# cuulee/reporter

Hardware: AMD Instinct MI355X
Metric: GPS probes matched/sec (whole node) (higher is better)
Workload: dtype f64; 1 GPU; c2; graph=metro, nodes=1048576, directed_edges=3527937, osmlr_segments=1361487, traces_per_gpu=10000, streams=1, device_batches=1, output_segments=1688548

## Files before the change

### reporter_amd/csrc/otr_devscan.h

```cpp
#pragma once
#include <hipcub/hipcub.hpp>

#include "otr_hostdev.h"

namespace otr {

struct Workspace {
  void* p = nullptr;
  size_t bytes = 0;
};


template <class In, class Out>
int scan_bytes(In in, Out out, int n, size_t* bytes, hipStream_t stream, std::string* err) {
  HIPCHK(hipcub::DeviceScan::InclusiveSum(nullptr, *bytes, in, out, n, stream));
  return OTR_OK;
}

template <class K, class V>
int sort_bytes(const K* k_in, K* k_out, const V* v_in, V* v_out, int n, int begin_bit, int end_bit, size_t* bytes,
               hipStream_t stream, std::string* err) {
  HIPCHK(hipcub::DeviceRadixSort::SortPairs(nullptr, *bytes, k_in, k_out, v_in, v_out, n, begin_bit, end_bit, stream));
  return OTR_OK;
}

template <class In, class Out, class K, class V>
int scan_sort_bytes(In in, Out out, const K* k_in, K* k_out, const V* v_in, V* v_out, int n, size_t* bytes,
                    hipStream_t stream, std::string* err) {
  size_t scan = 0, sort = 0;
  if (int rc = scan_bytes(in, out, n, &scan, stream, err)) return rc;
  if (int rc = sort_bytes(k_in, k_out, v_in, v_out, n, 0, 8 * (int)sizeof(K), &sort, stream, err)) return rc;
  *bytes = std::max(scan, sort);
  return OTR_OK;
}

template <class In, class Out>
int inclusive_sum(Workspace ws, In in, Out out, int n, hipStream_t stream, std::string* err) {
  HIPCHK(hipcub::DeviceScan::InclusiveSum(ws.p, ws.bytes, in, out, n, stream));
  return OTR_OK;
}

template <class K, class V>
int sort_pairs(Workspace ws, const K* k_in, K* k_out, const V* v_in, V* v_out, int n, int begin_bit, int end_bit,
               hipStream_t stream, std::string* err) {
  HIPCHK(hipcub::DeviceRadixSort::SortPairs(ws.p, ws.bytes, k_in, k_out, v_in, v_out, n, begin_bit, end_bit, stream));
  return OTR_OK;
}

template <class In, class Out>
int pool_scan(DevPool& pool, int slot, In in, Out out, int64_t n, hipStream_t stream, std::string* err) {
  Workspace ws;
  if (int rc = scan_bytes(in, out, (int)n, &ws.bytes, stream, err)) return rc;
  ws.p = pool.get<char>(slot, ws.bytes);
  return inclusive_sum(ws, in, out, (int)n, stream, err);
}

template <class K, class V>
int pool_sort(DevPool& pool, int slot, const K* k_in, K* k_out, const V* v_in, V* v_out, int64_t n, int begin_bit,
              int end_bit, hipStream_t stream, std::string* err) {
  Workspace ws;
  if (int rc = sort_bytes(k_in, k_out, v_in, v_out, (int)n, begin_bit, end_bit, &ws.bytes, stream, err)) return rc;
  ws.p = pool.get<char>(slot, ws.bytes);
  return sort_pairs(ws, k_in, k_out, v_in, v_out, (int)n, begin_bit, end_bit, stream, err);
}

template <class T>
struct Fetch {
  T* host;
  const T* dev;
};
template <class T>
Fetch<T> fetch(T* host, const T* dev) {
  return Fetch<T>{host, dev};
}
template <class... T>
int read_back(hipStream_t stream, std::string* err, Fetch<T>... f) {
  hipError_t e = hipSuccess;
  ((e = e != hipSuccess ? e : hipMemcpyAsync(f.host, f.dev, sizeof(T), hipMemcpyDeviceToHost, stream)), ...);
  HIPCHK(e);
  HIPCHK(hipStreamSynchronize(stream));
  return OTR_OK;
}

}
```

### reporter_amd/csrc/otr_engine.h

```cpp
#pragma once
#include <hip/hip_runtime.h>

#include <shared_mutex>
#include <string>
#include <vector>

#include "../../include/otr.h"
#include "otr_device.h"
#include "otr_hostdev.h"
#include "otr_tiers.h"

namespace otr {

struct Config {
  ModeParams mp;
  std::string graph_path;
  int device = 0;
};

ModeParams default_mode_params();
void finalize_params(MatchParams* p);
const char* check_params(const MatchParams& p);

struct GraphState {
  bool ready = false;
  int device = 0;
  DevGraph dg{};
  ModeParams defaults{};
  std::vector<void*> allocs;
  uint64_t n_nodes = 0, n_edges = 0, n_segments = 0;
  std::vector<unsigned long long> seg_id;
  std::shared_mutex mu;
};

GraphState& graph_state();
int engine_configure(const Config& cfg, std::string* err);

struct ReportLists {
  int32_t n;
  const int64_t* seg_off;
  const unsigned long long* seg_id;
  const double *start, *end;
  const uint8_t* internal;
  const int32_t* queue;
  const uint8_t* has_length;
  const int32_t *length, *begin_shape;
  const int64_t* end_time;
  const double* threshold;
  const uint32_t *rl, *tl;
  unsigned long long *rep_id, *rep_next;
  double *rep_t0, *rep_t1;
  int32_t *rep_length, *rep_queue, *n_rep, *shape_used, *counts;
  double* lengths;
  int32_t* length_set;
};

int report_lists_device(const ReportLists& h, std::string* err);

struct GSlab {
  uint32_t* key = nullptr;
  unsigned long long* lab = nullptr;
  uint32_t* qmark = nullptr;
  uint32_t* fr = nullptr;
  uint32_t* touched = nullptr;
};

void turn_table(double factor, int32_t* tab181);

uint64_t uuid_key_host(const char* uuid, int64_t len);

struct SessionStore;
void sessions_destroy(SessionStore* s);

struct SessionReports {
  int64_t n_windows, n_reports;
  const int64_t *trigger, *rep_off;
  const unsigned long long *id, *next_id;
  const double *t0, *t1;
  const int32_t *length, *queue_length;
  bool* added;
};
bool sessions_last_reports(SessionStore* s, SessionReports* out);

struct TileStore;
void tile_store_destroy(TileStore* s);

struct TileText;
void tile_text_destroy(TileText* t);

struct CulledRows {
  const otr_tile_row* sorted;
  const otr_tile_row* kept;
  const int64_t* kept_incl;
  int64_t n_kept;
};

struct Matcher {
  hipStream_t stream = nullptr;
  SessionStore* ses = nullptr;
  TileStore* tst = nullptr;
  TileText* ttx = nullptr;
  DevPool pool{PoolOwner::matcher, nullptr, 0};
  GSlab gslab[2];
  std::vector<int32_t> h_turn;
  std::vector<int64_t> h_trace_state_off, h_state_probe, h_trace_route_off, h_trace_seg_off, h_seg_way_off,
      h_trace_rep_off;
  std::vector<int32_t> h_cand_count, h_winner, h_subpath, h_seg_length, h_seg_queue, h_seg_bshape, h_seg_eshape,
      h_rep_length, h_rep_queue, h_shape_used, h_stats, h_trace_status;
  std::vector<uint32_t> h_cand_edge, h_route_edge, h_seg_way;
  std::vector<double> h_cand_p, h_cand_sqd, h_seg_start, h_seg_end, h_rep_t0, h_rep_t1, h_stats_len;
  std::vector<unsigned long long> h_seg_id, h_rep_id, h_rep_next;
  std::vector<uint8_t> h_seg_internal;
  std::vector<otr_tile_row> h_tile_rows;
  bool pts_have = false;
  otr_point_result pts{};
  std::vector<uint8_t> h_pt_kind;
  std::vector<uint32_t> h_pt_edge;
  std::vector<double> h_pt_frac, h_pt_lat, h_pt_lon, h_pt_dist;
  std::vector<int64_t> h_pt_state, h_pt_pos;
  bool trv_have = false;
  otr_traversal_result trv{};
  std::vector<int64_t> h_tr_off, h_tr_first, h_tr_s0, h_tr_s1;
  std::vector<uint32_t> h_tr_edge, h_tr_way;
  std::vector<uint64_t> h_tr_seg;
  std::vector<double> h_tr_f0, h_tr_f1, h_tr_t0, h_tr_t1;
  hipEvent_t ev[kEvents];
  bool ev_init = false;

  template <class T>
  T* need(int slot, size_t n);
  template <class T>
  T* want(int slot, size_t n);
  bool release_optional();
  bool opt_busy = false;
  int run(const otr_trace_batch* in, const ModeParams& mp, otr_batch_result* out, std::string* err);
  int matched_points(otr_point_result* out, std::string* err) const;
  int edge_traversals(otr_traversal_result* out, std::string* err) const;
  int edge_observations(int quantisation, otr_hist_entry** d_entries, int64_t* n, std::string* err);
  int tiles_cull(const otr_tile_row* rows, int64_t n, int memory, int privacy, int rules, const otr_tile_row** out,
                 int64_t* n_out, std::string* err);
  int hist_reduce(const void* in, int64_t n, int memory, int rows_in, int privacy, const otr_hist_entry** out,
                  int64_t* n_out, std::string* err);
  int cull_device(const otr_tile_row* d_in, int64_t n, int privacy, int rules, CulledRows* out, std::string* err);
  int copy_out(void* dst, const void* src, size_t bytes, int dst_memory, std::string* err);
  int ingest(const char* text, int64_t len, int memory, const otr_ingest_format* fmt, otr_ingest_result* out,
             std::string* err);
  int format_messages(const otr_message_format* fmt, const otr_messages* msgs, otr_format_result* out,
                      std::string* err);
  int sessions_open(const otr_session_config* cfg, int32_t uuid_bytes, std::string* err);
  int sessions_close(std::string* err);
  int sessions_push(const otr_session_points* pts, const otr_session_names* names, otr_session_result* out,
                    std::string* err);
  int sessions_punctuate(int64_t ts, otr_session_result* out, std::string* err);
  int sessions_advance(const otr_session_points* pts, const otr_session_names* names, otr_trace_batch* out,
                       std::string* err);
  int sessions_commit(const int32_t* shape_used, const int32_t* status, int memory, std::string* err);
  int sessions_windows(otr_session_result* out, std::string* err);
  int sessions_snapshot(otr_session_snapshot* out, std::string* err);
  int sessions_restore(const otr_session_snapshot* snap, const otr_session_names* names, int memory,
                       otr_session_restore_result* out, std::string* err);
  int sessions_restore_records(const otr_session_records* recs, const otr_session_names* names,
                               otr_session_restore_result* out, std::string* err);
  int sessions_export_records(otr_session_records* out, std::string* err);
  int sessions_take(int n_parts, int part, int remove, otr_session_snapshot* out, std::string* err);
  bool sessions_named() const;
  int sessions_names(otr_session_name_list* out, std::string* err);
  int sessions_last_refusal(otr_session_name_refusal* out, std::string* err);
  void sessions_refusal_message(const int64_t* d_message);
  void sessions_refusal_clear();
  const uint8_t* fmt_text = nullptr;
  int64_t fmt_text_len = 0;
  int tile_store_open(const otr_tile_store_config* cfg, int flags, std::string* err);
  int tile_store_snapshot(int flags, otr_tile_snapshot* out, std::string* err);
  int tile_store_restore(const otr_tile_snapshot* snap, int memory, otr_tile_restore_result* out, std::string* err);
  int tile_store_export_records(int32_t slice_size, otr_tile_records* out, std::string* err);
  int tile_store_restore_records(const otr_tile_records* in, otr_tile_restore_result* out, std::string* err);
  int tile_store_close(std::string* err);
  int tile_store_add_session(otr_tile_add_result* out, std::string* err);
  int tile_store_add_reports(int64_t n_windows, const int64_t* rep_off, const uint64_t* id, const uint64_t* next_id,
                             const double* t0, const double* t1, const int32_t* length, const int32_t* queue_length,
                             int memory, otr_tile_add_result* out, std::string* err);
  int tile_store_add_rows(const otr_tile_row* rows, int64_t n, int memory, otr_tile_add_result* out, std::string* err);
  int tile_store_flush(otr_tile_flush_result* out, std::string* err);
  int tiles_text(const otr_tile_row* rows, int64_t n, int memory, int quantisation, int rules, const char* source,
                 const char* mode, int flags, otr_tile_text_result* out, std::string* err);
  int tile_store_flush_text(const char* source, const char* mode, int flags, otr_tile_flush_result* flush,
                            otr_tile_text_result* out, std::string* err);
  ~Matcher();
};

}
```

### reporter_amd/csrc/otr_engine.hip

```cpp
#include <cerrno>
#include <cstdio>
#include <cstring>
#include <fcntl.h>
#include <sys/mman.h>
#include <sys/stat.h>
#include <unistd.h>

#include "otr_devscan.h"
#include "otr_engine.h"
#include "otr_kernels.h"
#include "otr_edge.h"
#include "otr_edge1.h"
#include "otr_launch.h"
#include "otr_points.h"
#include "otr_slots.h"
#include "otr_traversals.h"

namespace otr {
static_assert(kTraceWaves == 4, "grid_trace_rows (otr_launch.h) assumes 4 traces per block");

void finalize_params(MatchParams* p) {
  p->inv2s2 = 1.0 / (p->sigma_z * p->sigma_z * 2.0);
  p->inv_beta = 1.0 / p->beta;
  if (p->kmax > OTR_KMAX) p->kmax = OTR_KMAX;
  if (p->kmax < 1) p->kmax = 1;
}

const char* check_params(const MatchParams& p) {
  if (!(p.breakage_distance >= 0.0 && p.breakage_distance <= kMaxBreakage))
    return "breakage_distance must be within [0, 30000] m";
  if (!(p.max_route_distance_factor >= 0.0) || !(p.max_route_distance_factor < 1e6))
    return "max_route_distance_factor must be >= 0";
  if (!(p.max_route_time_factor >= 0.0) || !(p.max_route_time_factor < 1e6)) return "max_route_time_factor must be >= 0";
  if (!(p.turn_penalty_factor >= 0.0) || !(p.turn_penalty_factor <= 1e6)) return "turn_penalty_factor must be within [0, 1e6]";
  if (!(p.sigma_z > 0.0)) return "sigma_z must be > 0";
  if (!(p.beta > 0.0)) return "beta must be > 0";
  if (!(p.search_radius >= 0.0) || !(p.max_search_radius >= 0.0)) return "search_radius must be >= 0";
  if (!(p.interpolation_distance >= 0.0)) return "interpolation_distance must be >= 0";
  if (!(p.speed_kph >= 0.0) || !(p.queue_kph >= 0.0)) return "speed_kph and queue_kph must be >= 0";
  return nullptr;
}

ModeParams default_mode_params() {
  ModeParams mp{};
  for (int m = 0; m < OTR_MODES; ++m) {
    MatchParams& p = mp.m[m];
    p.sigma_z = 4.07;
    p.beta = 3.0;
    p.max_route_distance_factor = 5.0;
    p.max_route_time_factor = 2.0;
    p.breakage_distance = 2000.0;
    p.interpolation_distance = 10.0;
    p.search_radius = 50.0;
    p.max_search_radius = 100.0;
    p.gps_accuracy = 5.0;
    p.kmax = 32;
    p.queue_kph = 10.0;
  }
  mp.m[0].turn_penalty_factor = 200.0;
  mp.m[1].turn_penalty_factor = 140.0;
  mp.m[1].speed_kph = 18.0;
  mp.m[1].queue_kph = 5.0;
  mp.m[2].turn_penalty_factor = 100.0;
  mp.m[2].speed_kph = 5.1;
  mp.m[2].queue_kph = 2.0;
  for (int m = 0; m < OTR_MODES; ++m) finalize_params(&mp.m[m]);
  mp.delta = 60.0;
  return mp;
}

static uint32_t edge_time_ds(uint32_t attr, uint32_t len_mm, double speed_cap) {
  double kph = (double)OTR_ATTR_SPEED(attr);
  if (!(kph > 0.0)) kph = 30.0;
  if (speed_cap > 0.0 && speed_cap < kph) kph = speed_cap;
  const double v = (double)len_mm * 0.036 / kph;
  return v < 2.0e9 ? (uint32_t)llround(v) : 2000000000u;
}

static int seg_heading(const int32_t* a, const int32_t* b) {
  const double la1 = (double)a[0] * 1e-6, lo1 = (double)a[1] * 1e-6;
  const double la2 = (double)b[0] * 1e-6, lo2 = (double)b[1] * 1e-6;
  const double m = 20037581.187 / 180.0;
  const double x = (lo2 - lo1) * m * cos_deg(0.5 * (la1 + la2));
  const double y = (la2 - la1) * m;
  if (x == 0.0 && y == 0.0) return -1;
  double deg = atan2(x, y) * (180.0 / 3.14159265358979323846);
  if (deg < 0.0) deg = deg + 360.0;
  return (int)(llround(deg) % 360);
}

void turn_table(double factor, int32_t* tab) {
  const double x = -1.0 / 45.0;
  double r = 1.0, term = 1.0;
  for (int k = 1; k <= 20; ++k) {
    term = term * x / (double)k;
    r = r + term;
  }
  double f = 1.0;
  for (int i = 0; i <= 180; ++i) {
    const double v = 1000.0 * factor * f;
    tab[i] = factor > 0.0 ? (int32_t)llround(v) : 0;
    f = f * r;
  }
}

GraphState& graph_state() {
  static GraphState gs;
  return gs;
}

namespace {
struct Mapped {
  void* p = MAP_FAILED;
  size_t n = 0;
  ~Mapped() {
    if (p != MAP_FAILED) munmap(p, n);
  }
};
struct Staged {
  std::vector<void*> allocs;
  bool adopted = false;
  ~Staged() {
    if (!adopted)
      for (void* q : allocs) (void)hipFree(q);
  }
};
}

int engine_configure(const Config& cfg, std::string* err) {
  for (int m = 0; m < OTR_MODES; ++m)
    if (const char* bad = check_params(cfg.mp.m[m])) {
      if (err) *err = std::string("config: ") + bad;
      return OTR_BAD_REQUEST;
    }
  int fd = open(cfg.graph_path.c_str(), O_RDONLY);
  if (fd < 0) {
    if (err) *err = "cannot open graph file " + cfg.graph_path + ": " + strerror(errno);
    return OTR_BAD_REQUEST;
  }
  struct stat st;
  fstat(fd, &st);
  Mapped mf;
  mf.n = (size_t)st.st_size;
  mf.p = mf.n >= sizeof(otr_graph_header) ? mmap(nullptr, mf.n, PROT_READ, MAP_PRIVATE, fd, 0) : MAP_FAILED;
  close(fd);
  if (mf.p == MAP_FAILED) {
    if (err) *err = "cannot map graph file " + cfg.graph_path;
    return OTR_BAD_REQUEST;
  }
  const char* base = (const char*)mf.p;
  otr_graph_header h;
  memcpy(&h, base, sizeof(h));
  if (memcmp(h.magic, OTR_GRAPH_MAGIC, 8) != 0 || h.version != OTR_GRAPH_VERSION ||
      h.array_offset[OTR_A_END] > (uint64_t)st.st_size) {
    if (err) *err = "not an OTR graph file: " + cfg.graph_path;
    return OTR_BAD_REQUEST;
  }
  if (h.n_nodes >= (1u << 28)) {
    if (err) *err = "graph has more than 2^28 nodes";
    return OTR_BAD_REQUEST;
  }
  if (h.n_edges >= (1u << 28)) {
    if (err) *err = "graph has more than 2^28 directed edges";
    return OTR_BAD_REQUEST;
  }
  const uint32_t* dst = (const uint32_t*)(base + h.array_offset[OTR_A_EDGE_DST]);
  const float* lenf = (const float*)(base + h.array_offset[OTR_A_EDGE_LEN]);
  const uint32_t* attr = (const uint32_t*)(base + h.array_offset[OTR_A_EDGE_ATTR]);
  const uint32_t* row = (const uint32_t*)(base + h.array_offset[OTR_A_NODE_ROW]);
// ... 51 lines not shown
    int hb = -1, he = -1;
    for (uint32_t k = k0; k + 1 < k1 && hb < 0; ++k) hb = seg_heading(sll + 2ull * k, sll + 2ull * k + 2);
    for (uint32_t k = k1 - 1; k > k0 && he < 0; --k) he = seg_heading(sll + 2ull * k - 2, sll + 2ull * k);
    head[e] = make_short2((short)(hb < 0 ? 0 : hb), (short)(he < 0 ? 0 : he));
  }
  std::vector<uint2> adje(4ull * h.n_nodes + 4, make_uint2(0u, 0u));
  for (uint32_t u = 0; u < h.n_nodes; ++u)
    for (uint32_t k = 0; k < 4 && row[u] + k < row[u + 1]; ++k) {
      const uint32_t e = row[u] + k;
      adje[4ull * u + k] = make_uint2(e, (uint32_t)(uint16_t)head[e].x | ((uint32_t)(uint16_t)head[e].y << 16));
    }
  const size_t es = 4ull * h.n_edges + 4;
  std::vector<uint4> erec(es, make_uint4(kAdjDstMask, 0u, 0u, 0u));
  std::vector<uint32_t> erec_t(es * OTR_MODES, 0u);
  for (uint32_t b = 0; b < h.n_edges; ++b) {
    const uint32_t v = dst[b], deg = row[v + 1] - row[v];
    for (uint32_t k = 0; k < 4; ++k) {
      const uint32_t hend = (uint32_t)(uint16_t)head[b].y << 8;
      if (k >= deg) {
        erec[4ull * b + k] = make_uint4(kAdjDstMask, 0u, hend, v);
        continue;
      }
      const uint32_t e = row[v] + k;
      const uint32_t x = e | ((attr[e] & OTR_ATTR_ACCESS_MASK) << 28) | ((k == 3 && deg > 4) ? kAdjMore : 0u);
      erec[4ull * b + k] =
          make_uint4(x, len[e], (uint32_t)turn_degree((int)head[b].y, (int)head[e].x) | hend, v);
      for (int m = 0; m < OTR_MODES; ++m) erec_t[es * m + 4ull * b + k] = std::min(et[m][e], 0x1FFFFu);
    }
  }
  const uint32_t* cedge = (const uint32_t*)(base + h.array_offset[OTR_A_CELL_EDGE]);
  std::vector<uint4> crec(3 * ((size_t)h.n_cell_entries + 1), make_uint4(0u, 0u, 0u, 0u));
  for (uint64_t q = 0; q < h.n_cell_entries; ++q) {
    const uint32_t e = cedge[q];
    if (e >= h.n_edges) {
      if (err) *err = "graph cell index names a missing edge";
      return OTR_BAD_REQUEST;
    }
    const uint32_t k0 = eshape[e], k1 = eshape[e + 1];
    crec[3 * q] = make_uint4(e, k0, k1, attr[e]);
    uint32_t pt[8] = {0u, 0u, 0u, 0u, 0u, 0u, 0u, 0u};
    for (uint32_t i = 0; i < 4 && k0 + i < k1; ++i) {
      pt[2 * i] = (uint32_t)sll[2ull * (k0 + i)];
      pt[2 * i + 1] = (uint32_t)sll[2ull * (k0 + i) + 1];
    }
    crec[3 * q + 1] = make_uint4(pt[0], pt[1], pt[2], pt[3]);
    crec[3 * q + 2] = make_uint4(pt[4], pt[5], pt[6], pt[7]);
  }
  HIPCHK(hipSetDevice(cfg.device));
  Staged sg;
  bool alloc_ok = true;
  auto upv = [&](const void* src, size_t bytes) -> void* {
    void* d = nullptr;
    if (hipMalloc(&d, bytes ? bytes : 16) != hipSuccess) {
      alloc_ok = false;
      return nullptr;
    }
    sg.allocs.push_back(d);
    if (bytes && hipMemcpy(d, src, bytes, hipMemcpyHostToDevice) != hipSuccess) alloc_ok = false;
    return d;
  };
  auto up = [&](int a, size_t bytes) -> void* { return upv(base + h.array_offset[a], bytes); };
  DevGraph g{};
  g.node_row = (const uint32_t*)up(OTR_A_NODE_ROW, 4ull * (h.n_nodes + 1));
  g.rev_row = (const uint32_t*)up(OTR_A_REV_ROW, 4ull * (h.n_nodes + 1));
  g.node_ll = (const int2*)up(OTR_A_NODE_LL, 8ull * h.n_nodes);
  g.rev_edge = (const uint32_t*)up(OTR_A_REV_EDGE, 4ull * h.n_edges);
  g.edge_src = (const uint32_t*)up(OTR_A_EDGE_SRC, 4ull * h.n_edges);
  g.edge_dst = (const uint32_t*)up(OTR_A_EDGE_DST, 4ull * h.n_edges);
  g.edge_len = (const float*)up(OTR_A_EDGE_LEN, 4ull * h.n_edges);
  g.edge_attr = (const uint32_t*)up(OTR_A_EDGE_ATTR, 4ull * h.n_edges);
  g.edge_shape = (const uint32_t*)up(OTR_A_EDGE_SHAPE, 4ull * (h.n_edges + 1));
  g.edge_seg = (const uint32_t*)up(OTR_A_EDGE_SEG, 4ull * h.n_edges);
  g.edge_way = (const uint32_t*)up(OTR_A_EDGE_WAY, 4ull * h.n_edges);
  g.shape_ll = (const int2*)up(OTR_A_SHAPE_LL, 8ull * h.n_shape);
  g.seg_id = (const unsigned long long*)up(OTR_A_SEG_ID, 8ull * h.n_segments);
  g.seg_len = (const uint32_t*)up(OTR_A_SEG_LEN, 4ull * h.n_segments);
  g.cell_row = (const uint32_t*)up(OTR_A_CELL_ROW, 4ull * (h.n_cells + 1));
  g.cell_edge = (const uint32_t*)up(OTR_A_CELL_EDGE, 4ull * h.n_cell_entries);
  g.len_mm = (const uint32_t*)upv(len.data(), 4ull * len.size());
  g.edge_pack = (const uint4*)upv(pack.data(), sizeof(uint4) * pack.size());
  g.eprep = (const uint4*)upv(eprep.data(), sizeof(uint4) * eprep.size());
  g.adj = (const uint4*)upv(adj.data(), sizeof(uint4) * adj.size());
  g.node_minin = (const uint32_t*)upv(minin.data(), 4ull * minin.size());
  {
    std::vector<uint32_t> all_et, all_at;
    for (int m = 0; m < OTR_MODES; ++m) {
      all_et.insert(all_et.end(), et[m].begin(), et[m].end());
      all_at.insert(all_at.end(), at[m].begin(), at[m].end());
    }
    g.edge_t = (const uint32_t*)upv(all_et.data(), 4ull * all_et.size());
    g.adj_t = (const uint32_t*)upv(all_at.data(), 4ull * all_at.size());
    g.edge_t_stride = (uint32_t)et[0].size();
    g.adj_t_stride = (uint32_t)at[0].size();
  }
  g.edge_head = (const short2*)upv(head.data(), sizeof(short2) * head.size());
  g.adj_e = (const uint2*)upv(adje.data(), sizeof(uint2) * adje.size());
  g.erec = (const uint4*)upv(erec.data(), sizeof(uint4) * erec.size());
  g.erec_t = (const uint32_t*)upv(erec_t.data(), 4ull * erec_t.size());
  g.erec_stride = es;
  g.cell_rec = (const uint4*)upv(crec.data(), sizeof(uint4) * crec.size());
  if (!alloc_ok) {
    if (err) *err = "device allocation for the graph failed";
    return OTR_DEVICE_ERROR;
  }
  g.n_nodes = h.n_nodes;
  g.n_edges = h.n_edges;
  g.n_segments = h.n_segments;
  g.grid_rows = h.grid_rows;
  g.grid_cols = h.grid_cols;
  g.grid_min_lat = h.grid_min_lat;
  g.grid_min_lon = h.grid_min_lon;
  g.grid_cell_deg = h.grid_cell_deg;
  std::vector<unsigned long long> sid((const unsigned long long*)(base + h.array_offset[OTR_A_SEG_ID]),
                                      (const unsigned long long*)(base + h.array_offset[OTR_A_SEG_ID]) + h.n_segments);
  GraphState& gs = graph_state();
  std::vector<void*> old;
  {
    std::unique_lock<std::shared_mutex> lk(gs.mu);
    old.swap(gs.allocs);
    gs.allocs = sg.allocs;
    sg.adopted = true;
    gs.dg = g;
    gs.n_nodes = h.n_nodes;
    gs.n_edges = h.n_edges;
    gs.n_segments = h.n_segments;
    gs.seg_id.swap(sid);
    gs.defaults = cfg.mp;
    gs.device = cfg.device;
    gs.ready = true;
  }
  for (void* q : old) (void)hipFree(q);
  return OTR_OK;
}



bool Matcher::release_optional() {
  if (opt_busy) return false;
  bool any = false;
  for (int s = 0; s < (int)pool.b.size(); ++s)
    if (optional_slot(s) && pool.held(s, 0)) {
      if (!any && stream) (void)hipStreamSynchronize(stream);
      any = true;
      pool.drop(s);
    }
  return any;
}

Matcher::~Matcher() {
  if (ses) sessions_destroy(ses);
  if (tst) tile_store_destroy(tst);
  if (ttx) tile_text_destroy(ttx);
  pool.release();
  for (auto& sl : gslab)
    for (void* q : {(void*)sl.key, (void*)sl.lab, (void*)sl.qmark, (void*)sl.fr, (void*)sl.touched})
      if (q) (void)hipFree(q);
  if (ev_init)
    for (auto& e : ev) (void)hipEventDestroy(e);
  if (stream) (void)hipStreamDestroy(stream);
}

__global__ void k_capacity(int32_t n_traces, const int64_t* trace_state_off, const int32_t* cand_count,
                           const int32_t* path_len, int64_t* cap) {
  int t = blockIdx.x * blockDim.x + threadIdx.x;
  if (t >= n_traces) return;
  int64_t c = 2;
  for (int64_t s = trace_state_off[t]; s < trace_state_off[t + 1]; ++s) {
    if (cand_count[s] <= 0) continue;
    c += 3;
    if (path_len[s] > 0) c += path_len[s];
  }
  cap[t] = c;
}

__global__ void k_fill_i32(int32_t* p, int64_t n, int32_t v) {
  int64_t i = (int64_t)blockIdx.x * blockDim.x + threadIdx.x;
  if (i < n) p[i] = v;
}

__device__ inline void block_append(bool hit, int64_t value, int64_t* list, unsigned long long* count) {
  __shared__ unsigned int s_n;
  __shared__ unsigned long long s_base;
  if (threadIdx.x == 0) s_n = 0;
  __syncthreads();
  unsigned int my = 0;
  if (hit) my = atomicAdd(&s_n, 1u);
  __syncthreads();
  if (threadIdx.x == 0) s_base = s_n ? atomicAdd(count, (unsigned long long)s_n) : 0ull;
  __syncthreads();
  if (hit) list[s_base + my] = value;
}

__global__ void k_collect(int64_t n, const int32_t* flag, int64_t* list, unsigned long long* count) {
  const int64_t i = (int64_t)blockIdx.x * blockDim.x + threadIdx.x;
  block_append(i < n && flag[i], i, list, count);
}

__global__ void k_collect_tier(int64_t n, int32_t* flag, uint32_t want, int64_t* list, unsigned long long* count) {
  const int64_t i = (int64_t)blockIdx.x * blockDim.x + threadIdx.x;
  const int f = i < n ? flag[i] : 0;
  const bool sel = f != 0 && ((want >> f) & 1u);
  if (sel) flag[i] = 0;
  block_append(sel, i, list, count);
}

__global__ void k_collect_flagged(int64_t n, const int32_t* flag, int64_t* list, unsigned long long* count) {
  const int64_t i = (int64_t)blockIdx.x * blockDim.x + threadIdx.x;
  block_append(i < n && flag[i] != 0, i, list, count);
}

__global__ void k_collect_tier_from(const int64_t* cand, const unsigned long long* n_cand, int32_t* flag,
                                    uint32_t want, int64_t* list, unsigned long long* count) {
  const int64_t n = (int64_t)*n_cand;
  for (int64_t base = (int64_t)blockIdx.x * blockDim.x; base < n; base += (int64_t)gridDim.x * blockDim.x) {
    const int64_t i = base + threadIdx.x;
    const int64_t task = i < n ? cand[i] : 0;
    const int f = i < n ? flag[task] : 0;
    const bool sel = f != 0 && ((want >> f) & 1u);
    if (sel) flag[task] = 0;
    block_append(sel, task, list, count);
  }
}

constexpr int kSortBuckets = 4096;
__global__ __launch_bounds__(1024) void k_sort_hist(const int64_t* list, const unsigned long long* n_in,
                                                    const uint4* rec, int shift, uint32_t* hist) {
  __shared__ uint32_t h[kSortBuckets];
  const int64_t n = (int64_t)*n_in, i = (int64_t)blockIdx.x * blockDim.x + threadIdx.x;
  if ((int64_t)blockIdx.x * blockDim.x >= n) return;
  for (int b = threadIdx.x; b < kSortBuckets; b += blockDim.x) h[b] = 0;
  __syncthreads();
  if (i < n) atomicAdd(&h[min(rec[3 * list[i]].z >> shift, (uint32_t)kSortBuckets - 1u)], 1u);
  __syncthreads();
  for (int b = threadIdx.x; b < kSortBuckets; b += blockDim.x)
    if (h[b]) atomicAdd(&hist[b], h[b]);
}
__global__ __launch_bounds__(1024) void k_sort_scan(uint32_t* hist) {
  __shared__ uint32_t part[1024];
  constexpr int per = kSortBuckets / 1024;
  uint32_t v[per], t = 0;
  for (int q = 0; q < per; ++q) t += (v[q] = hist[threadIdx.x * per + q]);
  part[threadIdx.x] = t;
  __syncthreads();
  for (int off = 1; off < 1024; off <<= 1) {
    const uint32_t x = threadIdx.x >= (unsigned)off ? part[threadIdx.x - off] : 0u;
    __syncthreads();
    part[threadIdx.x] += x;
    __syncthreads();
  }
  uint32_t base = part[threadIdx.x] - t;
  for (int q = 0; q < per; ++q) {
    hist[threadIdx.x * per + q] = base;
    base += v[q];
  }
}
__global__ __launch_bounds__(1024) void k_sort_place(const int64_t* list, const unsigned long long* n_in,
                                                     const uint4* rec, int shift, uint32_t* cursor, int64_t* out) {
  __shared__ uint32_t h[kSortBuckets];
  const int64_t n = (int64_t)*n_in, i = (int64_t)blockIdx.x * blockDim.x + threadIdx.x;
  if ((int64_t)blockIdx.x * blockDim.x >= n) return;
  for (int b = threadIdx.x; b < kSortBuckets; b += blockDim.x) h[b] = 0;
  __syncthreads();
  int64_t task = 0;
  uint32_t key = 0, r = 0;
  if (i < n) {
    task = list[i];
    key = min(rec[3 * task].z >> shift, (uint32_t)kSortBuckets - 1u);
    r = atomicAdd(&h[key], 1u);
  }
  __syncthreads();
  for (int b = threadIdx.x; b < kSortBuckets; b += blockDim.x)
    if (h[b]) h[b] = atomicAdd(&cursor[b], h[b]);
  __syncthreads();
  if (i < n) out[h[key] + r] = task;
}

__global__ void k_collect_tier_list(const unsigned long long* n_in, int32_t* flag, uint32_t want, int64_t* list,
                                    unsigned long long* count) {
  const int64_t i = (int64_t)blockIdx.x * blockDim.x + threadIdx.x;
  const int f = i < (int64_t)*n_in ? flag[i] : 0;
  const bool sel = f != 0 && ((want >> f) & 1u);
  if (sel) flag[i] = 0;
  block_append(sel, i, list, count);
}

__global__ void k_step_list(int64_t n_states, const int64_t* prev, const uint8_t* brk, const int32_t* cand_count,
                            int64_t* list, unsigned long long* count) {
  const int64_t s = (int64_t)blockIdx.x * blockDim.x + threadIdx.x;
  block_append(s < n_states && cand_count[s] > 0 && prev[s] >= 0 && !brk[s], s, list, count);
}

__global__ void k_step_lists(int64_t n_states, const int64_t* prev, const uint8_t* brk, const int32_t* cand_count,
                             PathClass pc, int64_t* list, unsigned long long* count_front,
                             unsigned long long* count_back, unsigned long long* n_all) {
  const int64_t s = (int64_t)blockIdx.x * blockDim.x + threadIdx.x;
  if (s == 0) *n_all = (unsigned long long)n_states;
  const bool hit = s < n_states && cand_count[s] > 0 && prev[s] >= 0 && !brk[s];
  bool small = false;
  if (hit) {
    const int64_t sp = prev[s];
    const int md = pc.mode[pc.state_trace[s]] < OTR_MODES ? pc.mode[pc.state_trace[s]] : 0;
    const uint32_t r = pc.trans[pc.trans_off[s] + (int64_t)pc.winner[sp] * cand_count[s] + pc.winner[s]];
    const double b = fmin(floor(pc.bound[s] * 1000.0), (double)r) * 1e-3;
    small = !((pc.turn_modes >> md) & 1u) && pc.est4 * (float)(b * b) <= pc.small_keys;
  }
  const unsigned long long mf = __ballot(hit && small), mb = __ballot(hit && !small);
  const int lane = (int)(threadIdx.x % OTR_WAVE);
  unsigned long long bf = 0, bb = 0;
  if (lane == 0) {
    if (mf) bf = atomicAdd(count_front, (unsigned long long)__popcll(mf));
    if (mb) bb = atomicAdd(count_back, (unsigned long long)__popcll(mb));
  }
  bf = __shfl(bf, 0);
  bb = __shfl(bb, 0);
  const unsigned long long below = (1ull << lane) - 1ull;
  if (hit && small) list[bf + __popcll(mf & below)] = s;
  if (hit && !small) list[n_states - 1 - (int64_t)(bb + __popcll(mb & below))] = s;
}

__global__ __launch_bounds__(kCShards) void k_ctr_fold(const unsigned long long* in, unsigned long long* out) {
  __shared__ unsigned long long part[kCShards / OTR_WAVE];
  unsigned long long v = in[(size_t)blockIdx.x * kCShards + threadIdx.x];
  for (int o = OTR_WAVE / 2; o > 0; o >>= 1) v += __shfl_xor(v, o);
  if (lane_id() == 0) part[threadIdx.x / OTR_WAVE] = v;
  __syncthreads();
  if (threadIdx.x == 0) {
    unsigned long long t = 0;
    for (int w = 0; w < kCShards / OTR_WAVE; ++w) t += part[w];
    out[blockIdx.x] = t;
  }
}

constexpr double kSmallKeys = 24.0;
constexpr double kTinyKeys = 12.0;
constexpr double kSmallPathKeys = 16.0;

static const std::vector<int>& route_tiers() {
  static const std::vector<int> t = parse_route_tiers(getenv("OTR_TIERS"));
  return t;
}

static unsigned pgrid(unsigned full, int64_t units) {
  const int64_t u = std::max<int64_t>(8, (units + 7) / 8 * 8);
  return (unsigned)std::min<int64_t>((int64_t)full, u);
}

constexpr unsigned kCollectGrid = 512;

struct Batch {
  Matcher& mat;
  const otr_trace_batch* in;
  const ModeParams& mp;
  otr_batch_result* out;
  std::string* err;
  const DevGraph& g;
  hipStream_t stream;
  bool timing;
  bool used[10] = {false};
  int32_t T = 0;
  int64_t N = 0, S = 0, NT = 0, NT4 = 0, NT8 = 0, NTR = 0, C = 0;
  BatchDev b{};
  CandBuf cb{};
  StepBuf sb{};
  PrepArgs pr{};
  RouteArgs ra{};
  GenArgs ga{};
  ViterbiArgs va{};
  SegArgs sa{};
  HistArgs ha{};
  PointArgs pta{};
  bool want_points = false;
  TravArgs tva{};
  bool want_traversals = false;
  int64_t n_trav = 0;
  size_t hist_len = 0, scan_bytes = 0;
  int64_t *trace_state_off = nullptr, *state_probe = nullptr, *trans_off = nullptr, *path_off = nullptr,
          *cap_off = nullptr;
  int32_t *state_trace = nullptr, *path_len = nullptr;
  uint32_t turn_modes = 0;
  bool k32 = true;
  int vit_variant = 0;
  int route_g = 2, n_est_tiers = 0;
  float est_k = 0.f, est_v[OTR_MODES] = {};
  uint32_t est_tier_keys[8] = {0u, 0u, 0u, 0u, 0u, 0u, 0u, 0u};
  double tiny_keys = 0.0;
  static constexpr size_t bank = (size_t)OTR_COUNTERS * kCShards;
  static constexpr size_t n_ctr = kBanks * (size_t)OTR_COUNTERS;
  unsigned long long *d_counters = nullptr, *cnt = nullptr;
  int64_t *list = nullptr, *fail_tasks = nullptr, *flagged = nullptr;
  int32_t *task_ovf = nullptr, *d_turn = nullptr;
  uint32_t *trans = nullptr, *trans_tc = nullptr;
  uint4* task_rec = nullptr;
  unsigned long long *rwork = nullptr, *queues = nullptr;
  int32_t* task_dump = nullptr;
  bool node_tasks = true, turns = false, nresume = true, eresume = true;
  int64_t* steps = nullptr;
  unsigned long long *nsteps_d = nullptr, *nsteps4_d = nullptr, h_nsteps[2] = {0ull, 0ull};
  const unsigned long long* nscan_d = nullptr;
  int32_t* step_ovf = nullptr;
  bool small_paths = false;
  std::vector<unsigned long long> hc;
  unsigned long long h_fail[2] = {0ull, 0ull};
  std::vector<int64_t> route_n, seg_n, way_n, rep_n;

  int upload(), states(), candidates(), link(), route_first(), route_retry(), route_edge(), route_global(), viterbi();
  int paths(), paths_attempt(int64_t capacity), segments(), points(), traversals(), drain(), debug_fail(),
      name_failed();
  void fold_counters();
  int copy_out(), points_out(), traversals_out();

  template <class X> X* need(int slot, size_t n) { return mat.need<X>(slot, n); }
  template <class X> X* want(int slot, size_t n) { return mat.want<X>(slot, n); }
  void tb(int k) {
    if (timing) (void)hipEventRecord(mat.ev[2 * k], stream);
  }
  void te(int k) {
    if (timing) (void)hipEventRecord(mat.ev[2 * k + 1], stream), used[k] = true;
  }
  void tier_begin(int slot) {
    if (timing) (void)hipEventRecord(mat.ev[route_event(slot)], stream);
  }
  void tier_end(int slot) {
    if (timing) (void)hipEventRecord(mat.ev[route_event(slot) + 1], stream);
  }
  unsigned long long* tier_bank(int slot) const { return d_counters + kRouteTiers[slot].bank * bank; }
  unsigned long long* tier_work(int slot) const { return rwork ? tier_bank(slot) : nullptr; }
  unsigned long long* tier_list(int slot) const { return cnt + kRouteTiers[slot].list; }
  unsigned long long* tier_queue(int slot) const { return queues + kRouteTiers[slot].queue * kQueueWords; }
  unsigned long long ctr(int bank_, int k) const { return hc[(size_t)bank_ * OTR_COUNTERS + (size_t)k]; }

  int scan(const int64_t* src, int64_t* dst_np1, int64_t n);
  int read_i64(const int64_t* p, int64_t* v);
  int slabs(int tier, GSlabs* out);
  template <class V>
  int dl(V& vec, const void* src, size_t n) {
    vec.resize(n ? n : 1);
    if (n) HIPCHK(hipMemcpyAsync(vec.data(), src, n * sizeof(vec[0]), hipMemcpyDeviceToHost, stream));
    return OTR_OK;
  }
  template <int CAP, int G, bool LIST>
  void launch_route(unsigned grid, const RouteArgs& args, unsigned long long* ctr_bank);
  void first_tier(int slot, int cap, int g_, int64_t n_tasks, int64_t task_base, int64_t units);
  int retry_tier(int code, const RouteArgs& rb, unsigned long long* ctr_bank);
};

int Matcher::run(const otr_trace_batch* in, const ModeParams& mp, otr_batch_result* out, std::string* err) {
  pts_have = false;
  pts = otr_point_result{};
  trv_have = false;
  trv = otr_traversal_result{};
  const int rc = guarded(stream, err, [&]() -> int {
    GraphState& gs = graph_state();
    std::shared_lock<std::shared_mutex> graph_lock(gs.mu);
    if (!gs.ready) {
      if (err) *err = "otr_configure has not been called";
      return OTR_NOT_CONFIGURED;
    }
    HIPCHK(hipSetDevice(gs.device));
    if (!stream) HIPCHK(hipStreamCreateWithFlags(&stream, hipStreamNonBlocking));
    if (!ev_init) {
      for (auto& e : ev) HIPCHK(hipEventCreate(&e));
      ev_init = true;
    }
    memset(out, 0, sizeof(*out));
    out->n_traces = in->n_traces;
    if (in->n_traces <= 0) {
      pts_have = (in->flags & OTR_BATCH_MATCHED_POINTS) != 0;
      if (in->flags & OTR_BATCH_EDGE_TRAVERSALS) {
        trv.d_trace_off = need<int64_t>(S_TR_OFF, 1);
        HIPCHK(hipMemsetAsync(trv.d_trace_off, 0, 8, stream));
        HIPCHK(hipStreamSynchronize(stream));
        if (in->flags & OTR_BATCH_COPY_OUT) {
          h_tr_off.assign(1, 0);
          trv.trace_off = h_tr_off.data();
        }
        trv_have = true;
      }
      return OTR_OK;
    }
    Batch c{*this, in, mp, out, err, gs.dg, stream, (in->flags & OTR_BATCH_TIMING) != 0};
    c.T = in->n_traces;
    c.want_points = (in->flags & OTR_BATCH_MATCHED_POINTS) != 0;
    c.want_traversals = (in->flags & OTR_BATCH_EDGE_TRAVERSALS) != 0;
    int rc;
    if ((rc = c.upload()) || (rc = c.states()) || (rc = c.candidates()) || (rc = c.link()) || (rc = c.route_first()) ||
        (rc = c.route_retry()) || (rc = c.route_edge()) || (rc = c.route_global()) || (rc = c.viterbi()) ||
        (rc = c.paths()) || (rc = c.segments()) || (rc = c.points()) || (rc = c.traversals()) || (rc = c.drain()) ||
        (rc = c.debug_fail()) || (rc = c.name_failed()))
      return rc;
    c.fold_counters();
    if ((rc = c.copy_out()) || (rc = c.points_out())) return rc;
    return c.traversals_out();
  });
  opt_busy = false;
  return rc;
}

int Batch::upload() {
  b.n_traces = T;
  if (in->memory == OTR_MEM_HOST) {
    N = in->trace_offsets[T];
    int64_t* d_off = need<int64_t>(S_TRACE_OFF, T + 1);
    double* d_lat = need<double>(S_LAT, N);
    double* d_lon = need<double>(S_LON, N);
    int64_t* d_time = need<int64_t>(S_TIME, N);
    uint8_t* d_mode = need<uint8_t>(S_MODE, T);
    float* d_acc = in->accuracy ? need<float>(S_ACC, N) : nullptr;
    HIPCHK(hipMemcpyAsync(d_off, in->trace_offsets, 8 * (T + 1), hipMemcpyHostToDevice, stream));
    HIPCHK(hipMemcpyAsync(d_lat, in->lat, 8 * N, hipMemcpyHostToDevice, stream));
    HIPCHK(hipMemcpyAsync(d_lon, in->lon, 8 * N, hipMemcpyHostToDevice, stream));
    HIPCHK(hipMemcpyAsync(d_time, in->time, 8 * N, hipMemcpyHostToDevice, stream));
    HIPCHK(hipMemcpyAsync(d_mode, in->mode, T, hipMemcpyHostToDevice, stream));
    if (d_acc) HIPCHK(hipMemcpyAsync(d_acc, in->accuracy, 4 * N, hipMemcpyHostToDevice, stream));
    b.trace_off = d_off;
    b.lat = d_lat;
    b.lon = d_lon;
    b.time = d_time;
    b.mode = d_mode;
    b.acc = d_acc;
  } else {
    if (int rc = read_back(stream, err, fetch(&N, in->trace_offsets + T))) return rc;
    b.trace_off = in->trace_offsets;
    b.lat = in->lat;
    b.lon = in->lon;
    b.time = in->time;
    b.mode = in->mode;
    b.acc = in->accuracy;
  }
  out->n_probes = N;
  if (N > kMaxBatchProbes || max_launch_items(N, N, 1) > kMaxDispatchItems) {
    if (err)
      *err = "batch of " + std::to_string(N) + " probes: at most " + std::to_string(kMaxBatchProbes) +
             " per otr_match_batch call";
    return OTR_BAD_REQUEST;
  }
  mat.h_trace_status.assign(T, OTR_OK);
  d_counters = need<unsigned long long>(S_COUNTERS, kBanks * bank + n_ctr);
  HIPCHK(hipMemsetAsync(d_counters, 0, kBanks * bank * 8, stream));
  return OTR_OK;
}

int Batch::scan(const int64_t* src, int64_t* dst_np1, int64_t n) {
  HIPCHK(hipMemsetAsync(dst_np1, 0, 8, stream));
  if (n == 0) return OTR_OK;
  Workspace tmp;
  if (int rc = otr::scan_bytes(src, dst_np1 + 1, (int)n, &tmp.bytes, stream, err)) return rc;
  scan_bytes = std::max(scan_bytes, tmp.bytes);
  tmp.p = need<char>(S_SCAN_TMP, scan_bytes);
  return inclusive_sum(tmp, src, dst_np1 + 1, (int)n, stream, err);
}

int Batch::read_i64(const int64_t* p, int64_t* v) { return read_back(stream, err, fetch(v, p)); }

int Batch::states() {
  int rc;
  int64_t* state_cnt = need<int64_t>(S_STATE_CNT, T);
  trace_state_off = need<int64_t>(S_TRACE_STATE_OFF, T + 1);
  tb(OTR_STAGE_STATES);
  k_select_states<<<grid_ceil(T, 256), 256, 0, stream>>>(b, mp, state_cnt, nullptr, nullptr, nullptr);
  te(OTR_STAGE_STATES);
  if ((rc = scan(state_cnt, trace_state_off, T))) return rc;
  if ((rc = read_i64(trace_state_off + T, &S))) return rc;
  out->n_states = S;
  state_probe = need<int64_t>(S_STATE_PROBE, S);
  state_trace = need<int32_t>(S_STATE_TRACE, S);
  k_select_states<<<grid_ceil(T, 256), 256, 0, stream>>>(b, mp, state_cnt, trace_state_off, state_probe,
                                                         state_trace);
  return OTR_OK;
}

int Batch::candidates() {
  cb.edge = need<uint32_t>(S_CAND_EDGE, (size_t)S * OTR_KMAX);
  cb.p = need<double>(S_CAND_P, (size_t)S * OTR_KMAX);
  cb.sqd = need<double>(S_CAND_SQD, (size_t)S * OTR_KMAX);
  cb.count = need<int32_t>(S_CAND_COUNT, S);
  cb.radius = need<double>(S_CAND_RADIUS, S);
  if (S > 0) {
    tb(OTR_STAGE_CANDIDATES);
    bool kc32 = true;
    for (int m = 0; m < OTR_MODES; ++m) {
      const MatchParams& q = mp.m[m];
      const double rmax = b.acc ? q.max_search_radius
                                : std::min(q.max_search_radius, std::max(q.search_radius, q.gps_accuracy));
      kc32 = kc32 && q.kmax <= 32 && rmax <= 100.0;
    }
    static const int cand_g = getenv("OTR_CAND_G") ? atoi(getenv("OTR_CAND_G")) : 2;
    if (kc32 && cand_g == 2)
      k_candidates<2><<<(unsigned)grid_candidates((S + 1) / 2).blocks, 64, 0, stream>>>(g, b, mp, S, state_probe,
                                                                                       state_trace, cb, d_counters);
    else
      k_candidates<1><<<(unsigned)grid_candidates(S).blocks, 64, 0, stream>>>(g, b, mp, S, state_probe, state_trace, cb,
                                                                        d_counters);
    te(OTR_STAGE_CANDIDATES);
  }
  return OTR_OK;
}

int Batch::link() {
  int rc;
  for (int m = 0; m < OTR_MODES; ++m)
    if (mp.m[m].turn_penalty_factor > 0.0) turn_modes |= 1u << m;
  sb.prev = need<int64_t>(S_PREV, S);
  sb.g = need<double>(S_G, S);
  sb.bound = need<double>(S_BOUND, S);
  sb.forced = need<uint8_t>(S_FORCED, S);
  sb.bt = need<int32_t>(S_BT, S);
  sb.ntask = need<int64_t>(S_NTASK, S);
  sb.ntrans = need<int64_t>(S_NTRANS, S);
  int64_t* task_off = need<int64_t>(S_TASK_OFF, S + 1);
  trans_off = need<int64_t>(S_TRANS_OFF, S + 1);
  tb(OTR_STAGE_LINK);
  k_link<<<(unsigned)grid_link(T).blocks, 256, 0, stream>>>(b, mp, trace_state_off, state_probe, cb.count, sb);
  pr.n_states = S;
  pr.prev = sb.prev;
  pr.bound = sb.bound;
  pr.cand_count = cb.count;
  pr.cand_edge = cb.edge;
  pr.cand_p = cb.p;
  pr.state_trace = state_trace;
  pr.mode = b.mode;
  pr.cprep = need<uint4>(S_CPREP, (size_t)S * OTR_KMAX);
  pr.cprep_t = need<uint2>(S_CPREP_T, (size_t)S * OTR_KMAX);
  pr.clen = need<uint2>(S_CLEN, (size_t)S * OTR_KMAX);
  pr.nroot = need<int32_t>(S_CAND_NROOT, S);
  pr.turn_modes = turn_modes;
  for (int m = 0; m < OTR_MODES; ++m) k32 = k32 && mp.m[m].kmax <= 32;
  if (S > 0) {
    if (k32) k_prep<2><<<(unsigned)grid_per_state_waves(S, 2).blocks, 256, 0, stream>>>(g, pr);
    else k_prep<1><<<(unsigned)grid_per_state_waves(S, 1).blocks, 256, 0, stream>>>(g, pr);
  }
  static const int route_g_env = getenv("OTR_ROUTE_G") ? atoi(getenv("OTR_ROUTE_G")) : 2;
  route_g = route_g_env;
  {
    static const double est_scale = getenv("OTR_EST_K") ? atof(getenv("OTR_EST_K")) : 1.0;
    const double mlat = g.grid_min_lat + 0.5 * g.grid_rows * g.grid_cell_deg;
    const double area = (g.grid_rows * g.grid_cell_deg * kMetersPerDeg) *
                        (g.grid_cols * g.grid_cell_deg * kMetersPerDeg * cos_deg(fmin(fabs(mlat), 89.0)));
    est_k = (float)(est_scale * 0.5 * (area > 0.0 ? (double)g.n_nodes / area : 0.0));
    for (int m = 0; m < OTR_MODES; ++m) {
      const double kph = mp.m[m].speed_kph > 0.0 && mp.m[m].speed_kph < 50.0 ? mp.m[m].speed_kph : 50.0;
      est_v[m] = (float)(kph / 3.6);
    }
    const std::vector<int>& tl = route_tiers();
    n_est_tiers = (int)std::min<size_t>(tl.size(), 8);
    for (int t = 0; t < n_est_tiers; ++t) est_tier_keys[t] = (uint32_t)((tl[t] / 10) * 7 / 8);
  }
  static const double small_keys = getenv("OTR_SMALL_KEYS") ? atof(getenv("OTR_SMALL_KEYS")) : kSmallKeys;
  static const double tiny_keys_env = getenv("OTR_TINY_KEYS") ? atof(getenv("OTR_TINY_KEYS")) : kTinyKeys;
  tiny_keys = tiny_keys_env;
  const bool small_tier = route_g == 2 && k32 && small_keys > 0.0 && est_k > 0.f;
  const bool tiny_tier = small_tier && tiny_keys > 0.0;
  int64_t* ntask4 = small_tier ? need<int64_t>(S_NTASK4, S) : nullptr;
  int64_t* task4_off = small_tier ? need<int64_t>(S_TASK4_OFF, S + 1) : nullptr;
  int64_t* ntask8 = tiny_tier ? need<int64_t>(S_NTASK8, S) : nullptr;
  int64_t* task8_off = tiny_tier ? need<int64_t>(S_TASK8_OFF, S + 1) : nullptr;
  if (S > 0) {
    SmallArgs sm{};
    sm.ntask4 = ntask4;
    sm.ntask8 = ntask8;
    sm.tiny_keys = (float)tiny_keys;
    sm.bound = sb.bound;
    sm.bt = sb.bt;
    sm.forced = sb.forced;
    sm.cand_count = cb.count;
    sm.state_trace = state_trace;
    sm.mode = b.mode;
    sm.turn_modes = turn_modes;
    sm.est_k = est_k;
    for (int m = 0; m < OTR_MODES; ++m) sm.est_v[m] = est_v[m];
    sm.small_keys = (float)small_keys;
    k_ntask<<<grid_ceil(S, 256), 256, 0, stream>>>(S, sb.prev, pr.nroot, sb.ntask, sm);
  }
  if ((rc = scan(sb.ntask, task_off, S))) return rc;
  if (small_tier && (rc = scan(ntask4, task4_off, S))) return rc;
  if (tiny_tier && (rc = scan(ntask8, task8_off, S))) return rc;
  if ((rc = scan(sb.ntrans, trans_off, S))) return rc;
  HIPCHK(hipMemcpyAsync(&NT, task_off + S, 8, hipMemcpyDeviceToHost, stream));
  if (small_tier) HIPCHK(hipMemcpyAsync(&NT4, task4_off + S, 8, hipMemcpyDeviceToHost, stream));
  if (tiny_tier) HIPCHK(hipMemcpyAsync(&NT8, task8_off + S, 8, hipMemcpyDeviceToHost, stream));
  if ((rc = read_back(stream, err, fetch(&NTR, trans_off + S)))) return rc;
  NT += NT4 + NT8;
  task_ovf = need<int32_t>(S_TASK_OVF, NT);
  trans = need<uint32_t>(S_TRANS, NTR);
  trans_tc = need<uint32_t>(S_TRANS_TC, turn_modes ? NTR : 1);
  task_rec = need<uint4>(S_TASK_REC, 3 * (size_t)std::max<int64_t>(NT, 1));
  if (S > 0) {
    TaskArgs ta{};
    ta.n_states = S;
    ta.prev = sb.prev;
    ta.cand_count = cb.count;
    ta.cand_edge = cb.edge;
    ta.edge_dst = g.edge_dst;
    ta.task_off = task_off;
    ta.bound = sb.bound;
    ta.forced = sb.forced;
    ta.bt = sb.bt;
    ta.state_trace = state_trace;
    ta.mode = b.mode;
    ta.cprep = pr.cprep;
    ta.cprep_t = pr.cprep_t;
    ta.trans_off = trans_off;
    ta.turn_modes = turn_modes;
    ta.rec = task_rec;
    ta.ntask4 = ntask4;
    ta.task4_off = task4_off;
    ta.nt4 = NT4;
    ta.ntask8 = ntask8;
    ta.task8_off = task8_off;
    ta.nt8 = NT8;
    ta.flag_turn = task_ovf;
    ta.est_first_keys = route_g == 2 ? (OTR_CAP1 * OTR_LOAD1) / 8 : 0;
    ta.est_k = est_k;
    for (int m = 0; m < OTR_MODES; ++m) ta.est_v[m] = est_v[m];
    ta.n_tiers = n_est_tiers;
    for (int t = 0; t < n_est_tiers; ++t) ta.tier_keys[t] = est_tier_keys[t];
    if (NT > 0) HIPCHK(hipMemsetAsync(task_ovf, 0, 4 * NT, stream));
    if (k32) k_tasks<2><<<(unsigned)grid_per_state_waves(S, 2).blocks, 256, 0, stream>>>(ta);
    else k_tasks<1><<<(unsigned)grid_per_state_waves(S, 1).blocks, 256, 0, stream>>>(ta);
  }
  te(OTR_STAGE_LINK);
  return OTR_OK;
}

int Batch::slabs(int tier, GSlabs* out) {
  GSlab& sl = mat.gslab[tier];
  const uint32_t cap = (uint32_t)kRouteTiers[SLOT_GLOBAL + tier].cap;
  const uint32_t n = tier == 0 ? 1024u : 8u;
  if (!sl.key) {
    const size_t c = (size_t)cap * n;
    void* p[5] = {nullptr, nullptr, nullptr, nullptr, nullptr};
    const size_t bytes[5] = {4 * c, 8 * c, 4 * c, 8 * c, 4 * c};
    bool good = true;
    for (int attempt = 0; attempt < 2; ++attempt) {
      good = true;
      for (int q = 0; q < 5 && good; ++q) good = hipMalloc(&p[q], bytes[q]) == hipSuccess;
      if (good) break;
      (void)hipGetLastError();
      for (void*& q : p)
        if (q) (void)hipFree(q), q = nullptr;
      if (attempt > 0 || !mat.release_optional()) break;
    }
    if (good)
      good = hipMemsetAsync(p[0], 0xFF, 4 * c, stream) == hipSuccess &&
             hipMemsetAsync(p[1], 0xFF, 8 * c, stream) == hipSuccess &&
             hipMemsetAsync(p[2], 0, 4 * c, stream) == hipSuccess;
    if (!good) {
      (void)hipGetLastError();
      for (void* q : p)
        if (q) (void)hipFree(q);
      throw DeviceOom{PoolOwner::matcher, nullptr, S_NUM + tier, 28 * c};
    }
    sl.key = (uint32_t*)p[0];
    sl.lab = (unsigned long long*)p[1];
    sl.qmark = (uint32_t*)p[2];
    sl.fr = (uint32_t*)p[3];
    sl.touched = (uint32_t*)p[4];
  }
  out->key = sl.key;
  out->lab = sl.lab;
  out->qmark = sl.qmark;
  out->fr = sl.fr;
  out->touched = sl.touched;
  out->cap = cap;
  out->n = n;
  return OTR_OK;
}

template <int CAP, int G, bool LIST>
void Batch::launch_route(unsigned grid, const RouteArgs& args, unsigned long long* ctr_bank) {
  if (ctr_bank) k_route<CAP, G, LIST, false, true><<<grid, 64, 0, stream>>>(g, args, ctr_bank);
  else k_route<CAP, G, LIST, false, false><<<grid, 64, 0, stream>>>(g, args, nullptr);
}

void Batch::first_tier(int slot, int cap, int g_, int64_t n_tasks, int64_t task_base, int64_t units) {
  constexpr int64_t kMaxUnits = 1ll << 25;
  unsigned long long* ctr_bank = tier_work(slot);
  if (slot != SLOT_FIRST) tier_begin(slot);
  for (int64_t base = 0; base < units; base += kMaxUnits) {
    RouteArgs rf = ra;
    rf.n_tasks = n_tasks;
    rf.task_base = task_base;
    rf.unit_base = base;
    const int64_t u = std::min<int64_t>(kMaxUnits, units - base);
    const unsigned grid = (unsigned)(8 * ((u + 7) / 8));
    if (slot == SLOT_TINY) launch_route<OTR_CAP8, 8, false>(grid, rf, ctr_bank);
    else if (slot == SLOT_SMALL) launch_route<OTR_CAP4, 4, false>(grid, rf, ctr_bank);
    else if (g_ == 2) launch_route<OTR_CAP1, 2, false>(grid, rf, ctr_bank);
    else launch_route<256, 1, false>(grid, rf, ctr_bank);
  }
  if (slot != SLOT_FIRST) tier_end(slot);
  out->route_tier_code[slot] = route_tier_code(slot, cap, g_);
}

template <int I = 0, class F>
static bool with_retry_shape(int code, F&& f) {
  if constexpr (I < kRetryShapeN) {
    if (code == kRetryShapes[I].code()) {
      f(std::integral_constant<int, I>{});
      return true;
    }
    return with_retry_shape<I + 1>(code, f);
  } else {
    return false;
  }
}

int Batch::retry_tier(int code, const RouteArgs& rb, unsigned long long* ctr_bank) {
  const bool known = with_retry_shape(code, [&](auto i) {
    constexpr int cap = kRetryShapes[decltype(i)::value].cap, gw = kRetryShapes[decltype(i)::value].g;
    launch_route<cap, gw, true>(pgrid(cap <= 512 ? 16384u : 16384u * 512u / cap, (NT + gw - 1) / gw), rb, ctr_bank);
  });
  if (!known) {
    if (err) *err = "no route kernel for retry tier " + std::to_string(code);
    return OTR_DEVICE_ERROR;
  }
  return OTR_OK;
}

int Batch::route_first() {
  d_turn = need<int32_t>(S_TURN, 181 * OTR_MODES);
  mat.h_turn.resize(181 * OTR_MODES);
  for (int m = 0; m < OTR_MODES; ++m) turn_table(mp.m[m].turn_penalty_factor, mat.h_turn.data() + 181 * m);
  HIPCHK(hipMemcpyAsync(d_turn, mat.h_turn.data(), 4 * 181 * OTR_MODES, hipMemcpyHostToDevice, stream));
  ra.task_list = nullptr;
  ra.n_tasks = NT;
  ra.prev = sb.prev;
  ra.g = sb.g;
  ra.bound = sb.bound;
  ra.forced = sb.forced;
  ra.trans_off = trans_off;
  ra.trans = trans;
  ra.cand_count = cb.count;
  ra.cand_edge = cb.edge;
  ra.cand_p = cb.p;
  ra.state_trace = state_trace;
  ra.mode = b.mode;
  ra.bt = sb.bt;
  ra.turn = d_turn;
  ra.trans_tc = trans_tc;
  ra.cprep = pr.cprep;
  ra.cprep_t = pr.cprep_t;
  ra.clen = pr.clen;
  ra.rec = task_rec;
  for (int m = 0; m < OTR_MODES; ++m) ra.inv_beta[m] = mp.m[m].inv_beta;
  ra.overflow_flag = task_ovf;
  ra.stamps = d_counters;
  ra.est_k = est_k;
  for (int m = 0; m < OTR_MODES; ++m) ra.est_v[m] = est_v[m];
  ra.n_tiers = n_est_tiers;
  for (int t = 0; t < n_est_tiers; ++t) ra.tier_keys[t] = est_tier_keys[t];
  cnt = need<unsigned long long>(S_MISC, C_CURSORS + kShards);
  HIPCHK(hipMemsetAsync(cnt, 0, 8 * (C_CURSORS + kShards), stream));
  list = need<int64_t>(S_LIST, std::max<int64_t>(NT, S));
  fail_tasks = need<int64_t>(S_GFLAG, std::max<int64_t>(NT, 1));
  flagged = need<int64_t>(S_FLAGGED, std::max<int64_t>(NT, 1));
  ga.prev = sb.prev;
  ga.g = sb.g;
  ga.bt = sb.bt;
  ga.bound = sb.bound;
  ga.cand_count = cb.count;
  ga.cand_edge = cb.edge;
  ga.cand_p = cb.p;
  ga.cprep = pr.cprep;
  ga.cprep_t = pr.cprep_t;
  ga.state_trace = state_trace;
  ga.mode_of_trace = b.mode;
  ga.turn_modes = turn_modes;
  ga.turn = d_turn;
  ga.rec = task_rec;
  ga.trans_off = trans_off;
  ga.trans = trans;
  ga.trans_tc = trans_tc;
  ga.counters = d_counters;
  ga.n_overflow = cnt + C_GEN_OVERFLOW;
  if (NT == 0) return OTR_OK;
  rwork = (in->flags & OTR_BATCH_ROUTE_WORK) ? d_counters : nullptr;
  turns = turn_modes != 0u;
#ifdef OTR_FORCE_GENERAL
  node_tasks = true;
#else
  node_tasks = turn_modes != (1u << OTR_MODES) - 1u;
#endif
#ifdef OTR_FORCE_RETRY
  {
    const char* fe = getenv("OTR_FORCE_EDGE");
    ra.force_edge = fe ? atoi(fe) : 0;
  }
#endif
  queues = need<unsigned long long>(S_QUEUE, kQueues * kQueueWords);
  HIPCHK(hipMemsetAsync(queues, 0, 8 * kQueues * kQueueWords, stream));
  static const bool nresume_env = !getenv("OTR_NRESUME") || atoi(getenv("OTR_NRESUME")) != 0;
  static const bool eresume_env = !getenv("OTR_E1RESUME") || atoi(getenv("OTR_E1RESUME")) != 0;
  nresume = nresume_env;
  eresume = eresume_env;
  if ((nresume && node_tasks) || (eresume && turns)) task_dump = want<int32_t>(S_TASK_DUMP, NT);
  mat.opt_busy = true;
  ra.task_dump = task_dump;
  tb(OTR_STAGE_ROUTE);
  if (node_tasks) {
    const bool tiny_run = NT8 > 0 && (2 * NT8 >= NT || tiny_keys >= 1e8);
    const int64_t small_lo = tiny_run ? NT8 : 0;
    if (tiny_run) first_tier(SLOT_TINY, OTR_CAP8, 8, NT8, 0, (NT8 + 7) / 8);
    if (NT8 + NT4 - small_lo > 0)
      first_tier(SLOT_SMALL, OTR_CAP4, 4, NT8 + NT4, small_lo, (NT8 + NT4 - small_lo + 3) / 4);
    if (route_g == 2) first_tier(SLOT_FIRST, OTR_CAP1, 2, NT, NT8 + NT4, (NT - NT8 - NT4 + 1) / 2);
    else first_tier(SLOT_FIRST, 256, 1, NT, NT8 + NT4, NT);
  }
  te(OTR_STAGE_ROUTE);
  return OTR_OK;
}

int Batch::route_retry() {
  if (NT == 0) return OTR_OK;
  int rc;
  tb(OTR_STAGE_ROUTE_BIG);
  const std::vector<int>& tiers = route_tiers();
  const int ntier = (int)tiers.size();
  k_collect_flagged<<<grid_ceil(NT, 1024), 1024, 0, stream>>>(NT, task_ovf, flagged, cnt + C_FLAGGED);
  unsigned long long* ndump[2] = {nullptr, nullptr};
  uint32_t nslots[8] = {0u, 0u, 0u, 0u, 0u, 0u, 0u, 0u};
  auto nd_in = [&](int t) { return t > 0 && t < ntier && tiers[t] / 10 >= OTR_ND_IN_MIN; };
  auto nd_out = [&](int t) { return t + 1 < ntier && tiers[t] / 10 >= OTR_ND_OUT_MIN && nd_in(t + 1); };
  if (nresume && node_tasks && task_dump && ntier > 1) {
    static const double gb = getenv("OTR_NDUMP_GB") ? atof(getenv("OTR_NDUMP_GB")) : 4.0;
    const int64_t cap_bytes = (int64_t)(gb * (double)(1ll << 30));
    size_t words[2] = {0, 0};
    for (int t = 0; t + 1 < ntier && t < 8; ++t) {
      if (!nd_out(t)) continue;
      const uint32_t w = nd_words(tiers[t] / 10);
      nslots[t] = (uint32_t)std::min<int64_t>(std::max<int64_t>(NT / 4, 1024), cap_bytes / (8 * (int64_t)w));
      words[t & 1] = std::max<size_t>(words[t & 1], (size_t)nslots[t] * w);
    }
    for (int q = 0; q < 2; ++q)
      if (words[q]) ndump[q] = want<unsigned long long>(q == 0 ? S_NDUMP0 : S_NDUMP1, words[q]);
    if ((words[0] && !ndump[0]) || (words[1] && !ndump[1])) ndump[0] = ndump[1] = nullptr;
  }
  for (int tier = 0; tier < (node_tasks ? ntier : 0); ++tier) {
    const int slot = SLOT_NODE + tier;
    unsigned long long* c = tier_list(slot);
    k_collect_tier_from<<<kCollectGrid, 1024, 0, stream>>>(flagged, cnt + C_FLAGGED, task_ovf,
                                                          0x2u | (((2u << tier) - 1u) << 16), list + 0, c);
    RouteArgs rb = ra;
    rb.task_list = list;
    rb.list_count = c;
    rb.queue = tier_queue(slot);
    const bool din = nd_in(tier) && nd_out(tier - 1) && ndump[(tier + 1) & 1] != nullptr;
    const bool dout = nd_out(tier) && ndump[tier & 1] != nullptr;
    rb.dump_in = din ? ndump[(tier + 1) & 1] : nullptr;
    rb.dump_in_words = din ? nd_words(tiers[tier - 1] / 10) : 0u;
    rb.dump_out = dout ? ndump[tier & 1] : nullptr;
    rb.dump_ctr = queues + dump_ctr_word(slot);
    rb.dump_out_words = dout ? nd_words(tiers[tier] / 10) : 0u;
    rb.dump_out_slots = dout ? nslots[tier] : 0u;
    out->route_tier_code[slot] = tiers[tier];
    tier_begin(slot);
    if ((rc = retry_tier(tiers[tier], rb, tier_work(slot)))) return rc;
    tier_end(slot);
  }
#ifndef OTR_FORCE_GENERAL
  {
    constexpr int cap = kRouteTiers[SLOT_WIDE64].cap;
    unsigned long long* c = tier_list(SLOT_WIDE64);
    k_collect_tier_from<<<kCollectGrid, 1024, 0, stream>>>(flagged, cnt + C_FLAGGED, task_ovf, 0x8u, list, c);
    RouteArgs rb = ra;
    rb.task_list = list;
    rb.list_count = c;
    rb.queue = tier_queue(SLOT_WIDE64);
    out->route_tier_code[SLOT_WIDE64] = route_tier_code(SLOT_WIDE64, cap, 1);
    tier_begin(SLOT_WIDE64);
    if (rwork) k_route<cap, 1, true, true, true><<<pgrid(4096, NT), 64, 0, stream>>>(g, rb, tier_bank(SLOT_WIDE64));
    else k_route<cap, 1, true, true, false><<<pgrid(4096, NT), 64, 0, stream>>>(g, rb, nullptr);
    tier_end(SLOT_WIDE64);
  }
#endif
  return OTR_OK;
}

int Batch::route_edge() {
  if (NT == 0) return OTR_OK;
  if (turns) {
    unsigned long long* dump[2] = {nullptr, nullptr};
    uint32_t dslots[2] = {0u, 0u};
    constexpr int cap512 = kRouteTiers[SLOT_EDGE_512].cap, cap1024 = kRouteTiers[SLOT_EDGE_1024].cap;
    const int caps[3] = {OTR_E1CAP, cap512, cap1024};
    const uint32_t dwords[2] = {e1_dump_words(OTR_E1CAP), e1_dump_words(cap512)};
    if (eresume && task_dump) {
      const int64_t cap_bytes[2] = {4ll << 30, 1ll << 30};
      const int64_t wanted[2] = {std::max<int64_t>(NT / 16, 4096), std::max<int64_t>(NT / 64, 1024)};
      for (int q = 0; q < 2; ++q) {
        const int64_t n = std::min<int64_t>(wanted[q], cap_bytes[q] / (8 * (int64_t)dwords[q]));
        dump[q] = want<unsigned long long>(q == 0 ? S_E1DUMP0 : S_E1DUMP1, (size_t)n * dwords[q]);
        dslots[q] = dump[q] ? (uint32_t)n : 0u;
      }
      if (!dump[0]) dump[1] = nullptr, dslots[1] = 0u;
    }
    for (int et = 0; et < 3; ++et) {
      const int slot = kEdgeSlots[et];
      out->route_tier_code[slot] = route_tier_code(slot, caps[et], 1);
      unsigned long long* c = tier_list(slot);
      k_collect_tier_from<<<kCollectGrid, 1024, 0, stream>>>(flagged, cnt + C_FLAGGED, task_ovf, 0x20u << et, list, c);
      RouteArgs rb = ra;
      rb.task_list = list;
      static const bool esort = !getenv("OTR_SORT") || atoi(getenv("OTR_SORT")) != 0;
      int64_t* list2 = nullptr;
      uint32_t* hist = nullptr;
      if (et == 0 && esort && NT >= 65536) {
        list2 = want<int64_t>(S_SORT_LIST, NT);
        hist = list2 ? want<uint32_t>(S_SORT_HIST, kSortBuckets) : nullptr;
      }
      if (list2 && hist) {
        int bits = 0;
        while (bits < 32 && (g.n_edges >> bits) > 0u) ++bits;
        const int shift = bits > 12 ? bits - 12 : 0;
        HIPCHK(hipMemsetAsync(hist, 0, 4 * kSortBuckets, stream));
        k_sort_hist<<<grid_ceil(NT, 1024), 1024, 0, stream>>>(list, c, task_rec, shift, hist);
        k_sort_scan<<<1, 1024, 0, stream>>>(hist);
        k_sort_place<<<grid_ceil(NT, 1024), 1024, 0, stream>>>(list, c, task_rec, shift, hist, list2);
        rb.task_list = list2;
      }
      rb.list_count = c;
      rb.queue = tier_queue(slot);
      rb.dump_in = et > 0 ? dump[et - 1] : nullptr;
      rb.dump_in_words = et > 0 ? dwords[et - 1] : 0u;
      rb.dump_in_cap = et == 1 ? OTR_E1CAP : cap512;
      rb.dump_out = et < 2 ? dump[et] : nullptr;
      rb.dump_ctr = queues + dump_ctr_word(slot);
      rb.dump_out_words = et < 2 ? dwords[et] : 0u;
      rb.dump_out_slots = et < 2 ? dslots[et] : 0u;
      rb.task_dump = task_dump;
      unsigned long long* rcn = tier_work(slot);
      tier_begin(slot);
      if (et == 0) k_route_e1<OTR_E1CAP><<<pgrid(8192, NT), 64, 0, stream>>>(g, rb, rcn);
      else if (et == 1) k_route_e1<cap512><<<pgrid(4096, NT), 64, 0, stream>>>(g, rb, rcn);
      else k_route_e1<cap1024><<<pgrid(2048, NT), 64, 0, stream>>>(g, rb, rcn);
      tier_end(slot);
    }
  }
  mat.opt_busy = false;
  return OTR_OK;
}

int Batch::route_global() {
  if (NT == 0) return OTR_OK;
  int rc;
  for (int gt = 0; gt < 2; ++gt) {
    const int slot = SLOT_GLOBAL + gt;
    unsigned long long* c = tier_list(slot);
    k_collect_tier_from<<<kCollectGrid, 1024, 0, stream>>>(flagged, cnt + C_FLAGGED, task_ovf,
                                                          gt == 0 ? 0x1Eu : 0x2u, list, c);
    GSlabs gs2;
    if ((rc = slabs(gt, &gs2))) return rc;
    ga.mode = 0;
    ga.list = list;
    ga.list_count = c;
    ga.flag = task_ovf;
    ga.counters = tier_bank(slot);
    out->route_tier_code[slot] = route_tier_code(slot, (int)gs2.cap, 0);
    tier_begin(slot);
    k_general<<<pgrid(gs2.n, NT), kGenThreads, 0, stream>>>(g, ga, gs2);
    tier_end(slot);
  }
  k_collect_tier_from<<<kCollectGrid, 1024, 0, stream>>>(flagged, cnt + C_FLAGGED, task_ovf, 0x1Eu, fail_tasks,
                                                        cnt + C_TASKS_LEFT);
  te(OTR_STAGE_ROUTE_BIG);
  return OTR_OK;
}

int Batch::viterbi() {
  va.n_traces = T;
  va.trace_state_off = trace_state_off;
  va.cand_count = cb.count;
  va.cand_sqd = cb.sqd;
  va.prev = sb.prev;
  va.trans_off = trans_off;
  va.trans = trans;
  va.trans_tc = trans_tc;
  va.turn_modes = turn_modes;
  va.g = sb.g;
  va.mode = b.mode;
  for (int m = 0; m < OTR_MODES; ++m) va.inv2s2[m] = mp.m[m].inv2s2;
  for (int m = 0; m < OTR_MODES; ++m) va.inv_beta[m] = mp.m[m].inv_beta;
  va.bp = need<int8_t>(S_BP, (size_t)S * OTR_KMAX);
  va.brk = need<uint8_t>(S_BRK, S);
  va.end_win = need<int32_t>(S_END_WIN, S);
  va.winner = need<int32_t>(S_WINNER, S);
  va.subpath = need<int32_t>(S_SUBPATH, S);
  tb(OTR_STAGE_VITERBI);
  {
    static const int64_t split_below = getenv("OTR_VIT_SPLIT") ? atoll(getenv("OTR_VIT_SPLIT")) : 8192;
    if (k32 && T < split_below) {
      vit_variant = 11;
      k_viterbi<1, true><<<(unsigned)(T < 1048576 ? T : 1048576), 64, 0, stream>>>(va, d_counters);
    } else if (k32) {
      vit_variant = 20;
      const int64_t w = (T + 1) / 2;
      k_viterbi<2><<<(unsigned)(w < 1048576 ? w : 1048576), 64, 0, stream>>>(va, d_counters);
    } else {
      vit_variant = 10;
      k_viterbi<1><<<(unsigned)(T < 1048576 ? T : 1048576), 64, 0, stream>>>(va, d_counters);
    }
  }
  te(OTR_STAGE_VITERBI);
  return OTR_OK;
}

int Batch::paths() {
  int rc;
  path_off = need<int64_t>(S_PATH_OFF, S);
  path_len = need<int32_t>(S_PATH_LEN, S);
  if (S > 0) k_fill_i32<<<grid_ceil(S, 256), 256, 0, stream>>>(path_len, S, 0);
  {
    steps = need<int64_t>(S_LIST2, std::max<int64_t>(S, 1));
    nsteps_d = cnt + C_STEPS;
    static const double small_path_keys =
        getenv("OTR_SMALL_PATH_KEYS") ? atof(getenv("OTR_SMALL_PATH_KEYS")) : kSmallPathKeys;
    small_paths = small_path_keys > 0.0 && est_k > 0.f && (small_path_keys >= 1e8 || 2 * (NT4 + NT8) >= NT);
    nsteps4_d = cnt + C_STEPS_FRONT;
    unsigned long long* nall_d = cnt + C_STEPS_ALL;
    static_assert(C_STEPS_ALL == C_STEPS_FRONT + 1, "cleared together below");
    if (S > 0 && small_paths) {
      PathClass pc{};
      pc.winner = va.winner;
      pc.trans_off = trans_off;
      pc.trans = trans;
      pc.bound = sb.bound;
      pc.state_trace = state_trace;
      pc.mode = b.mode;
      pc.turn_modes = turn_modes;
      pc.est4 = 8.f * est_k;
      pc.small_keys = (float)small_path_keys;
      HIPCHK(hipMemsetAsync(nsteps4_d, 0, 16, stream));
      k_step_lists<<<grid_ceil(S, 256), 256, 0, stream>>>(S, sb.prev, va.brk, cb.count, pc, steps, nsteps4_d, nsteps_d,
                                                          nall_d);
      if ((rc = read_back(stream, err, fetch(&h_nsteps[0], nsteps4_d), fetch(&h_nsteps[1], nsteps_d)))) return rc;
    } else if (S > 0) {
      k_step_list<<<grid_ceil(S, 1024), 1024, 0, stream>>>(S, sb.prev, va.brk, cb.count, steps, nsteps_d);
    }
    nscan_d = small_paths ? nall_d : nsteps_d;
    step_ovf = need<int32_t>(S_STEP_OVF, S + 1);
    int64_t capacity = kShards * ((int64_t)S * 24 / kShards + 1024);
    bool paths_fit = S == 0;
    for (int attempt = 0; attempt < 8 && S > 0; ++attempt) {
      if ((rc = paths_attempt(capacity))) return rc;
      unsigned long long capflag = 0;
      std::vector<unsigned long long> cur(kShards);
      HIPCHK(hipMemcpyAsync(&capflag, cnt + C_CAP_FLAG, 8, hipMemcpyDeviceToHost, stream));
      HIPCHK(hipMemcpyAsync(cur.data(), cnt + C_CURSORS, 8 * kShards, hipMemcpyDeviceToHost, stream));
      HIPCHK(hipStreamSynchronize(stream));
      if ((capflag & 0xFFFFFFFFu) == 0) {
        paths_fit = true;
        break;
      }
      unsigned long long mx = 0;
      for (auto c : cur) mx = c > mx ? c : mx;
      capacity = kShards * ((int64_t)mx + (int64_t)mx / 2 + 1024);
    }
    if (!paths_fit) {
      if (err) *err = "winner paths did not fit the path buffer after 8 attempts";
      return OTR_DEVICE_ERROR;
    }
  }
  return OTR_OK;
}

int Batch::paths_attempt(int64_t capacity) {
  int rc;
  uint32_t* path = need<uint32_t>(S_PATH, capacity);
  HIPCHK(hipMemsetAsync(step_ovf, 0, 4 * (S + 1), stream));
  HIPCHK(hipMemsetAsync(cnt + C_PATH_TIER, 0, 8 * (C_CAP_FLAG + 1 - C_PATH_TIER), stream));
  HIPCHK(hipMemsetAsync(cnt + C_EDGE_PATH, 0, 8 * 2, stream));
  HIPCHK(hipMemsetAsync(cnt + C_CURSORS, 0, 8 * kShards, stream));
  PathArgs pa{};
  pa.steps = steps;
  pa.n_steps = S;
  pa.n_steps_dev = nsteps_d;
  pa.prev = sb.prev;
  pa.bound = sb.bound;
  pa.brk = va.brk;
  pa.winner = va.winner;
  pa.cand_edge = cb.edge;
  pa.cand_p = cb.p;
  pa.state_trace = state_trace;
  pa.mode = b.mode;
  pa.cprep = ra.cprep;
  pa.cprep_t = ra.cprep_t;
  pa.bt = sb.bt;
  pa.turn_modes = turn_modes;
  pa.path_off = path_off;
  pa.path_len = path_len;
  pa.path = path;
  pa.cursor = cnt + C_CURSORS;
  pa.capacity = capacity;
  pa.overflow_flag = step_ovf;
  pa.cap_flag = (int32_t*)(cnt + C_CAP_FLAG);
  pa.cand_count = cb.count;
  pa.trans_off = trans_off;
  pa.trans = trans;
  pa.force_edge = ra.force_edge;
  constexpr int kPQWords = 16 * 8;
  unsigned long long* pq = need<unsigned long long>(S_PQUEUE, 8 * kPQWords);
  HIPCHK(hipMemsetAsync(pq, 0, 8 * 8 * kPQWords, stream));
  tb(OTR_STAGE_PATHS);
  if (small_paths) {
    if (h_nsteps[0] > 0) {
      PathArgs p4 = pa;
      p4.n_steps_dev = nsteps4_d;
      k_paths<OTR_CAP4, 4><<<(unsigned)grid_paths((int64_t)(h_nsteps[0] + 1) / 2).blocks, 64, 0, stream>>>(
          g, p4, nullptr, nullptr);
    }
    if (h_nsteps[1] > 0) {
      PathArgs p2 = pa;
      p2.from_back = true;
      k_paths<OTR_CAP1, 2><<<(unsigned)grid_paths((int64_t)h_nsteps[1]).blocks, 64, 0, stream>>>(g, p2, nullptr,
                                                                                                 nullptr);
    }
  } else {
    k_paths<OTR_CAP1, 2><<<(unsigned)grid_paths(S).blocks, 64, 0, stream>>>(g, pa, nullptr, nullptr);
  }
  te(OTR_STAGE_PATHS);
  tb(OTR_STAGE_PATHS_BIG);
  for (int tier = 0; tier < 3; ++tier) {
    unsigned long long* c = cnt + C_PATH_TIER + tier;
    k_collect_tier_list<<<grid_ceil(S, 1024), 1024, 0, stream>>>(nscan_d, step_ovf, 0x2u, list, c);
    PathArgs pb = pa;
    pb.queue = pq + tier * kPQWords;
    if (tier == 0) k_paths<512, 1><<<pgrid(16384, S), 64, 0, stream>>>(g, pb, list, c);
    else if (tier == 1) k_paths<1024, 1><<<pgrid(8192, S), 64, 0, stream>>>(g, pb, list, c);
    else k_paths<4096, 1><<<pgrid(4096, S), 64, 0, stream>>>(g, pb, list, c);
  }
  if (turn_modes != 0u) {
    for (int et = 0; et < 2; ++et) {
      unsigned long long* c = cnt + C_EDGE_PATH + et;
      k_collect_tier_list<<<grid_ceil(S, 1024), 1024, 0, stream>>>(nscan_d, step_ovf, et == 0 ? 0x20u : 0x40u,
                                                                   list, c);
      PathArgs pb = pa;
      pb.queue = pq + (3 + et) * kPQWords;
      if (et == 0) k_paths_edge<384><<<pgrid(4096, S), 64, 0, stream>>>(g, pb, d_turn, list, c, 6);
      else k_paths_edge<2048><<<pgrid(512, S), 64, 0, stream>>>(g, pb, d_turn, list, c, 3);
    }
  }
  ga.steps = steps;
  ga.winner = va.winner;
  ga.path_off = path_off;
  ga.path_len = path_len;
  ga.path = path;
  ga.cursor = cnt + C_CURSORS;
  ga.capacity = capacity;
  ga.cap_flag = (int32_t*)(cnt + C_CAP_FLAG);
  for (int gt = 0; gt < 2; ++gt) {
    unsigned long long* c = cnt + C_PATH_GLOBAL + gt;
    k_collect_tier_list<<<grid_ceil(S, 1024), 1024, 0, stream>>>(nscan_d, step_ovf, gt == 0 ? 0xAu : 0x2u, list,
                                                                 c);
    GSlabs gs2;
    if ((rc = slabs(gt, &gs2))) return rc;
    ga.mode = 1;
    ga.list = list;
    ga.list_count = c;
    ga.flag = step_ovf;
    ga.counters = nullptr;
    k_general<<<pgrid(gs2.n, S), kGenThreads, 0, stream>>>(g, ga, gs2);
  }
  k_collect_tier_list<<<grid_ceil(S, 1024), 1024, 0, stream>>>(nscan_d, step_ovf, 0xAu, list, cnt + C_PATHS_LEFT);
  te(OTR_STAGE_PATHS_BIG);
  return OTR_OK;
}

int Batch::segments() {
  int rc;
  int64_t* cap = need<int64_t>(S_CAP, T);
  cap_off = need<int64_t>(S_CAP_OFF, T + 1);
  k_capacity<<<grid_ceil(T, 256), 256, 0, stream>>>(T, trace_state_off, cb.count, path_len, cap);
  if ((rc = scan(cap, cap_off, T))) return rc;
  if ((rc = read_i64(cap_off + T, &C))) return rc;
  sa.b = b;
  sa.trace_state_off = trace_state_off;
  sa.state_probe = state_probe;
  sa.cand_count = cb.count;
  sa.cand_edge = cb.edge;
  sa.cand_p = cb.p;
  sa.prev = sb.prev;
  sa.brk = va.brk;
  sa.winner = va.winner;
  sa.path_off = path_off;
  sa.path_len = path_len;
  sa.path = (const uint32_t*)need<uint32_t>(S_PATH, 1);
  sa.pos = need<int64_t>(S_POS, S);
  sa.act = need<int64_t>(S_ACT, S);
  sa.ent = need<int64_t>(S_ENT, S);
  sa.suba = need<int32_t>(S_SUBA, S);
  sa.subb = need<int32_t>(S_SUBB, S);
  sa.por_e = need<uint32_t>(S_POR_E, C);
  sa.por_s0 = need<int64_t>(S_POR_S0, C);
  sa.por_s1 = need<int64_t>(S_POR_S1, C);
  sa.por_sa = need<int32_t>(S_POR_SA, C);
  sa.gstart = need<int32_t>(S_GSTART, C);
  sa.cap_off = cap_off;
  sa.route = need<uint32_t>(S_ROUTE, C);
  sa.route_n = need<int64_t>(S_ROUTE_N, T);
  sa.seg_id = need<unsigned long long>(S_SEG_ID, C);
  sa.seg_start = need<double>(S_SEG_START, C);
  sa.seg_end = need<double>(S_SEG_END, C);
  sa.seg_length = need<int32_t>(S_SEG_LEN, C);
  sa.seg_queue = need<int32_t>(S_SEG_QUEUE, C);
  sa.seg_internal = need<uint8_t>(S_SEG_INTERNAL, C);
  sa.seg_bshape = need<int32_t>(S_SEG_BSHAPE, C);
  sa.seg_eshape = need<int32_t>(S_SEG_ESHAPE, C);
  sa.seg_index = need<uint32_t>(S_SEG_INDEX, C);
  sa.seg_n = need<int64_t>(S_SEG_N, T);
  sa.seg_way_n = need<int64_t>(S_SEG_WAY_N, C);
  sa.seg_way = need<uint32_t>(S_SEG_WAY, C);
  sa.way_n = need<int64_t>(S_WAY_N, T);
  sa.rep_id = need<unsigned long long>(S_REP_ID, C);
  sa.rep_next = need<unsigned long long>(S_REP_NEXT, C);
  sa.rep_t0 = need<double>(S_REP_T0, C);
  sa.rep_t1 = need<double>(S_REP_T1, C);
  sa.rep_length = need<int32_t>(S_REP_LEN, C);
  sa.rep_queue = need<int32_t>(S_REP_QUEUE, C);
  sa.rep_seg = need<uint32_t>(S_REP_SEG, C);
  sa.rep_n = need<int64_t>(S_REP_N, T);
  sa.shape_used = need<int32_t>(S_SHAPE_USED, T);
  sa.stats = need<int32_t>(S_STATS, 7 * (size_t)T);
  sa.stats_len = need<double>(S_STATS_LEN, 2 * (size_t)T);
  sa.threshold = (double)(in->threshold_sec >= 0 ? in->threshold_sec : 15);
  sa.report_levels = in->report_levels;
  sa.transition_levels = in->transition_levels;
  for (int m = 0; m < OTR_MODES; ++m) sa.queue_kph[m] = mp.m[m].queue_kph;
  tb(OTR_STAGE_SEGMENTS);
  k_segments<<<(unsigned)grid_segments(T).blocks, 64, 0, stream>>>(g, sa, d_counters);
  te(OTR_STAGE_SEGMENTS);
  ha.b = b;
  ha.cap_off = cap_off;
  ha.rep_n = sa.rep_n;
  ha.rep_id = sa.rep_id;
  ha.rep_t0 = sa.rep_t0;
  ha.rep_t1 = sa.rep_t1;
  ha.rep_length = sa.rep_length;
  ha.rep_queue = sa.rep_queue;
  ha.rep_seg = sa.rep_seg;
  ha.quantisation = in->quantisation > 0 ? in->quantisation : 3600;
  ha.base_time = in->hist_base_time;
  ha.hours = in->hist_hours;
  ha.n_segments = g.n_segments;
  ha.n_rows = d_counters + 8 * kCShards;
  hist_len = (size_t)(in->hist_hours > 0 ? in->hist_hours : 0) * g.n_segments * OTR_HIST_BINS;
  ha.hist = hist_len ? (in->hist_device ? in->hist_device : need<uint32_t>(S_HIST, hist_len)) : nullptr;
  if (hist_len) HIPCHK(hipMemsetAsync(ha.hist, 0, hist_len * 4, stream));
  tb(OTR_STAGE_HISTOGRAM);
  if (hist_len || !(in->flags & OTR_BATCH_TILE_ROWS))
    k_histogram<<<(unsigned)grid_trace_rows(T).blocks, 256, 0, stream>>>(ha);
  te(OTR_STAGE_HISTOGRAM);
  if (in->flags & OTR_BATCH_TILE_ROWS) {
    TileArgs ta{};
    ta.b = b;
    ta.cap_off = cap_off;
    ta.rep_n = sa.rep_n;
    ta.rep_id = sa.rep_id;
    ta.rep_next = sa.rep_next;
    ta.rep_t0 = sa.rep_t0;
    ta.rep_t1 = sa.rep_t1;
    ta.rep_length = sa.rep_length;
    ta.rep_queue = sa.rep_queue;
    ta.quantisation = ha.quantisation;
    ta.rules = in->tile_rules;
    ta.row_cnt = need<int64_t>(S_ROW_CNT, T);
    k_tile_rows<<<(unsigned)grid_trace_rows(T).blocks, 256, 0, stream>>>(ta);
    int64_t* row_off = need<int64_t>(S_ROW_OFF, T + 1);
    if ((rc = scan(ta.row_cnt, row_off, T))) return rc;
    int64_t R = 0;
    if ((rc = read_i64(row_off + T, &R))) return rc;
    ta.row_off = row_off;
    ta.rows = need<otr_tile_row>(S_ROWS, R > 0 ? R : 1);
    if (R > 0) k_tile_rows<<<(unsigned)grid_trace_rows(T).blocks, 256, 0, stream>>>(ta);
    out->d_rows = ta.rows;
    out->n_rows = R;
  }
  HIPCHK(hipGetLastError());
  return OTR_OK;
}

int Batch::points() {
  if (!want_points) return OTR_OK;
  pta.b = b;
  pta.trace_state_off = trace_state_off;
  pta.state_probe = state_probe;
  pta.cand_count = cb.count;
  pta.cand_edge = cb.edge;
  pta.cand_p = cb.p;
  pta.winner = va.winner;
  pta.brk = va.brk;
  pta.path_off = path_off;
  pta.path_len = path_len;
  pta.path = sa.path;
  pta.act = sa.act;
  pta.pos = sa.pos;
  pta.kind = need<uint8_t>(S_PT_KIND, N);
  pta.edge = need<uint32_t>(S_PT_EDGE, N);
  pta.frac = need<double>(S_PT_FRAC, N);
  pta.lat = need<double>(S_PT_LAT, N);
  pta.lon = need<double>(S_PT_LON, N);
  pta.dist = need<double>(S_PT_DIST, N);
  pta.state = need<int64_t>(S_PT_STATE, N);
  pta.pos_mm = need<int64_t>(S_PT_POS, N);
  if (timing) (void)hipEventRecord(mat.ev[kPointsEvent], stream);
  k_matched_points<<<(unsigned)grid_segments(T).blocks, 64, 0, stream>>>(g, pta);
  if (timing) (void)hipEventRecord(mat.ev[kPointsEvent + 1], stream);
  HIPCHK(hipGetLastError());
  return OTR_OK;
}

int Batch::points_out() {
  int rc;
  if (!want_points) return OTR_OK;
  if (out->n_overflow_traces > 0) {
    int32_t* d_status = need<int32_t>(S_PT_STATUS, T);
    HIPCHK(hipMemcpyAsync(d_status, mat.h_trace_status.data(), 4 * (size_t)T, hipMemcpyHostToDevice, stream));
    k_points_failed<<<(unsigned)std::min<int64_t>(T, 1024), 64, 0, stream>>>(pta, d_status);
    HIPCHK(hipGetLastError());
  }
  otr_point_result& r = mat.pts;
  r.n_probes = N;
  if (timing) {
    (void)hipEventElapsedTime(&r.kernel_ms, mat.ev[kPointsEvent], mat.ev[kPointsEvent + 1]);
    (void)hipGetLastError();
  }
  r.d_kind = pta.kind;
  r.d_edge = pta.edge;
  r.d_frac = pta.frac;
  r.d_lat = pta.lat;
  r.d_lon = pta.lon;
  r.d_dist = pta.dist;
  r.d_state = pta.state;
  r.d_pos_mm = pta.pos_mm;
  if (in->flags & OTR_BATCH_COPY_OUT) {
    if ((rc = dl(mat.h_pt_kind, pta.kind, N)) || (rc = dl(mat.h_pt_edge, pta.edge, N)) ||
        (rc = dl(mat.h_pt_frac, pta.frac, N)) || (rc = dl(mat.h_pt_lat, pta.lat, N)) ||
        (rc = dl(mat.h_pt_lon, pta.lon, N)) || (rc = dl(mat.h_pt_dist, pta.dist, N)) ||
        (rc = dl(mat.h_pt_state, pta.state, N)) || (rc = dl(mat.h_pt_pos, pta.pos_mm, N)))
      return rc;
    r.kind = mat.h_pt_kind.data();
    r.edge = mat.h_pt_edge.data();
    r.frac = mat.h_pt_frac.data();
    r.lat = mat.h_pt_lat.data();
    r.lon = mat.h_pt_lon.data();
    r.dist = mat.h_pt_dist.data();
    r.state = mat.h_pt_state.data();
    r.pos_mm = mat.h_pt_pos.data();
  }
  HIPCHK(hipStreamSynchronize(stream));
  mat.pts_have = true;
  return OTR_OK;
}

int Matcher::matched_points(otr_point_result* out, std::string* err) const {
  if (!pts_have) {
    if (err)
      *err = "otr_matched_points: the matcher has run no batch, or its last otr_match_batch did not set "
             "OTR_BATCH_MATCHED_POINTS";
    return OTR_BAD_REQUEST;
  }
  *out = pts;
  return OTR_OK;
}

int Batch::traversals() {
  int rc;
  if (!want_traversals) return OTR_OK;
  tva.b = b;
  tva.trace_state_off = trace_state_off;
  tva.state_probe = state_probe;
  tva.cand_count = cb.count;
  tva.cand_edge = cb.edge;
  tva.cand_p = cb.p;
  tva.winner = va.winner;
  tva.act = sa.act;
  tva.pos = sa.pos;
  tva.subb = sa.subb;
  tva.por_e = sa.por_e;
  tva.por_s0 = sa.por_s0;
  tva.por_s1 = sa.por_s1;
  tva.por_sa = sa.por_sa;
  tva.cap_off = cap_off;
  tva.route = sa.route;
  tva.route_n = sa.route_n;
  tva.count = need<int64_t>(S_TR_CNT, T);
  int64_t* off = need<int64_t>(S_TR_OFF, T + 1);
  tva.trav_off = off;
  if (timing) (void)hipEventRecord(mat.ev[kTravEvent], stream);
  k_trav_count<<<(unsigned)grid_segments(T).blocks, 64, 0, stream>>>(tva);
  if ((rc = scan(tva.count, off, T))) return rc;
  if ((rc = read_i64(off + T, &n_trav))) return rc;
  const size_t n = (size_t)n_trav;
  tva.edge = need<uint32_t>(S_TR_EDGE, n);
  tva.way = need<uint32_t>(S_TR_WAY, n);
  tva.seg_id = need<unsigned long long>(S_TR_SEG, n);
  tva.first_state = need<int64_t>(S_TR_FIRST, n);
  tva.f0 = need<double>(S_TR_F0, n);
  tva.f1 = need<double>(S_TR_F1, n);
  tva.s0_mm = need<int64_t>(S_TR_S0, n);
  tva.s1_mm = need<int64_t>(S_TR_S1, n);
  tva.t_enter = need<double>(S_TR_T0, n);
  tva.t_exit = need<double>(S_TR_T1, n);
  if (n_trav > 0) k_edge_traversals<<<(unsigned)grid_segments(T).blocks, 64, 0, stream>>>(g, tva);
  if (timing) (void)hipEventRecord(mat.ev[kTravEvent + 1], stream);
  HIPCHK(hipGetLastError());
  return OTR_OK;
}

int Batch::traversals_out() {
  int rc;
  if (!want_traversals) return OTR_OK;
  otr_traversal_result& r = mat.trv;
  r.n_traversals = n_trav;
  r.n_traces = T;
  if (timing) {
    (void)hipEventElapsedTime(&r.kernel_ms, mat.ev[kTravEvent], mat.ev[kTravEvent + 1]);
    (void)hipGetLastError();
  }
  r.d_trace_off = const_cast<int64_t*>(tva.trav_off);
  r.d_edge = tva.edge;
  r.d_way = tva.way;
  r.d_seg_id = reinterpret_cast<uint64_t*>(tva.seg_id);
  r.d_first_state = tva.first_state;
  r.d_f0 = tva.f0;
  r.d_f1 = tva.f1;
  r.d_s0_mm = tva.s0_mm;
  r.d_s1_mm = tva.s1_mm;
  r.d_t_enter = tva.t_enter;
  r.d_t_exit = tva.t_exit;
  if (in->flags & OTR_BATCH_COPY_OUT) {
    const size_t n = (size_t)n_trav;
    if ((rc = dl(mat.h_tr_off, tva.trav_off, (size_t)T + 1)) || (rc = dl(mat.h_tr_edge, tva.edge, n)) ||
        (rc = dl(mat.h_tr_way, tva.way, n)) || (rc = dl(mat.h_tr_seg, tva.seg_id, n)) ||
        (rc = dl(mat.h_tr_first, tva.first_state, n)) || (rc = dl(mat.h_tr_f0, tva.f0, n)) ||
        (rc = dl(mat.h_tr_f1, tva.f1, n)) || (rc = dl(mat.h_tr_s0, tva.s0_mm, n)) ||
        (rc = dl(mat.h_tr_s1, tva.s1_mm, n)) || (rc = dl(mat.h_tr_t0, tva.t_enter, n)) ||
        (rc = dl(mat.h_tr_t1, tva.t_exit, n)))
      return rc;
    r.trace_off = mat.h_tr_off.data();
    r.edge = mat.h_tr_edge.data();
    r.way = mat.h_tr_way.data();
    r.seg_id = mat.h_tr_seg.data();
    r.first_state = mat.h_tr_first.data();
    r.f0 = mat.h_tr_f0.data();
    r.f1 = mat.h_tr_f1.data();
    r.s0_mm = mat.h_tr_s0.data();
    r.s1_mm = mat.h_tr_s1.data();
    r.t_enter = mat.h_tr_t0.data();
    r.t_exit = mat.h_tr_t1.data();
  }
  HIPCHK(hipStreamSynchronize(stream));
  mat.trv_have = true;
  return OTR_OK;
}

static const char kNoTraversals[] =
    ": the matcher has run no batch, or its last otr_match_batch did not set OTR_BATCH_EDGE_TRAVERSALS";

int Matcher::edge_traversals(otr_traversal_result* out, std::string* err) const {
  if (!trv_have) {
    if (err) *err = std::string("otr_edge_traversals") + kNoTraversals;
    return OTR_BAD_REQUEST;
  }
  *out = trv;
  return OTR_OK;
}

int Matcher::edge_observations(int quantisation, otr_hist_entry** d_entries, int64_t* n, std::string* err) {
  return guarded(stream, err, [&]() -> int {
    *d_entries = nullptr;
    *n = 0;
    if (!trv_have) {
      if (err) *err = std::string("otr_edge_observations") + kNoTraversals;
      return OTR_BAD_REQUEST;
    }
    const int64_t nt = trv.n_traversals;
    if (nt <= 0) return OTR_OK;
    if (nt >= (int64_t)INT32_MAX) {
      if (err) *err = "too many traversals for one call";
      return OTR_BAD_REQUEST;
    }
    GraphState& gs = graph_state();
    std::shared_lock<std::shared_mutex> graph_lock(gs.mu);
    HIPCHK(hipSetDevice(gs.device));
    TravObsArgs oa{};
    oa.n = nt;
    oa.edge = trv.d_edge;
    oa.first_state = trv.d_first_state;
    oa.f0 = trv.d_f0;
    oa.f1 = trv.d_f1;
    oa.s0_mm = trv.d_s0_mm;
    oa.s1_mm = trv.d_s1_mm;
    oa.t_enter = trv.d_t_enter;
    oa.t_exit = trv.d_t_exit;
    oa.quantisation = quantisation > 0 ? quantisation : 3600;
    oa.keep = need<int64_t>(S_TR_KEEP, (size_t)nt);
    int64_t* keep_off = need<int64_t>(S_TR_KEEP_OFF, (size_t)nt + 1);
    oa.keep_off = keep_off;
    int rc;
    Workspace tmp;
    if ((rc = scan_bytes(oa.keep, keep_off + 1, (int)nt, &tmp.bytes, stream, err))) return rc;
    tmp.p = need<char>(S_TR_TMP, tmp.bytes);
    const unsigned grid = (unsigned)std::min<int64_t>(kTravObsGrid, (nt + 255) / 256);
    k_trav_obs_keep<<<grid, 256, 0, stream>>>(oa);
    HIPCHK(hipMemsetAsync(keep_off, 0, 8, stream));
    if ((rc = inclusive_sum(tmp, oa.keep, keep_off + 1, (int)nt, stream, err))) return rc;
    int64_t ne = 0;
    if ((rc = read_back(stream, err, fetch(&ne, keep_off + nt)))) return rc;
    if (ne < 0 || ne > nt) {
      if (err) *err = "edge observations: the keep scan failed";
      return OTR_DEVICE_ERROR;
    }
    oa.entries = need<otr_hist_entry>(S_TR_ENTRIES, (size_t)ne);
    if (ne > 0) k_trav_obs_fill<<<grid, 256, 0, stream>>>(gs.dg, oa);
    HIPCHK(hipGetLastError());
    HIPCHK(hipStreamSynchronize(stream));
    *d_entries = oa.entries;
    *n = ne;
    return OTR_OK;
  });
}

int Batch::drain() {
  hc.resize(n_ctr);
  k_ctr_fold<<<(unsigned)n_ctr, kCShards, 0, stream>>>(d_counters, d_counters + kBanks * bank);
  HIPCHK(hipMemcpyAsync(hc.data(), d_counters + kBanks * bank, n_ctr * 8, hipMemcpyDeviceToHost, stream));
  HIPCHK(hipMemcpyAsync(&h_fail[0], cnt + C_TASKS_LEFT, 8, hipMemcpyDeviceToHost, stream));
  HIPCHK(hipMemcpyAsync(&h_fail[1], cnt + C_PATHS_LEFT, 8, hipMemcpyDeviceToHost, stream));
  route_n.resize(T), seg_n.resize(T), way_n.resize(T), rep_n.resize(T);
  HIPCHK(hipMemcpyAsync(route_n.data(), sa.route_n, 8 * T, hipMemcpyDeviceToHost, stream));
  HIPCHK(hipMemcpyAsync(seg_n.data(), sa.seg_n, 8 * T, hipMemcpyDeviceToHost, stream));
  HIPCHK(hipMemcpyAsync(rep_n.data(), sa.rep_n, 8 * T, hipMemcpyDeviceToHost, stream));
  HIPCHK(hipMemcpyAsync(way_n.data(), sa.way_n, 8 * T, hipMemcpyDeviceToHost, stream));
  HIPCHK(hipStreamSynchronize(stream));
  return OTR_OK;
}

int Batch::debug_fail() {
  if (h_fail[0] + h_fail[1] > 0 && getenv("OTR_DEBUG_FAIL")) {
    unsigned long long hc2[C_CURSORS];
    HIPCHK(hipMemcpy(hc2, cnt, 8 * C_CURSORS, hipMemcpyDeviceToHost));
    fprintf(stderr, "otr: %llu route tasks, %llu paths beyond every tier; tier lists:", h_fail[0], h_fail[1]);
    for (int k = 0; k < C_CURSORS; ++k) fprintf(stderr, " %llu", hc2[k]);
    fprintf(stderr, "\n");
    if (h_fail[1]) {
      const int64_t* steps_d = need<int64_t>(S_LIST2, 1);
      std::vector<int64_t> ks(std::min<unsigned long long>(h_fail[1], 6));
      HIPCHK(hipMemcpy(ks.data(), list, 8 * ks.size(), hipMemcpyDeviceToHost));
      for (int64_t k : ks) {
        int64_t s = 0, sp = 0, to = 0;
        int32_t wi = 0, wj = 0, K = 0;
        double bd = 0;
        HIPCHK(hipMemcpy(&s, steps_d + k, 8, hipMemcpyDeviceToHost));
        HIPCHK(hipMemcpy(&sp, sb.prev + s, 8, hipMemcpyDeviceToHost));
        HIPCHK(hipMemcpy(&wj, need<int32_t>(S_WINNER, 1) + s, 4, hipMemcpyDeviceToHost));
        HIPCHK(hipMemcpy(&wi, need<int32_t>(S_WINNER, 1) + sp, 4, hipMemcpyDeviceToHost));
        HIPCHK(hipMemcpy(&K, cb.count + s, 4, hipMemcpyDeviceToHost));
        HIPCHK(hipMemcpy(&to, trans_off + s, 8, hipMemcpyDeviceToHost));
        HIPCHK(hipMemcpy(&bd, sb.bound + s, 8, hipMemcpyDeviceToHost));
        uint32_t r = 0;
        HIPCHK(hipMemcpy(&r, trans + to + (int64_t)wi * K + wj, 4, hipMemcpyDeviceToHost));
        fprintf(stderr, "otr: step k %lld state %lld prev %lld winners %d/%d K %d trans_off %lld bound %.3f route %u\n",
                (long long)k, (long long)s, (long long)sp, wi, wj, K, (long long)to, bd, r);
      }
    }
  }
  return OTR_OK;
}

int Batch::name_failed() {
  if (h_fail[0] + h_fail[1] > 0) {
    for (int which = 0; which < 2; ++which) {
      const unsigned long long nf = h_fail[which];
      if (!nf) continue;
      std::vector<int64_t> idx(nf), st(nf);
      HIPCHK(hipMemcpy(idx.data(), which == 0 ? fail_tasks : list, 8 * nf, hipMemcpyDeviceToHost));
      const int64_t* src = need<int64_t>(S_LIST2, 1);
      for (unsigned long long k = 0; k < nf; ++k) {
        int64_t sidx = 0;
        int32_t t = 0;
        if (which == 0) {
          uint32_t s32 = 0;
          HIPCHK(hipMemcpy(&s32, task_rec + 3 * idx[k], 4, hipMemcpyDeviceToHost));
          sidx = s32;
        } else {
          HIPCHK(hipMemcpy(&sidx, src + idx[k], 8, hipMemcpyDeviceToHost));
        }
        HIPCHK(hipMemcpy(&t, state_trace + sidx, 4, hipMemcpyDeviceToHost));
        if (t >= 0 && t < T && mat.h_trace_status[t] == OTR_OK) {
          mat.h_trace_status[t] = OTR_MATCH_ERROR;
          ++out->n_overflow_traces;
        }
      }
    }
  }
  return OTR_OK;
}

void Batch::fold_counters() {
  const int bank_first = kRouteTiers[SLOT_FIRST].bank;
  for (int k = 0; k < OTR_COUNTERS; ++k) out->counters[k] = ctr(bank_first, k);
  for (int k : {3, 4, 13, 14})
    out->counters[k] += ctr(kRouteTiers[SLOT_SMALL].bank, k) + ctr(kRouteTiers[SLOT_TINY].bank, k);
  out->counters[11] = out->counters[12] = 0;
  for (int t = 0; t < kRouteSlots; ++t) {
    const int tb_ = kRouteTiers[t].bank;
    const TierKind kind = kRouteTiers[t].kind;
    out->route_tier_work[t][0] = ctr(tb_, 6);
    out->route_tier_work[t][1] = ctr(tb_, 3);
    out->route_tier_work[t][2] = ctr(tb_, 4);
    out->route_tier_work[t][3] = ctr(tb_, 5);
    if (kind == TierKind::NodeRetry || kind == TierKind::Wide64) {
      out->counters[9] += ctr(tb_, 3);
      out->counters[10] += ctr(tb_, 4);
    }
    if (kind == TierKind::NodeRetry) {
      out->counters[11] += ctr(tb_, 11);
      out->counters[12] += ctr(tb_, 12);
    }
  }
  out->counters[5] = (uint64_t)NT;
  out->counters[6] = (uint64_t)NTR;
  out->counters[22] = ctr(kRouteTiers[kEdgeSlots[1]].bank, 22) + ctr(kRouteTiers[kEdgeSlots[2]].bank, 22);
  out->counters[23] = ctr(kRouteTiers[kEdgeSlots[0]].bank, 23) + ctr(kRouteTiers[kEdgeSlots[1]].bank, 23);
  if (!(in->flags & OTR_BATCH_TILE_ROWS)) out->n_rows = (int64_t)out->counters[8];
  else out->counters[8] = (uint64_t)out->n_rows;
  out->d_hist = ha.hist;
  out->hist_len = (int64_t)hist_len;
  out->kernel_ms[OTR_VITERBI_VARIANT] = (float)vit_variant;
  if (timing) {
    for (int k = 0; k < 10; ++k)
      if (used[k]) (void)hipEventElapsedTime(&out->kernel_ms[k], mat.ev[2 * k], mat.ev[2 * k + 1]);
    for (int t = 0; t < kRouteSlots; ++t)
      if (t != SLOT_FIRST && out->route_tier_code[t] != 0)
        (void)hipEventElapsedTime(&out->route_tier_ms[t], mat.ev[route_event(t)], mat.ev[route_event(t) + 1]);
    out->route_tier_ms[SLOT_FIRST] =
        out->kernel_ms[OTR_STAGE_ROUTE] - out->route_tier_ms[SLOT_SMALL] - out->route_tier_ms[SLOT_TINY];
    (void)hipGetLastError();
  }
}

int Batch::copy_out() {
  int rc;
  int64_t nroute = 0, nseg = 0, nrep = 0;
  for (int t = 0; t < T; ++t) {
    nroute += route_n[t];
    nseg += seg_n[t];
    nrep += rep_n[t];
  }
  out->n_route = nroute;
  out->n_seg = nseg;
  out->n_rep = nrep;
  out->status = out->n_overflow_traces ? OTR_MATCH_ERROR : OTR_OK;
  const bool full = (in->flags & OTR_BATCH_COPY_OUT) != 0;
  if (!full && !(in->flags & OTR_BATCH_COPY_REPORTS)) return OTR_OK;
  out->trace_status = mat.h_trace_status.data();
  if (full) {
    if ((rc = dl(mat.h_trace_state_off, trace_state_off, T + 1))) return rc;
    if ((rc = dl(mat.h_state_probe, state_probe, S))) return rc;
    if ((rc = dl(mat.h_cand_count, cb.count, S))) return rc;
    if ((rc = dl(mat.h_cand_edge, cb.edge, (size_t)S * OTR_KMAX))) return rc;
    if ((rc = dl(mat.h_cand_p, cb.p, (size_t)S * OTR_KMAX))) return rc;
    if ((rc = dl(mat.h_cand_sqd, cb.sqd, (size_t)S * OTR_KMAX))) return rc;
    if ((rc = dl(mat.h_winner, va.winner, S))) return rc;
    if ((rc = dl(mat.h_subpath, va.subpath, S))) return rc;
  }
  if ((rc = dl(mat.h_shape_used, sa.shape_used, T))) return rc;
  if ((rc = dl(mat.h_stats, sa.stats, 7 * (size_t)T))) return rc;
  if ((rc = dl(mat.h_stats_len, sa.stats_len, 2 * (size_t)T))) return rc;
  int64_t nway = 0;
  for (int t = 0; t < T; ++t) nway += way_n[t];
  CompactArgs ca{};
  ca.n_traces = T;
  ca.cap_off = cap_off;
  int64_t* route_off = need<int64_t>(S_C_ROUTE_OFF, T + 1);
  int64_t* seg_off = need<int64_t>(S_C_SEG_OFF, T + 1);
  int64_t* way_off = need<int64_t>(S_C_WAY_OFF, T + 1);
  int64_t* rep_off = need<int64_t>(S_C_REP_OFF, T + 1);
  if ((rc = scan(sa.seg_n, seg_off, T)) || (rc = scan(sa.way_n, way_off, T)) || (rc = scan(sa.rep_n, rep_off, T)))
    return rc;
  if (full && (rc = scan(sa.route_n, route_off, T))) return rc;
  ca.route_off = full ? route_off : nullptr;
  ca.seg_off = seg_off;
  ca.way_off = way_off;
  ca.rep_off = rep_off;
  SegArgs* d_sa = need<SegArgs>(S_C_ARGS, 1);
  HIPCHK(hipMemcpyAsync(d_sa, &sa, sizeof(SegArgs), hipMemcpyHostToDevice, stream));
  ca.s = d_sa;
  auto n1 = [](int64_t n) { return (size_t)(n > 0 ? n : 1); };
  ca.route = need<uint32_t>(S_C_ROUTE, n1(nroute));
  ca.seg_id = need<unsigned long long>(S_C_SEG_ID, n1(nseg));
  ca.seg_start = need<double>(S_C_SEG_START, n1(nseg));
  ca.seg_end = need<double>(S_C_SEG_END, n1(nseg));
  ca.seg_length = need<int32_t>(S_C_SEG_LEN, n1(nseg));
  ca.seg_queue = need<int32_t>(S_C_SEG_QUEUE, n1(nseg));
  ca.seg_internal = need<uint8_t>(S_C_SEG_INTERNAL, n1(nseg));
  ca.seg_bshape = need<int32_t>(S_C_SEG_BSHAPE, n1(nseg));
  ca.seg_eshape = need<int32_t>(S_C_SEG_ESHAPE, n1(nseg));
  ca.seg_way_n = need<int64_t>(S_C_SEG_WAY_N, n1(nseg));
  ca.seg_way = need<uint32_t>(S_C_SEG_WAY, n1(nway));
  ca.rep_id = need<unsigned long long>(S_C_REP_ID, n1(nrep));
  ca.rep_next = need<unsigned long long>(S_C_REP_NEXT, n1(nrep));
  ca.rep_t0 = need<double>(S_C_REP_T0, n1(nrep));
  ca.rep_t1 = need<double>(S_C_REP_T1, n1(nrep));
  ca.rep_length = need<int32_t>(S_C_REP_LEN, n1(nrep));
  ca.rep_queue = need<int32_t>(S_C_REP_QUEUE, n1(nrep));
  k_compact<<<(unsigned)grid_compact(T).blocks, 64, 0, stream>>>(ca);
  int64_t* seg_way_off = need<int64_t>(S_C_SEG_WAY_OFF, (size_t)nseg + 1);
  if ((rc = scan(ca.seg_way_n, seg_way_off, nseg))) return rc;
  HIPCHK(hipGetLastError());
  if (full && (rc = dl(mat.h_route_edge, ca.route, nroute))) return rc;
  if (!full) mat.h_route_edge.clear();
  if ((rc = dl(mat.h_seg_id, ca.seg_id, nseg)) || (rc = dl(mat.h_seg_start, ca.seg_start, nseg)) ||
      (rc = dl(mat.h_seg_end, ca.seg_end, nseg)) || (rc = dl(mat.h_seg_length, ca.seg_length, nseg)) ||
      (rc = dl(mat.h_seg_queue, ca.seg_queue, nseg)) || (rc = dl(mat.h_seg_internal, ca.seg_internal, nseg)) ||
      (rc = dl(mat.h_seg_bshape, ca.seg_bshape, nseg)) || (rc = dl(mat.h_seg_eshape, ca.seg_eshape, nseg)) ||
      (rc = dl(mat.h_seg_way_off, seg_way_off, (size_t)nseg + 1)) || (rc = dl(mat.h_seg_way, ca.seg_way, nway)) ||
      (rc = dl(mat.h_rep_id, ca.rep_id, nrep)) || (rc = dl(mat.h_rep_next, ca.rep_next, nrep)) ||
      (rc = dl(mat.h_rep_t0, ca.rep_t0, nrep)) || (rc = dl(mat.h_rep_t1, ca.rep_t1, nrep)) ||
      (rc = dl(mat.h_rep_length, ca.rep_length, nrep)) || (rc = dl(mat.h_rep_queue, ca.rep_queue, nrep)))
    return rc;
  HIPCHK(hipStreamSynchronize(stream));
  mat.h_trace_route_off.assign(T + 1, 0);
  mat.h_trace_seg_off.assign(T + 1, 0);
  mat.h_trace_rep_off.assign(T + 1, 0);
  for (int t = 0; t < T; ++t) {
    mat.h_trace_route_off[t + 1] = mat.h_trace_route_off[t] + route_n[t];
    mat.h_trace_seg_off[t + 1] = mat.h_trace_seg_off[t] + seg_n[t];
    mat.h_trace_rep_off[t + 1] = mat.h_trace_rep_off[t] + rep_n[t];
  }
  auto P = [](auto& v) { return v.empty() ? nullptr : v.data(); };
  if (full) {
    out->trace_state_off = P(mat.h_trace_state_off);
    out->state_probe = P(mat.h_state_probe);
    out->cand_count = P(mat.h_cand_count);
    out->cand_edge = P(mat.h_cand_edge);
    out->cand_p = P(mat.h_cand_p);
    out->cand_sqd = P(mat.h_cand_sqd);
    out->winner = P(mat.h_winner);
    out->subpath = P(mat.h_subpath);
    out->trace_route_off = P(mat.h_trace_route_off);
    out->route_edge = P(mat.h_route_edge);
  }
  out->trace_seg_off = P(mat.h_trace_seg_off);
  out->seg_id = (uint64_t*)P(mat.h_seg_id);
  out->seg_start = P(mat.h_seg_start);
  out->seg_end = P(mat.h_seg_end);
  out->seg_length = P(mat.h_seg_length);
  out->seg_queue = P(mat.h_seg_queue);
  out->seg_internal = P(mat.h_seg_internal);
  out->seg_begin_shape = P(mat.h_seg_bshape);
  out->seg_end_shape = P(mat.h_seg_eshape);
  out->seg_way_off = P(mat.h_seg_way_off);
  out->seg_way = P(mat.h_seg_way);
  out->trace_rep_off = P(mat.h_trace_rep_off);
  out->rep_id = (uint64_t*)P(mat.h_rep_id);
  out->rep_next = (uint64_t*)P(mat.h_rep_next);
  out->rep_t0 = P(mat.h_rep_t0);
  out->rep_t1 = P(mat.h_rep_t1);
  out->rep_length = P(mat.h_rep_length);
  out->rep_queue = P(mat.h_rep_queue);
  out->shape_used = P(mat.h_shape_used);
  out->stats = P(mat.h_stats);
  out->stats_len = P(mat.h_stats_len);
  return OTR_OK;
}

__global__ void k_report_lists(ReportLists a) {
  const int c = blockIdx.x * blockDim.x + threadIdx.x;
  if (c >= a.n) return;
  const int64_t o = a.seg_off[c];
  ReportStats rs;
  report_segments((int32_t)(a.seg_off[c + 1] - o), a.seg_id + o, a.start + o, a.end + o, a.internal + o, a.queue + o,
                  a.has_length + o, a.length + o, a.begin_shape + o, nullptr, a.end_time[c], a.threshold[c], a.rl[c],
                  a.tl[c], a.rep_id + o, a.rep_next + o, a.rep_t0 + o, a.rep_t1 + o, a.rep_length + o, a.rep_queue + o,
                  nullptr, &rs);
  a.n_rep[c] = rs.n_rep;
  a.shape_used[c] = rs.shape_used;
  for (int k = 0; k < 6; ++k) a.counts[6 * c + k] = rs.counts[k];
  for (int k = 0; k < 2; ++k) {
    a.lengths[2 * c + k] = rs.lengths[k];
    a.length_set[2 * c + k] = rs.length_set[k];
  }
}

int report_lists_device(const ReportLists& h, std::string* err) {
  GraphState& gs = graph_state();
  HIPCHK(hipSetDevice(gs.device));
  const int32_t n = h.n;
  if (n <= 0) return OTR_OK;
  const int64_t S = h.seg_off[n];
  std::vector<void*> mem;
  bool ok = true;
  auto put = [&](const void* src, size_t bytes) -> void* {
    void* d = nullptr;
    if (hipMalloc(&d, bytes ? bytes : 16) != hipSuccess) ok = false;
    mem.push_back(d);
    if (ok && bytes && src && hipMemcpy(d, src, bytes, hipMemcpyHostToDevice) != hipSuccess) ok = false;
    return d;
  };
  ReportLists d = h;
  d.seg_off = (const int64_t*)put(h.seg_off, 8ull * (n + 1));
  d.seg_id = (const unsigned long long*)put(h.seg_id, 8ull * S);
  d.start = (const double*)put(h.start, 8ull * S);
  d.end = (const double*)put(h.end, 8ull * S);
  d.internal = (const uint8_t*)put(h.internal, (size_t)S);
  d.queue = (const int32_t*)put(h.queue, 4ull * S);
  d.has_length = (const uint8_t*)put(h.has_length, (size_t)S);
  d.length = (const int32_t*)put(h.length, 4ull * S);
  d.begin_shape = (const int32_t*)put(h.begin_shape, 4ull * S);
  d.end_time = (const int64_t*)put(h.end_time, 8ull * n);
  d.threshold = (const double*)put(h.threshold, 8ull * n);
  d.rl = (const uint32_t*)put(h.rl, 4ull * n);
  d.tl = (const uint32_t*)put(h.tl, 4ull * n);
  d.rep_id = (unsigned long long*)put(nullptr, 8ull * S);
  d.rep_next = (unsigned long long*)put(nullptr, 8ull * S);
  d.rep_t0 = (double*)put(nullptr, 8ull * S);
  d.rep_t1 = (double*)put(nullptr, 8ull * S);
  d.rep_length = (int32_t*)put(nullptr, 4ull * S);
  d.rep_queue = (int32_t*)put(nullptr, 4ull * S);
  d.n_rep = (int32_t*)put(nullptr, 4ull * n);
  d.shape_used = (int32_t*)put(nullptr, 4ull * n);
  d.counts = (int32_t*)put(nullptr, 24ull * n);
  d.lengths = (double*)put(nullptr, 16ull * n);
  d.length_set = (int32_t*)put(nullptr, 8ull * n);
  auto release = [&] {
    for (void* q : mem)
      if (q) (void)hipFree(q);
  };
  if (!ok) {
    release();
    if (err) *err = "device allocation failed (report lists)";
    return OTR_DEVICE_ERROR;
  }
  k_report_lists<<<grid_ceil(n, 128), 128>>>(d);
  hipError_t e = hipDeviceSynchronize();
  auto get = [&](void* dst, const void* src, size_t bytes) {
    if (e == hipSuccess && bytes) e = hipMemcpy(dst, src, bytes, hipMemcpyDeviceToHost);
  };
  get(h.rep_id, d.rep_id, 8ull * S);
// ... 20 lines not shown
```

### reporter_amd/csrc/otr_kernels.h

```cpp
#pragma once
#include <cstddef>
#include <type_traits>

#include "otr_device.h"
#include "otr_mincode.h"
#include "otr_pred.h"
#include "otr_report.h"
#include "otr_tilerow.h"

#ifndef OTR_CAP1
#define OTR_CAP1 160
#endif
#ifndef OTR_LOAD1
#define OTR_LOAD1 7
#endif
#ifndef OTR_E1CAP
#define OTR_E1CAP 360
#endif
#ifndef OTR_E1LOAD
#define OTR_E1LOAD 14
#endif

namespace otr {

// ... 1171 lines not shown
  const int64_t n = sp >= 0 ? nroot[sp] : 0;
  bool small = false, tiny = false;
  if (sa.ntask4 != nullptr && n > 0 && sa.cand_count[s] <= OTR_WAVE / 4 && !sa.forced[s]) {
    const int md = sa.mode[sa.state_trace[s]] < OTR_MODES ? sa.mode[sa.state_trace[s]] : 0;
    const uint32_t bmm = (uint32_t)bound_mm_of(sa.bound[s]);
    const int32_t bt = sa.bt[s];
#ifdef OTR_FORCE_GENERAL
    const bool general = true;
#else
    const bool general = !pack_fits(bmm, pack_shift(bt)) || ((sa.turn_modes >> md) & 1u);
#endif
    if (!general) {
      float reach = (float)bmm * 1e-3f;
      if (bt >= 0) reach = fminf(reach, (float)bt * 0.1f * sa.est_v[md]);
      const float est = sa.est_k * reach * reach;
      small = est <= sa.small_keys;
      tiny = sa.ntask8 != nullptr && sa.cand_count[s] <= OTR_WAVE / 8 && est <= sa.tiny_keys;
    }
  }
  if (sa.ntask8 != nullptr) sa.ntask8[s] = tiny ? n : 0;
  if (sa.ntask4 != nullptr) sa.ntask4[s] = small && !tiny ? n : 0;
  ntask[s] = small || tiny ? 0 : n;
}

struct RouteArgs {
  const int64_t* task_list;
  int64_t n_tasks;
  const int64_t* prev;
  const double* g;
  const double* bound;
  const uint8_t* forced;
  const int64_t* trans_off;
  uint32_t* trans;
  const int32_t* cand_count;
  const uint32_t* cand_edge;
  const double* cand_p;
  const int32_t* state_trace;
  const uint8_t* mode;
  const uint4* cprep;
  const uint2* cprep_t;
  const uint2* clen;
  const int32_t* bt;
  const uint4* rec;
  const unsigned long long* list_count;
  const int32_t* turn;
  uint32_t* trans_tc;
  double inv_beta[OTR_MODES];
  int32_t* overflow_flag;
  float est_k;
  float est_v[OTR_MODES];
  uint32_t tier_keys[8];
  int n_tiers;
  int64_t unit_base;
  int64_t task_base;
  unsigned long long* queue;
  unsigned long long* stamps;
  int force_edge;
  const unsigned long long* dump_in;
  uint32_t dump_in_words, dump_in_cap;
  unsigned long long* dump_out;
  unsigned long long* dump_ctr;
  uint32_t dump_out_words, dump_out_slots;
  int32_t* task_dump;
};

struct TaskArgs {
  int64_t n_states;
  const int64_t* prev;
  const int32_t* cand_count;
  const uint32_t* cand_edge;
  const uint32_t* edge_dst;
  const int64_t* task_off;
  const double* bound;
  const uint8_t* forced;
  const int32_t* bt;
  const int32_t* state_trace;
  const uint8_t* mode;
  const uint4* cprep;
  const uint2* cprep_t;
  const int64_t* trans_off;
  uint32_t turn_modes;
  uint4* rec;
  const int64_t* ntask4;
  const int64_t* task4_off;
  int64_t nt4;
  const int64_t* ntask8;
  const int64_t* task8_off;
  int64_t nt8;
  int32_t* flag_turn;
  int est_first_keys;
  float est_k;
  float est_v[OTR_MODES];
  uint32_t tier_keys[8];
  int n_tiers;
};

template <int G>
__global__ __launch_bounds__(256) void k_tasks(TaskArgs a) {
  constexpr int GL = OTR_WAVE / G;
  const int64_t s = ((int64_t)blockIdx.x * (blockDim.x / OTR_WAVE) + threadIdx.x / OTR_WAVE) * G +
                    (threadIdx.x % OTR_WAVE) / GL;
  const int lane = threadIdx.x % GL;
  if (s >= a.n_states) return;
  const int64_t sp = a.prev[s];
  if (sp < 0 || a.cand_count[s] <= 0) return;
  const int Ka = a.cand_count[sp];
  const int md = a.mode[a.state_trace[s]] < OTR_MODES ? a.mode[a.state_trace[s]] : 0;
  const uint32_t turn = (a.turn_modes >> md) & 1u;
  const uint32_t ce = lane < Ka ? a.cand_edge[sp * OTR_KMAX + lane] : 0xFFFFFFFFu;
  const uint32_t root = lane < Ka ? (turn ? ce : a.edge_dst[ce]) : 0xFFFFFFFFu;
  const uint32_t w = lane < Ka ? a.cprep[sp * OTR_KMAX + lane].w : 0xFFFFFFFFu;
  const uint32_t t0 = (lane < Ka && !turn) ? a.cprep_t[sp * OTR_KMAX + lane].y : 0u;
  unsigned long long same = 0;
  uint32_t d0min = 0xFFFFFFFFu;
  for (int k = 0; k < Ka; ++k) {
    const uint32_t rk = (uint32_t)__shfl((int)root, k, GL), wk = (uint32_t)__shfl((int)w, k, GL);
    const uint32_t tk = (uint32_t)__shfl((int)t0, k, GL);
    if (rk == root && tk == t0) {
      same |= 1ull << k;
      d0min = wk < d0min ? wk : d0min;
    }
  }
  const bool rep = lane < Ka && (__ffsll((long long)same) - 1) == lane;
  const unsigned long long reps = group_bits<G>(__ballot(rep));
  if (!rep) return;
  const int64_t n4 = a.ntask4 != nullptr ? a.ntask4[s] : 0;
  const int64_t n8 = a.ntask8 != nullptr ? a.ntask8[s] : 0;
  const int64_t tbase = n8 > 0 ? a.task8_off[s] : (n4 > 0 ? a.nt8 + a.task4_off[s] : a.nt8 + a.nt4 + a.task_off[s]);
  const int64_t tend = n8 > 0 ? tbase + n8 : (n4 > 0 ? tbase + n4 : a.nt8 + a.nt4 + a.task_off[s + 1]);
  const int64_t o = tbase + __popcll(reps & ((1ull << lane) - 1ull));
  if (o >= tend) return;
  const uint32_t bmm = (uint32_t)bound_mm_of(a.bound[s]);
  const int32_t bt = a.bt[s];
  const uint32_t sh = pack_shift(bt);
#ifdef OTR_FORCE_GENERAL
  const bool general = true;
#else
  const bool general = !pack_fits(bmm, sh) || turn;
#endif
  uint32_t pre = 0u;
  if (a.est_first_keys > 0 && !general && !turn && !a.forced[s]) {
    float reach = (float)bmm * 1e-3f;
    if (bt >= 0) reach = fminf(reach, (float)bt * 0.1f * a.est_v[md]);
    const float est = a.est_k * reach * reach;
    if (est > (float)a.est_first_keys) {
      uint32_t st = 0;
      while ((int)st + 1 < a.n_tiers && (float)a.tier_keys[st] < est) ++st;
      pre = 1u | (st << 1);
    }
  }
  const uint32_t meta = (uint32_t)a.cand_count[s] | ((uint32_t)md << 8) | ((a.forced[s] ? 1u : 0u) << 10) |
                        (sh << 11) | ((general ? 1u : 0u) << 16) | (turn << 17) | (pre << 18);
  const int64_t to = a.trans_off[s];
  if (turn && a.flag_turn) a.flag_turn[o] = 5;
  a.rec[3 * o] = make_uint4((uint32_t)s, (uint32_t)sp, root, bmm);
  a.rec[3 * o + 1] = make_uint4(d0min, meta, (uint32_t)same, (uint32_t)(same >> 32));
  a.rec[3 * o + 2] = make_uint4(0u, (uint32_t)bt, (uint32_t)to, (uint32_t)((uint64_t)to >> 32));
}

#ifndef OTR_ROUTE2_WAVES
#define OTR_ROUTE2_WAVES 8
#endif

__device__ inline int nth_set_bit(unsigned long long m, int q) {
  for (int j = 0; j < q; ++j) m &= m - 1;
  return __ffsll((long long)m) - 1;
}

template <int CAP, int G, bool LIST, bool WIDE = false, bool CNT = true>
__device__ __forceinline__ void route_unit(const DevGraph& gr, const RouteArgs& a, unsigned long long* counters,
                                           SearchLds<CAP, WIDE ? 2 : 0>* Ls, int64_t w, int64_t n_tasks,
                                           uint32_t* sink, uint4 (*trec)[3]) {
  constexpr int LM = WIDE ? 2 : 0;
  using Gr = Grp<G>;
  const int lane = Gr::gl();
  const int64_t tw = (LIST ? 0 : a.task_base) + w * G + Gr::g();
  const bool have = tw < n_tasks;
  const int64_t task = have ? (LIST ? a.task_list[tw] : tw) : 0;
  OTR_STAMP(ts_in);
  bool search, fits, forced;
  int start_tier = -1;
  uint32_t tnode = kEmpty, tpart = 0, gapT = 1, d0min = 0xFFFFFFFFu, root = 0, bmm = 0, mode_bit = 1;
  uint32_t pd = 0, pt = 0xFFFFFFFFu;
  int Kb;
  Pack K;
  uint32_t ej = 0, e_q = 0, t_q = 0;
  double pj = 0, p_q = 0;
  int iq = 0;
  constexpr bool kKeep = !LIST && !CNT && !old_rounds(G);
  {
    const uint4 r0 = have ? a.rec[3 * task] : make_uint4(0u, 0u, 0u, 0u);
    const uint4 r1 = have ? a.rec[3 * task + 1] : make_uint4(0xFFFFFFFFu, 0u, 0u, 0u);
    const uint4 r2 = have ? a.rec[3 * task + 2] : make_uint4(0u, 0u, 0u, 0u);
    if (lane == 0) {
      trec[Gr::g()][0] = r0;
      trec[Gr::g()][1] = r1;
      trec[Gr::g()][2] = r2;
    }
    const int64_t s = r0.x;
    const unsigned long long mask = ((unsigned long long)r1.w << 32) | r1.z;
    const int64_t sp = r0.y;
    Kb = (int)(r1.y & 0xFFu);
    K.sh = (r1.y >> 11) & 31u;
    const bool general = (r1.y >> 16) & 1u;
    fits = Kb <= Gr::GL && (WIDE || !general) && !((r1.y >> 17) & 1u);
    const bool pre = G >= 2 && !LIST && have && ((r1.y >> 18) & 1u);
    if (pre) {
      start_tier = (int)((r1.y >> 19) & 7u);
      fits = false;
    }
    mode_bit = 1u << ((r1.y >> 8) & 3u);
    bmm = r0.w;
    root = r0.z;
    d0min = r1.x;
    const int32_t bt = (int32_t)r2.y;
    bool needed = false;
    uint4 cq = make_uint4(0u, 0u, 0u, 0u);
    if (have && !pre && lane < Kb) {
      ej = a.cand_edge[s * OTR_KMAX + lane];
      pj = a.cand_p[s * OTR_KMAX + lane];
      cq = a.cprep[s * OTR_KMAX + lane];
      tpart = cq.x;
    }
    const int nsrc = have && !pre ? __popcll(mask) : 0;
    iq = lane < nsrc ? nth_set_bit(mask, lane) : 0;
    if (lane < nsrc) {
      e_q = a.cand_edge[sp * OTR_KMAX + iq];
      p_q = a.cand_p[sp * OTR_KMAX + iq];
      if (bt >= 0) t_q = a.cprep_t[sp * OTR_KMAX + iq].y;
    }
    for (int q = 0; q < nsrc; ++q) {
      uint32_t ei;
      double pi;
      if (q < Gr::GL) {
        ei = (uint32_t)__shfl((int)e_q, q, Gr::GL);
        pi = __shfl(p_q, q, Gr::GL);
      } else {
        const int i = nth_set_bit(mask, q);
        ei = a.cand_edge[sp * OTR_KMAX + i];
        pi = a.cand_p[sp * OTR_KMAX + i];
      }
      if (lane < Kb && !(ej == ei && pj >= pi)) needed = true;
    }
    const uint32_t t0 = (uint32_t)__shfl((int)t_q, 0, Gr::GL);
    bool feasible_root = d0min <= bmm;
    pd = feasible_root ? bmm - d0min : 0u;
    if (bt >= 0) {
      feasible_root = feasible_root && t0 <= (uint32_t)bt;
      pt = t0 <= (uint32_t)bt ? (uint32_t)bt - t0 : 0u;
    }
    forced = have && ((r1.y >> 10) & 1u);
    const unsigned long long need_mask = __ballot(needed);
    search = have && fits && !forced && feasible_root && Gr::mine(need_mask) != 0ull;
    if (needed) {
      tnode = cq.y;
      gapT = cq.z ? cq.z : 1u;
    }
  }
  unsigned long long settled = 0, relaxed = 0, rounds = 0;
  OTR_STAMP(ts_set);
  NDump nd{};
  int dslot = -1;
  constexpr bool kIn = LIST && !WIDE && CAP >= OTR_ND_IN_MIN, kOut = LIST && !WIDE && CAP >= OTR_ND_OUT_MIN;
  constexpr bool kDumps = kIn || kOut;
  if (kIn) {
    const int32_t rs = (a.dump_in != nullptr && search) ? a.task_dump[task] : -1;
    nd.in = rs >= 0 ? a.dump_in + (size_t)rs * a.dump_in_words : nullptr;
  }
  if (kOut) {
    nd.base = a.dump_out;
    nd.ctr = a.dump_ctr;
    nd.words = a.dump_out_words;
    nd.slots = a.dump_out_slots;
#ifdef OTR_FORCE_RETRY
    nd.stop_rounds = (a.force_edge >> 7) & 1 ? 2 + Gr::g() : 0;
#endif
  }
  search_init<CAP, LM, G>(Ls);
  bool ok = search_run<CAP, LM, G, kIn, kOut>(Ls, gr, K, mode_bit, search, root, pd, pt, tnode, tpart, gapT, Kb, &settled,
                                   &relaxed, &rounds, counters ? counters + 16 * kCShards : nullptr, sink,
                                   kDumps ? &nd : nullptr, kDumps ? &dslot : nullptr) &&
            fits;
#ifdef OTR_FORCE_RETRY
  if (G >= 2 && !LIST) ok = false;
#endif
  OTR_STAMP(ts_srch);
  SearchLds<CAP, LM>& L = Ls[Gr::g()];
  int64_t lab = -1;
  if (ok && search && tnode != kEmpty && !forced) {
    const int sl = lds_find(L, tnode);
    if (sl >= 0 && LabelT<LM>::label(L.lab[sl]) != LabelT<LM>::kNone) lab = (int64_t)LabelT<LM>::label(L.lab[sl]);
  }
  asm volatile("" ::: "memory");
  uint32_t ntr = 0;
  if (have && forced && Kb > Gr::GL) {
    const uint4 r1 = trec[Gr::g()][1], r2 = trec[Gr::g()][2];
    const unsigned long long mask = ((unsigned long long)r1.w << 32) | r1.z;
    uint32_t* trow = a.trans + (int64_t)(((uint64_t)r2.w << 32) | r2.z);
    for (int q = 0; q < __popcll(mask); ++q) {
      const int i = nth_set_bit(mask, q);
      for (int j = lane; j < Kb; j += Gr::GL) trow[(int64_t)i * Kb + j] = kNoRoute;
    }
  } else if (have && (ok || forced)) {
    const uint4 r0 = trec[Gr::g()][0], r1 = trec[Gr::g()][1], r2 = trec[Gr::g()][2];
    const int64_t s = r0.x;
    const unsigned long long mask = ((unsigned long long)r1.w << 32) | r1.z;
    if (search) ntr = (uint32_t)Kb * (uint32_t)__popcll(mask);
// ... 1111 lines not shown
```

### reporter_amd/csrc/otr_tiles.hip

```cpp
#include <cstring>
#include <utility>
#include <vector>

#include "otr_devscan.h"
#include "otr_engine.h"
#include "otr_slots.h"
#include "otr_tile_kernels.h"
#include "otr_util_kernels.h"

namespace otr {

int Matcher::tiles_cull(const otr_tile_row* rows, int64_t n, int memory, int privacy, int rules,
                        const otr_tile_row** out, int64_t* n_out, std::string* err) {
  return guarded(stream, err, [&]() -> int {
    GraphState& gs = graph_state();
    HIPCHK(hipSetDevice(gs.device));
    if (!stream) HIPCHK(hipStreamCreateWithFlags(&stream, hipStreamNonBlocking));
    *n_out = 0;
    *out = nullptr;
    h_tile_rows.clear();
    if (n <= 0) return OTR_OK;
    if (n >= (int64_t)INT32_MAX) {
      if (err) *err = "too many tile rows for one call";
      return OTR_BAD_REQUEST;
    }
    otr_tile_row* d_in = need<otr_tile_row>(S_ROWS_IN, n);
    HIPCHK(hipMemcpyAsync(d_in, rows, sizeof(otr_tile_row) * n,
                          memory == OTR_MEM_DEVICE ? hipMemcpyDeviceToDevice : hipMemcpyHostToDevice, stream));
    CulledRows c;
    const int rc = cull_device(d_in, n, privacy, rules, &c, err);
    if (rc != OTR_OK) return rc;
    const int64_t nk = c.n_kept;
    h_tile_rows.resize(nk > 0 ? nk : 1);
    if (nk > 0) HIPCHK(hipMemcpy(h_tile_rows.data(), c.kept, sizeof(otr_tile_row) * nk, hipMemcpyDeviceToHost));
    HIPCHK(hipGetLastError());
    *out = h_tile_rows.data();
    *n_out = nk;
    return OTR_OK;
  });
}

int Matcher::cull_device(const otr_tile_row* d_in, int64_t n, int privacy, int rules, CulledRows* out,
                         std::string* err) {
  return guarded(stream, err, [&]() -> int {
    otr_tile_row* d = need<otr_tile_row>(S_ROWS_OUT, n);
    otr_tile_row* d_kept = need<otr_tile_row>(S_ROWS_KEPT, n);
    int32_t* perm_a = need<int32_t>(S_IDX_A, n);
    int32_t* perm_b = need<int32_t>(S_IDX_B, n);
    unsigned long long* key_a = need<unsigned long long>(S_KEY_A, n);
    unsigned long long* key_b = need<unsigned long long>(S_KEY_B, n);
    int64_t* head = need<int64_t>(S_FILE_HEAD, n);
    int64_t* keep = need<int64_t>(S_KEEP, n);
    int64_t* pos = need<int64_t>(S_POS_SCAN, n);
    int64_t* fstart = need<int64_t>(S_FILE_START, n);
    const int ni = (int)n;
    int rc;
    Workspace tmp;
    if ((rc = scan_sort_bytes(head, pos, key_a, key_b, perm_a, perm_b, ni, &tmp.bytes, stream, err))) return rc;
    tmp.p = need<char>(S_SORT_TMP, tmp.bytes);
    k_iota<int32_t><<<grid_ceil(n, 256), 256, 0, stream>>>(perm_a, n);
    const bool pair_order = rules == OTR_TILE_RULES_STREAM;
    for (int f = pair_order ? TF_NEXT : TF_COUNT - 1; f >= 0; --f) {
      if (pair_order) k_pair_key<<<grid_ceil(n, 256), 256, 0, stream>>>(d_in, perm_a, n, f, key_a);
      else k_line_key<<<grid_ceil(n, 256), 256, 0, stream>>>(d_in, perm_a, n, f, key_a);
      const int end_bit = (f == TF_FILE || pair_order) ? 64 : 63;
      if ((rc = sort_pairs(tmp, key_a, key_b, perm_a, perm_b, ni, 0, end_bit, stream, err))) return rc;
      std::swap(perm_a, perm_b);
    }
    k_gather_rows<<<grid_ceil(n, 256), 256, 0, stream>>>(d_in, perm_a, n, d);
    k_run_heads<<<grid_ceil(n, 256), 256, 0, stream>>>(d, n, head);
    if ((rc = inclusive_sum(tmp, head, pos, ni, stream, err))) return rc;
    k_scatter_index<int64_t><<<grid_ceil(n, 256), 256, 0, stream>>>(head, pos, n, fstart);
    int64_t nr = 0;
    if ((rc = read_back(stream, err, fetch(&nr, pos + (n - 1))))) return rc;
    if (nr < 1 || nr > n) {
      if (err) *err = "tile run split failed";
      return OTR_DEVICE_ERROR;
    }
    uint8_t* run_keep = need<uint8_t>(S_RUN_KEEP, nr);
    k_cull_runs<<<grid_ceil(nr, 256), 256, 0, stream>>>(d, n, fstart, nr, privacy, run_keep);
    k_row_keep<<<grid_ceil(n, 256), 256, 0, stream>>>(pos, run_keep, n, keep);
    if ((rc = inclusive_sum(tmp, keep, head, ni, stream, err))) return rc;
    std::swap(pos, head);
    k_scatter_flagged<otr_tile_row><<<grid_ceil(n, 256), 256, 0, stream>>>(d, keep, pos, n, d_kept);
    int64_t nk = 0;
    if ((rc = read_back(stream, err, fetch(&nk, pos + (n - 1))))) return rc;
    if (nk < 0 || nk > n) {
      if (err) *err = "tile cull compaction failed";
      return OTR_DEVICE_ERROR;
    }
    out->sorted = d;
    out->kept = d_kept;
    out->kept_incl = pos;
    out->n_kept = nk;
    return OTR_OK;
  });
}

__global__ void k_rows_to_entries(const otr_tile_row* r, int64_t n, otr_hist_entry* e) {
  const int64_t i = (int64_t)blockIdx.x * blockDim.x + threadIdx.x;
  if (i >= n) return;
  otr_hist_entry x;
  x.file = r[i].file;
  x.id = r[i].id;
  x.next_id = r[i].next_id;
  x.speed_bin = (uint32_t)r[i].speed_bin;
  x.count = 1u;
  e[i] = x;
}
struct EntryRange {
  unsigned long long id_or, next_or, file_or, bmin, bmax, foreign;
};
constexpr int kRangeBlocks = 128;
__global__ __launch_bounds__(1024) void k_entry_range(const otr_hist_entry* e, int64_t n, EntryRange* r) {
  unsigned long long v[6] = {0ull, 0ull, 0ull, ~0ull, 0ull, 0ull};
  for (int64_t i = (int64_t)blockIdx.x * blockDim.x + threadIdx.x; i < n; i += (int64_t)gridDim.x * blockDim.x) {
    const otr_hist_entry x = e[i];
    v[0] |= x.id;
    v[1] |= x.next_id;
    v[2] |= x.file;
    const unsigned long long b = x.file >> 25;
    v[3] = b < v[3] ? b : v[3];
    v[4] = b > v[4] ? b : v[4];
    v[5] |= (x.file & 0x1FFFFFFull) != (((x.id & 7ull) << 22) | ((x.id >> 3) & 0x3FFFFFull)) ? 1ull : 0ull;
  }
  for (int o = OTR_WAVE / 2; o > 0; o >>= 1) {
    for (int q : {0, 1, 2, 5}) v[q] |= __shfl_xor(v[q], o);
    const unsigned long long a = __shfl_xor(v[3], o), b = __shfl_xor(v[4], o);
    v[3] = a < v[3] ? a : v[3];
    v[4] = b > v[4] ? b : v[4];
  }
  __shared__ unsigned long long part[1024 / OTR_WAVE][6];
  if (lane_id() == 0)
    for (int q = 0; q < 6; ++q) part[threadIdx.x / OTR_WAVE][q] = v[q];
  __syncthreads();
  if (threadIdx.x == 0) {
    for (int w = 1; w < (int)(blockDim.x / OTR_WAVE); ++w) {
      for (int q : {0, 1, 2, 5}) v[q] |= part[w][q];
      v[3] = part[w][3] < v[3] ? part[w][3] : v[3];
      v[4] = part[w][4] > v[4] ? part[w][4] : v[4];
    }
    atomicOr(&r->id_or, v[0]);
    atomicOr(&r->next_or, v[1]);
    atomicOr(&r->file_or, v[2]);
    atomicMin(&r->bmin, v[3]);
    atomicMax(&r->bmax, v[4]);
    atomicOr(&r->foreign, v[5]);
  }
}
static int bit_width(unsigned long long v) { return v ? 64 - __builtin_clzll(v) : 0; }
__global__ void k_entry_key(const otr_hist_entry* e, const int32_t* perm, int64_t n, int field,
                            unsigned long long bmin, unsigned long long* key) {
  const int64_t i = (int64_t)blockIdx.x * blockDim.x + threadIdx.x;
  if (i >= n) return;
  const otr_hist_entry& x = e[perm[i]];
  unsigned long long k;
  switch (field) {
    case 0: k = x.file; break;
    case 1: k = x.id; break;
    case 2: k = x.next_id; break;
    case 3: k = x.speed_bin; break;
    case 4: k = (x.next_id << 3) | (x.speed_bin & 7u); break;
    default:
      k = (((x.file >> 25) - bmin) << 46) | ((x.id & 7ull) << 43) | (((x.id >> 3) & 0x3FFFFFull) << 21) |
          ((x.id >> 25) & 0x1FFFFFull);
  }
  key[i] = k;
}
__global__ void k_gather_entries(const otr_hist_entry* in, const int32_t* idx, int64_t n, otr_hist_entry* out) {
  const int64_t i = (int64_t)blockIdx.x * blockDim.x + threadIdx.x;
  if (i < n) out[i] = in[idx[i]];
}
__global__ void k_entry_heads(const otr_hist_entry* e, int64_t n, int pair, int64_t* head) {
  const int64_t i = (int64_t)blockIdx.x * blockDim.x + threadIdx.x;
  if (i >= n) return;
  bool h = i == 0;
  if (!h) {
    const otr_hist_entry &a = e[i - 1], &b = e[i];
    h = a.file != b.file || a.id != b.id || a.next_id != b.next_id || (!pair && a.speed_bin != b.speed_bin);
  }
  head[i] = h ? 1 : 0;
}
__global__ void k_entry_counts(const otr_hist_entry* e, int64_t n, int64_t* c) {
  const int64_t i = (int64_t)blockIdx.x * blockDim.x + threadIdx.x;
  if (i < n) c[i] = e[i].count;
}
__global__ void k_entry_reduce(const otr_hist_entry* e, int64_t n, const int64_t* run_start, int64_t n_runs,
                               const int64_t* csum, otr_hist_entry* out) {
  const int64_t r = (int64_t)blockIdx.x * blockDim.x + threadIdx.x;
  if (r >= n_runs) return;
  const int64_t s = run_start[r], t = r + 1 < n_runs ? run_start[r + 1] : n;
  otr_hist_entry x = e[s];
  const int64_t tot = csum[t - 1] - (s > 0 ? csum[s - 1] : 0);
  x.count = (uint32_t)(tot < 0xFFFFFFFFll ? tot : 0xFFFFFFFFll);
  out[r] = x;
}
struct PairFile {
  unsigned long long s1, n1, s2, n2;
  int64_t t1, t2;
};
__device__ inline bool pf_after(unsigned long long as, unsigned long long an, unsigned long long bs,
                                unsigned long long bn) {
  return as > bs || (as == bs && an > bn);
}
__device__ inline void pf_add(PairFile& T, unsigned long long s, unsigned long long n, int64_t t) {
  if (pf_after(s, n, T.s1, T.n1)) {
    T.s2 = T.s1;
    T.n2 = T.n1;
    T.t2 = T.t1;
    T.s1 = s;
    T.n1 = n;
    T.t1 = t;
  } else if (pf_after(s, n, T.s2, T.n2)) {
    T.s2 = s;
    T.n2 = n;
    T.t2 = t;
  }
}
__global__ void k_pair_file_heads(const otr_hist_entry* e, const int64_t* pair_start, int64_t n_pairs, int64_t* head) {
  const int64_t p = (int64_t)blockIdx.x * blockDim.x + threadIdx.x;
  if (p < n_pairs) head[p] = p == 0 || e[pair_start[p]].file != e[pair_start[p - 1]].file ? 1 : 0;
}
struct PairKey {
  unsigned long long s, n;
  int64_t t;
};
__global__ void k_pair_keys(const otr_hist_entry* e, const int64_t* pair_start, int64_t n_pairs, int64_t n,
                            const int64_t* csum, PairKey* K) {
  const int64_t p = (int64_t)blockIdx.x * blockDim.x + threadIdx.x;
  if (p >= n_pairs) return;
  const int64_t s = pair_start[p], t = p + 1 < n_pairs ? pair_start[p + 1] : n;
  const otr_hist_entry& x = e[s];
  K[p] = PairKey{dec_key(x.id), dec_key(x.next_id), csum[t - 1] - (s > 0 ? csum[s - 1] : 0)};
}
__global__ __launch_bounds__(1024) void k_pair_file_top2(const PairKey* K, int64_t n_pairs, const int64_t* ffirst,
                                                        int64_t nf, PairFile* F) {
  const int64_t f = blockIdx.x;
  const int64_t p0 = ffirst[f], p1 = f + 1 < nf ? ffirst[f + 1] : n_pairs;
  PairFile T{0ull, 0ull, 0ull, 0ull, 0, 0};
  for (int64_t p = p0 + threadIdx.x; p < p1; p += blockDim.x) {
    const PairKey k = K[p];
    pf_add(T, k.s, k.n, k.t);
  }
  __shared__ PairFile sh[1024];
  sh[threadIdx.x] = T;
  __syncthreads();
  for (int w = 512; w > 0; w >>= 1) {
    if ((int)threadIdx.x < w) {
      const PairFile U = sh[threadIdx.x + w];
      if (U.s1) pf_add(T, U.s1, U.n1, U.t1);
      if (U.s2) pf_add(T, U.s2, U.n2, U.t2);
      sh[threadIdx.x] = T;
    }
    __syncthreads();
  }
  if (threadIdx.x == 0) F[f] = T;
}
__global__ void k_entry_keep(const int64_t* pair_pos, int64_t n, const PairKey* K, const int64_t* fidx,
                             const PairFile* F, int32_t privacy, int64_t* keep) {
  const int64_t i = (int64_t)blockIdx.x * blockDim.x + threadIdx.x;
  if (i >= n) return;
  const int64_t p = pair_pos[i] - 1;
  const PairKey pk = K[p];
  bool k = pk.t >= (int64_t)privacy;
  const PairFile& f = F[fidx[p] - 1];
  if (f.s2 != 0ull && f.t1 == 1) {
    if ((pk.s == f.s1 && pk.n == f.n1) || (pk.s == f.s2 && pk.n == f.n2)) k = f.t2 + 1 >= (int64_t)privacy;
  }
  keep[i] = k ? 1 : 0;
}

int Matcher::copy_out(void* dst, const void* src, size_t bytes, int dst_memory, std::string* err) {
  HIPCHK(hipMemcpyAsync(dst, src, bytes, dst_memory == OTR_MEM_DEVICE ? hipMemcpyDeviceToDevice : hipMemcpyDeviceToHost,
                        stream));
  HIPCHK(hipStreamSynchronize(stream));
  return OTR_OK;
}

int Matcher::hist_reduce(const void* in, int64_t n, int memory, int rows_in, int privacy, const otr_hist_entry** out,
                         int64_t* n_out, std::string* err) {
  return guarded(stream, err, [&]() -> int {
    GraphState& gs = graph_state();
    HIPCHK(hipSetDevice(gs.device));
    if (!stream) HIPCHK(hipStreamCreateWithFlags(&stream, hipStreamNonBlocking));
    *out = nullptr;
    *n_out = 0;
    if (n <= 0) return OTR_OK;
    if (n >= (int64_t)INT32_MAX) {
      if (err) *err = "too many histogram entries for one call";
      return OTR_BAD_REQUEST;
    }
    otr_hist_entry* e_in = need<otr_hist_entry>(S_HE_IN, n);
    otr_hist_entry* e_sorted = need<otr_hist_entry>(S_HE_SORTED, n);
    otr_hist_entry* e_red = need<otr_hist_entry>(S_HE_RED, n);
    otr_hist_entry* e_out = need<otr_hist_entry>(S_HE_OUT, n);
    int32_t* perm_a = need<int32_t>(S_IDX_A, n);
    int32_t* perm_b = need<int32_t>(S_IDX_B, n);
    unsigned long long* key_a = need<unsigned long long>(S_KEY_A, n);
    unsigned long long* key_b = need<unsigned long long>(S_KEY_B, n);
    int64_t* head = need<int64_t>(S_FILE_HEAD, n);
    int64_t* pos = need<int64_t>(S_POS_SCAN, n);
    int64_t* rstart = need<int64_t>(S_FILE_START, n);
    int64_t* csum = need<int64_t>(S_KEEP, n);
    EntryRange* rng = need<EntryRange>(S_HE_RANGE, 1);
    const int ni = (int)n;
    int rc;
    Workspace tmp;
    if ((rc = scan_sort_bytes(head, pos, key_a, key_b, perm_a, perm_b, ni, &tmp.bytes, stream, err))) return rc;
    tmp.p = need<char>(S_SORT_TMP, tmp.bytes);
    const hipMemcpyKind kind = memory == OTR_MEM_DEVICE ? hipMemcpyDeviceToDevice : hipMemcpyHostToDevice;
    if (rows_in) {
      otr_tile_row* rows = need<otr_tile_row>(S_ROWS_IN, n);
      HIPCHK(hipMemcpyAsync(rows, in, sizeof(otr_tile_row) * n, kind, stream));
      k_rows_to_entries<<<grid_ceil(n, 256), 256, 0, stream>>>(rows, n, e_in);
    } else {
      HIPCHK(hipMemcpyAsync(e_in, in, sizeof(otr_hist_entry) * n, kind, stream));
    }
    EntryRange hr{0ull, 0ull, 0ull, ~0ull, 0ull, 0ull};
    HIPCHK(hipMemcpyAsync(rng, &hr, sizeof(hr), hipMemcpyHostToDevice, stream));
    k_entry_range<<<(unsigned)std::min<int64_t>(kRangeBlocks, (n + 1023) / 1024), 1024, 0, stream>>>(e_in, n, rng);
    if ((rc = read_back(stream, err, fetch(&hr, rng)))) return rc;
    std::vector<std::pair<int, int>> passes;
    const int wn = bit_width(hr.next_or), wi = bit_width(hr.id_or), ws = bit_width(hr.bmax - hr.bmin);
    if (wn + 3 <= 64) passes.push_back({4, wn + 3});
    else passes.insert(passes.end(), {{3, 3}, {2, wn}});
    if (!hr.foreign && wi <= 46 && ws + 46 <= 64) passes.push_back({5, std::max(46 + ws, 1)});
    else passes.insert(passes.end(), {{1, std::max(wi, 1)}, {0, std::max(bit_width(hr.file_or), 1)}});
    k_iota<int32_t><<<grid_ceil(n, 256), 256, 0, stream>>>(perm_a, n);
    for (const auto& ps : passes) {
      k_entry_key<<<grid_ceil(n, 256), 256, 0, stream>>>(e_in, perm_a, n, ps.first, hr.bmin, key_a);
      if ((rc = sort_pairs(tmp, key_a, key_b, perm_a, perm_b, ni, 0, ps.second, stream, err))) return rc;
      std::swap(perm_a, perm_b);
    }
    k_gather_entries<<<grid_ceil(n, 256), 256, 0, stream>>>(e_in, perm_a, n, e_sorted);
    k_entry_heads<<<grid_ceil(n, 256), 256, 0, stream>>>(e_sorted, n, 0, head);
    if ((rc = inclusive_sum(tmp, head, pos, ni, stream, err))) return rc;
    k_scatter_index<int64_t><<<grid_ceil(n, 256), 256, 0, stream>>>(head, pos, n, rstart);
    k_entry_counts<<<grid_ceil(n, 256), 256, 0, stream>>>(e_sorted, n, head);
    if ((rc = inclusive_sum(tmp, head, csum, ni, stream, err))) return rc;
    int64_t nr = 0;
    if ((rc = read_back(stream, err, fetch(&nr, pos + (n - 1))))) return rc;
    if (nr < 1 || nr > n) {
      if (err) *err = "histogram run split failed";
      return OTR_DEVICE_ERROR;
    }
    k_entry_reduce<<<grid_ceil(nr, 256), 256, 0, stream>>>(e_sorted, n, rstart, nr, csum, e_red);
    otr_hist_entry* result = e_red;
    int64_t nres = nr;
    if (privacy > 1) {
      const int nri = (int)nr;
      k_entry_heads<<<grid_ceil(nr, 256), 256, 0, stream>>>(e_red, nr, 1, head);
      if ((rc = inclusive_sum(tmp, head, pos, nri, stream, err))) return rc;
      k_scatter_index<int64_t><<<grid_ceil(nr, 256), 256, 0, stream>>>(head, pos, nr, rstart);
      int64_t np = 0;
      HIPCHK(hipMemcpyAsync(&np, pos + (nr - 1), 8, hipMemcpyDeviceToHost, stream));
      k_entry_counts<<<grid_ceil(nr, 256), 256, 0, stream>>>(e_red, nr, head);
      if ((rc = inclusive_sum(tmp, head, csum, nri, stream, err))) return rc;
      HIPCHK(hipStreamSynchronize(stream));
      int64_t* fidx = need<int64_t>(S_HE_FIDX, std::max<int64_t>(np, 1));
      int64_t* fhead = need<int64_t>(S_HE_FHEAD, std::max<int64_t>(np, 1));
      k_pair_file_heads<<<grid_ceil(np, 256), 256, 0, stream>>>(e_red, rstart, np, fhead);
      if ((rc = inclusive_sum(tmp, fhead, fidx, (int)np, stream, err))) return rc;
      int64_t nf = 0;
      if ((rc = read_back(stream, err, fetch(&nf, fidx + (np - 1))))) return rc;
      PairFile* pf = need<PairFile>(S_HE_PFILE, std::max<int64_t>(nf, 1));
      int64_t* ffirst = need<int64_t>(S_HE_FFIRST, std::max<int64_t>(nf, 1));
      PairKey* pkey = need<PairKey>(S_HE_PKEY, std::max<int64_t>(np, 1));
      k_scatter_index<int64_t><<<grid_ceil(np, 256), 256, 0, stream>>>(fhead, fidx, np, ffirst);
      k_pair_keys<<<grid_ceil(np, 256), 256, 0, stream>>>(e_red, rstart, np, nr, csum, pkey);
      k_pair_file_top2<<<(unsigned)nf, 1024, 0, stream>>>(pkey, np, ffirst, nf, pf);
      int64_t* keep = head;
      k_entry_keep<<<grid_ceil(nr, 256), 256, 0, stream>>>(pos, nr, pkey, fidx, pf, privacy, keep);
      int64_t* kpos = rstart;
      if ((rc = inclusive_sum(tmp, keep, kpos, nri, stream, err))) return rc;
      k_scatter_flagged<otr_hist_entry><<<grid_ceil(nr, 256), 256, 0, stream>>>(e_red, keep, kpos, nr, e_out);
      if ((rc = read_back(stream, err, fetch(&nres, kpos + (nr - 1))))) return rc;
      result = e_out;
    }
    HIPCHK(hipGetLastError());
    HIPCHK(hipStreamSynchronize(stream));
    *out = result;
    *n_out = nres;
    return OTR_OK;
  });
}

}
```

### reporter_amd/csrc/otr_util_kernels.h

```cpp
#pragma once
#include <hip/hip_runtime.h>

#include <cstdint>

namespace otr {

template <class T>
__global__ void k_iota(T* v, int64_t n) {
  const int64_t i = (int64_t)blockIdx.x * blockDim.x + threadIdx.x;
  if (i < n) v[i] = (T)i;
}

template <class T>
__global__ void k_gather_by(const T* src, const int32_t* idx, int64_t n, T* dst) {
  const int64_t i = (int64_t)blockIdx.x * blockDim.x + threadIdx.x;
  if (i < n) dst[i] = src[idx[i]];
}

template <class T>
__global__ void k_scatter_flagged(const T* in, const int64_t* flag, const int64_t* pos, int64_t n, T* out) {
  const int64_t i = (int64_t)blockIdx.x * blockDim.x + threadIdx.x;
  if (i < n && flag[i]) out[pos[i] - 1] = in[i];
}

template <class Out>
__global__ void k_scatter_index(const int64_t* flag, const int64_t* pos, int64_t n, Out* out) {
  const int64_t i = (int64_t)blockIdx.x * blockDim.x + threadIdx.x;
  if (i < n && flag[i]) out[pos[i] - 1] = (Out)i;
}

}
```

Baseline: 36.96 million probes/s.

## Batch device readbacks through pinned mailbox and fuse multi-column scans

Result: faster. 37.70 million probes/s, median of 6 (+2.0%).

```diff
diff --git a/reporter_amd/csrc/otr_devscan.h b/reporter_amd/csrc/otr_devscan.h
--- a/reporter_amd/csrc/otr_devscan.h
+++ b/reporter_amd/csrc/otr_devscan.h
@@ -34,6 +34,28 @@
   return OTR_OK;
 }
 
+template <int K, bool SHIFT>
+struct ArrayColumns {
+  const int64_t* p[K];
+  __host__ __device__ int64_t operator()(int q, int64_t i) const {
+    if (!p[q]) return 0;
+    if (SHIFT) return i > 0 ? p[q][i - 1] : 0;
+    return p[q][i];
+  }
+};
+
+template <class T>
+struct ShiftedLoad {
+  const T* src;
+  __host__ __device__ T operator()(int64_t i) const { return i > 0 ? src[i - 1] : T(0); }
+};
+template <class T>
+using ShiftedInput = hipcub::TransformInputIterator<T, ShiftedLoad<T>, hipcub::CountingInputIterator<int64_t>>;
+template <class T>
+ShiftedInput<T> shifted_input(const T* src) {
+  return ShiftedInput<T>(hipcub::CountingInputIterator<int64_t>(0), ShiftedLoad<T>{src});
+}
+
 template <class In, class Out>
 int inclusive_sum(Workspace ws, In in, Out out, int n, hipStream_t stream, std::string* err) {
   HIPCHK(hipcub::DeviceScan::InclusiveSum(ws.p, ws.bytes, in, out, n, stream));
@@ -44,6 +66,75 @@
 int sort_pairs(Workspace ws, const K* k_in, K* k_out, const V* v_in, V* v_out, int n, int begin_bit, int end_bit,
                hipStream_t stream, std::string* err) {
   HIPCHK(hipcub::DeviceRadixSort::SortPairs(ws.p, ws.bytes, k_in, k_out, v_in, v_out, n, begin_bit, end_bit, stream));
+  return OTR_OK;
+}
+
+template <int K>
+struct TupleK {
+  int64_t v[K];
+};
+template <int K>
+struct TupleAdd {
+  __host__ __device__ TupleK<K> operator()(const TupleK<K>& a, const TupleK<K>& b) const {
+    TupleK<K> r;
+    for (int q = 0; q < K; ++q) r.v[q] = a.v[q] + b.v[q];
+    return r;
+  }
+};
+template <int K, class Load>
+struct TupleLoad {
+  Load load;
+  __host__ __device__ TupleK<K> operator()(int64_t i) const {
+    TupleK<K> r;
+    for (int q = 0; q < K; ++q) r.v[q] = load(q, i);
+    return r;
+  }
+};
+template <int K>
+struct TupleOut {
+  int64_t* out[K];
+  int64_t at;
+  struct Ref {
+    int64_t* out[K];
+    int64_t i;
+    __host__ __device__ const Ref& operator=(const TupleK<K>& x) const {
+      for (int q = 0; q < K; ++q)
+        if (out[q]) out[q][i] = x.v[q];
+      return *this;
+    }
+  };
+  using iterator_category = std::random_access_iterator_tag;
+  using value_type = TupleK<K>;
+  using difference_type = int64_t;
+  using pointer = void;
+  using reference = Ref;
+  __host__ __device__ Ref operator[](int64_t n) const {
+    Ref r;
+    for (int q = 0; q < K; ++q) r.out[q] = out[q];
+    r.i = at + n;
+    return r;
+  }
+  __host__ __device__ Ref operator*() const { return (*this)[0]; }
+  __host__ __device__ TupleOut operator+(int64_t n) const {
+    TupleOut r = *this;
+    r.at += n;
+    return r;
+  }
+  __host__ __device__ TupleOut& operator+=(int64_t n) {
+    at += n;
+    return *this;
+  }
+};
+template <int K, class Load>
+using TupleInput = hipcub::TransformInputIterator<TupleK<K>, TupleLoad<K, Load>, hipcub::CountingInputIterator<int64_t>>;
+
+template <int K, class Load>
+int tuple_sums(Workspace* ws, Load load, int64_t* const (&out)[K], int n, hipStream_t stream, std::string* err) {
+  TupleInput<K, Load> in(hipcub::CountingInputIterator<int64_t>(0), TupleLoad<K, Load>{load});
+  TupleOut<K> o{};
+  for (int q = 0; q < K; ++q) o.out[q] = out[q];
+  o.at = 0;
+  HIPCHK(hipcub::DeviceScan::InclusiveScan(ws->p, ws->bytes, in, o, TupleAdd<K>(), n, stream));
   return OTR_OK;
 }
 
diff --git a/reporter_amd/csrc/otr_engine.h b/reporter_amd/csrc/otr_engine.h
--- a/reporter_amd/csrc/otr_engine.h
+++ b/reporter_amd/csrc/otr_engine.h
@@ -1,6 +1,7 @@
 #pragma once
 #include <hip/hip_runtime.h>
 
+#include <initializer_list>
 #include <shared_mutex>
 #include <string>
 #include <vector>
@@ -103,6 +104,19 @@
   DevPool pool{PoolOwner::matcher, nullptr, 0};
   GSlab gslab[2];
   std::vector<int32_t> h_turn;
+  const int32_t* turn_dev = nullptr;
+  std::vector<char> seg_args;
+  const void* seg_args_dev = nullptr;
+  static constexpr int kMailWords = 512;
+  unsigned long long* mail = nullptr;
+  struct MailRun {
+    const void* src;
+    int words;
+  };
+  int post(std::initializer_list<MailRun> runs, unsigned long long* dst, std::string* err);
+  int post_wait(std::initializer_list<MailRun> runs, std::string* err);
+  unsigned long long* h_drain = nullptr;
+  size_t h_drain_words = 0;
   std::vector<int64_t> h_trace_state_off, h_state_probe, h_trace_route_off, h_trace_seg_off, h_seg_way_off,
       h_trace_rep_off;
   std::vector<int32_t> h_cand_count, h_winner, h_subpath, h_seg_length, h_seg_queue, h_seg_bshape, h_seg_eshape,
diff --git a/reporter_amd/csrc/otr_engine.hip b/reporter_amd/csrc/otr_engine.hip
--- a/reporter_amd/csrc/otr_engine.hip
+++ b/reporter_amd/csrc/otr_engine.hip
@@ -15,6 +15,7 @@
 #include "otr_points.h"
 #include "otr_slots.h"
 #include "otr_traversals.h"
+#include "otr_util_kernels.h"
 
 namespace otr {
 static_assert(kTraceWaves == 4, "grid_trace_rows (otr_launch.h) assumes 4 traces per block");
@@ -372,12 +373,40 @@
   if (tst) tile_store_destroy(tst);
   if (ttx) tile_text_destroy(ttx);
   pool.release();
+  if (mail) (void)hipHostFree(mail);
+  if (h_drain) (void)hipHostFree(h_drain);
   for (auto& sl : gslab)
     for (void* q : {(void*)sl.key, (void*)sl.lab, (void*)sl.qmark, (void*)sl.fr, (void*)sl.touched})
       if (q) (void)hipFree(q);
   if (ev_init)
     for (auto& e : ev) (void)hipEventDestroy(e);
   if (stream) (void)hipStreamDestroy(stream);
+}
+
+int Matcher::post(std::initializer_list<MailRun> runs, unsigned long long* dst, std::string* err) {
+  if (!mail) HIPCHK(hipHostMalloc((void**)&mail, 8 * kMailWords, hipHostMallocMapped | hipHostMallocCoherent));
+  PostArgs a{};
+  int q = 0, words = 0;
+  for (const MailRun& r : runs) {
+    if (q >= kPostRuns || r.words < 0 || (!dst && words + r.words > kMailWords)) {
+      if (err) *err = "mailbox record too large";
+      return OTR_DEVICE_ERROR;
+    }
+    a.src[q] = (const unsigned long long*)r.src;
+    a.n[q] = r.words;
+    words += r.words;
+    ++q;
+  }
+  a.dst = dst;
+  if (!dst) HIPCHK(hipHostGetDevicePointer((void**)&a.dst, mail, 0));
+  k_post<<<1, 64, 0, stream>>>(a);
+  return OTR_OK;
+}
+
+int Matcher::post_wait(std::initializer_list<MailRun> runs, std::string* err) {
+  if (int rc = post(runs, nullptr, err)) return rc;
+  HIPCHK(hipStreamSynchronize(stream));
+  return OTR_OK;
 }
 
 __global__ void k_capacity(int32_t n_traces, const int64_t* trace_state_off, const int32_t* cand_count,
@@ -424,9 +453,45 @@
   block_append(sel, i, list, count);
 }
 
-__global__ void k_collect_flagged(int64_t n, const int32_t* flag, int64_t* list, unsigned long long* count) {
-  const int64_t i = (int64_t)blockIdx.x * blockDim.x + threadIdx.x;
-  block_append(i < n && flag[i] != 0, i, list, count);
+constexpr int kFlagsPerThread = 4, kFlaggedBlock = 1024;
+__global__ __launch_bounds__(kFlaggedBlock) void k_collect_flagged(int64_t n, const int32_t* flag, int64_t* list,
+                                                                  unsigned long long* count) {
+  __shared__ unsigned int s_wave[kFlaggedBlock / OTR_WAVE];
+  __shared__ unsigned long long s_base;
+  const int64_t i0 = ((int64_t)blockIdx.x * kFlaggedBlock + threadIdx.x) * kFlagsPerThread;
+  int4 f = make_int4(0, 0, 0, 0);
+  if (i0 + 3 < n) {
+    f = *reinterpret_cast<const int4*>(flag + i0);
+  } else if (i0 < n) {
+    f.x = flag[i0];
+    if (i0 + 1 < n) f.y = flag[i0 + 1];
+    if (i0 + 2 < n) f.z = flag[i0 + 2];
+  }
+  const unsigned int c = (f.x != 0) + (f.y != 0) + (f.z != 0) + (f.w != 0);
+  const int lane = (int)(threadIdx.x % OTR_WAVE), w = (int)(threadIdx.x / OTR_WAVE);
+  unsigned int incl = c;
+  for (int o = 1; o < OTR_WAVE; o <<= 1) {
+    const unsigned int v = (unsigned int)__shfl_up((int)incl, o);
+    if (lane >= o) incl += v;
+  }
+  if (lane == OTR_WAVE - 1) s_wave[w] = incl;
+  __syncthreads();
+  if (threadIdx.x == 0) {
+    unsigned int t = 0;
+    for (int k = 0; k < kFlaggedBlock / OTR_WAVE; ++k) {
+      const unsigned int x = s_wave[k];
+      s_wave[k] = t;
+      t += x;
+    }
+    s_base = t ? atomicAdd(count, (unsigned long long)t) : 0ull;
+  }
+  __syncthreads();
+  if (c == 0) return;
+  int64_t o = (int64_t)s_base + s_wave[w] + (incl - c);
+  if (f.x != 0) list[o++] = i0;
+  if (f.y != 0) list[o++] = i0 + 1;
+  if (f.z != 0) list[o++] = i0 + 2;
+  if (f.w != 0) list[o++] = i0 + 3;
 }
 
 __global__ void k_collect_tier_from(const int64_t* cand, const unsigned long long* n_cand, int32_t* flag,
@@ -505,16 +570,20 @@
 }
 
 __global__ void k_step_list(int64_t n_states, const int64_t* prev, const uint8_t* brk, const int32_t* cand_count,
-                            int64_t* list, unsigned long long* count) {
+                            int64_t* list, unsigned long long* count, int32_t* ovf) {
   const int64_t s = (int64_t)blockIdx.x * blockDim.x + threadIdx.x;
+  if (s < n_states) ovf[s] = 0;
+  if (s == 0) ovf[n_states] = 0;
   block_append(s < n_states && cand_count[s] > 0 && prev[s] >= 0 && !brk[s], s, list, count);
 }
 
 __global__ void k_step_lists(int64_t n_states, const int64_t* prev, const uint8_t* brk, const int32_t* cand_count,
                              PathClass pc, int64_t* list, unsigned long long* count_front,
-                             unsigned long long* count_back, unsigned long long* n_all) {
+                             unsigned long long* count_back, unsigned long long* n_all, int32_t* ovf) {
   const int64_t s = (int64_t)blockIdx.x * blockDim.x + threadIdx.x;
   if (s == 0) *n_all = (unsigned long long)n_states;
+  if (s < n_states) ovf[s] = 0;
+  if (s == 0) ovf[n_states] = 0;
   const bool hit = s < n_states && cand_count[s] > 0 && prev[s] >= 0 && !brk[s];
   bool small = false;
   if (hit) {
@@ -566,6 +635,8 @@
 }
 
 constexpr unsigned kCollectGrid = 512;
+
+static constexpr size_t line(size_t words) { return (words + 31) / 32 * 32; }
 
 struct Batch {
   Matcher& mat;
@@ -606,7 +677,12 @@
   double tiny_keys = 0.0;
   static constexpr size_t bank = (size_t)OTR_COUNTERS * kCShards;
   static constexpr size_t n_ctr = kBanks * (size_t)OTR_COUNTERS;
-  unsigned long long *d_counters = nullptr, *cnt = nullptr;
+  static constexpr int kPQWords = 16 * 8;
+  static constexpr size_t kCntAt = line(kBanks * bank + n_ctr);
+  static constexpr size_t kQueuesAt = kCntAt + line(C_CURSORS + kShards);
+  static constexpr size_t kPQAt = kQueuesAt + line((size_t)kQueues * kQueueWords);
+  static constexpr size_t kControlWords = kPQAt + line(8 * kPQWords);
+  unsigned long long *d_counters = nullptr, *cnt = nullptr, *pq = nullptr;
   int64_t *list = nullptr, *fail_tasks = nullptr, *flagged = nullptr;
   int32_t *task_ovf = nullptr, *d_turn = nullptr;
   uint32_t *trans = nullptr, *trans_tc = nullptr;
@@ -619,12 +695,14 @@
   const unsigned long long* nscan_d = nullptr;
   int32_t* step_ovf = nullptr;
   bool small_paths = false;
-  std::vector<unsigned long long> hc;
+  int64_t* cap = nullptr;
+  int path_attempts = 0;
+  const unsigned long long* hc = nullptr;
   unsigned long long h_fail[2] = {0ull, 0ull};
-  std::vector<int64_t> route_n, seg_n, way_n, rep_n;
-
-  int upload(), states(), candidates(), link(), route_first(), route_retry(), route_edge(), route_global(), viterbi();
-  int paths(), paths_attempt(int64_t capacity), segments(), points(), traversals(), drain(), debug_fail(),
+  const int64_t *route_n = nullptr, *seg_n = nullptr, *way_n = nullptr, *rep_n = nullptr;
+
+  int upload(), check_probes(), states(), candidates(), link(), route_first(), route_retry(), route_edge(), route_global(), viterbi();
+  int paths(), paths_attempt(int64_t capacity, bool again), segments(), points(), traversals(), drain(), debug_fail(),
       name_failed();
   void fold_counters();
   int copy_out(), points_out(), traversals_out();
@@ -651,6 +729,10 @@
 
   int scan(const int64_t* src, int64_t* dst_np1, int64_t n);
   int read_i64(const int64_t* p, int64_t* v);
+  template <class... R>
+  int post_wait(R... runs) {
+    return mat.post_wait({runs...}, err);
+  }
   int slabs(int tier, GSlabs* out);
   template <class V>
   int dl(V& vec, const void* src, size_t n) {
@@ -739,7 +821,6 @@
     b.mode = d_mode;
     b.acc = d_acc;
   } else {
-    if (int rc = read_back(stream, err, fetch(&N, in->trace_offsets + T))) return rc;
     b.trace_off = in->trace_offsets;
     b.lat = in->lat;
     b.lon = in->lon;
@@ -747,6 +828,16 @@
     b.mode = in->mode;
     b.acc = in->accuracy;
   }
+  mat.h_trace_status.assign(T, OTR_OK);
+  d_counters = need<unsigned long long>(S_COUNTERS, kControlWords);
+  cnt = d_counters + kCntAt;
+  queues = d_counters + kQueuesAt;
+  pq = d_counters + kPQAt;
+  HIPCHK(hipMemsetAsync(d_counters, 0, kControlWords * 8, stream));
+  return in->memory == OTR_MEM_HOST ? check_probes() : OTR_OK;
+}
+
+int Batch::check_probes() {
   out->n_probes = N;
   if (N > kMaxBatchProbes || max_launch_items(N, N, 1) > kMaxDispatchItems) {
     if (err)
@@ -754,23 +845,23 @@
              " per otr_match_batch call";
     return OTR_BAD_REQUEST;
   }
-  mat.h_trace_status.assign(T, OTR_OK);
-  d_counters = need<unsigned long long>(S_COUNTERS, kBanks * bank + n_ctr);
-  HIPCHK(hipMemsetAsync(d_counters, 0, kBanks * bank * 8, stream));
   return OTR_OK;
 }
 
 int Batch::scan(const int64_t* src, int64_t* dst_np1, int64_t n) {
-  HIPCHK(hipMemsetAsync(dst_np1, 0, 8, stream));
-  if (n == 0) return OTR_OK;
+  const auto in0 = shifted_input(src);
   Workspace tmp;
-  if (int rc = otr::scan_bytes(src, dst_np1 + 1, (int)n, &tmp.bytes, stream, err)) return rc;
+  if (int rc = otr::scan_bytes(in0, dst_np1, (int)n + 1, &tmp.bytes, stream, err)) return rc;
   scan_bytes = std::max(scan_bytes, tmp.bytes);
   tmp.p = need<char>(S_SCAN_TMP, scan_bytes);
-  return inclusive_sum(tmp, src, dst_np1 + 1, (int)n, stream, err);
-}
-
-int Batch::read_i64(const int64_t* p, int64_t* v) { return read_back(stream, err, fetch(v, p)); }
+  return inclusive_sum(tmp, in0, dst_np1, (int)n + 1, stream, err);
+}
+
+int Batch::read_i64(const int64_t* p, int64_t* v) {
+  if (int rc = post_wait(Matcher::MailRun{p, 1})) return rc;
+  *v = (int64_t)mat.mail[0];
+  return OTR_OK;
+}
 
 int Batch::states() {
   int rc;
@@ -780,7 +871,14 @@
   k_select_states<<<grid_ceil(T, 256), 256, 0, stream>>>(b, mp, state_cnt, nullptr, nullptr, nullptr);
   te(OTR_STAGE_STATES);
   if ((rc = scan(state_cnt, trace_state_off, T))) return rc;
-  if ((rc = read_i64(trace_state_off + T, &S))) return rc;
+  if (in->memory == OTR_MEM_HOST) {
+    if ((rc = read_i64(trace_state_off + T, &S))) return rc;
+  } else {
+    if ((rc = post_wait(Matcher::MailRun{trace_state_off + T, 1}, Matcher::MailRun{in->trace_offsets + T, 1}))) return rc;
+    S = (int64_t)mat.mail[0];
+    N = (int64_t)mat.mail[1];
+    if ((rc = check_probes())) return rc;
+  }
   out->n_states = S;
   state_probe = need<int64_t>(S_STATE_PROBE, S);
   state_trace = need<int32_t>(S_STATE_TRACE, S);
@@ -891,14 +989,23 @@
     sm.small_keys = (float)small_keys;
     k_ntask<<<grid_ceil(S, 256), 256, 0, stream>>>(S, sb.prev, pr.nroot, sb.ntask, sm);
   }
-  if ((rc = scan(sb.ntask, task_off, S))) return rc;
-  if (small_tier && (rc = scan(ntask4, task4_off, S))) return rc;
-  if (tiny_tier && (rc = scan(ntask8, task8_off, S))) return rc;
-  if ((rc = scan(sb.ntrans, trans_off, S))) return rc;
-  HIPCHK(hipMemcpyAsync(&NT, task_off + S, 8, hipMemcpyDeviceToHost, stream));
-  if (small_tier) HIPCHK(hipMemcpyAsync(&NT4, task4_off + S, 8, hipMemcpyDeviceToHost, stream));
-  if (tiny_tier) HIPCHK(hipMemcpyAsync(&NT8, task8_off + S, 8, hipMemcpyDeviceToHost, stream));
-  if ((rc = read_back(stream, err, fetch(&NTR, trans_off + S)))) return rc;
+  {
+    const ArrayColumns<4, true> cols{{sb.ntask, sb.ntrans, ntask4, ntask8}};
+    int64_t* const offs[4] = {task_off, trans_off, task4_off, task8_off};
+    Workspace tmp;
+    if ((rc = tuple_sums<4>(&tmp, cols, offs, (int)S + 1, stream, err))) return rc;
+    scan_bytes = std::max(scan_bytes, tmp.bytes);
+    tmp.p = need<char>(S_SCAN_TMP, scan_bytes);
+    if ((rc = tuple_sums<4>(&tmp, cols, offs, (int)S + 1, stream, err))) return rc;
+  }
+  if ((rc = post_wait(Matcher::MailRun{task_off + S, 1}, Matcher::MailRun{trans_off + S, 1},
+                      Matcher::MailRun{small_tier ? task4_off + S : nullptr, small_tier ? 1 : 0},
+                      Matcher::MailRun{tiny_tier ? task8_off + S : nullptr, tiny_tier ? 1 : 0})))
+    return rc;
+  NT = (int64_t)mat.mail[0];
+  NTR = (int64_t)mat.mail[1];
+  if (small_tier) NT4 = (int64_t)mat.mail[2];
+  if (tiny_tier) NT8 = (int64_t)mat.mail[3];
   NT += NT4 + NT8;
   task_ovf = need<int32_t>(S_TASK_OVF, NT);
   trans = need<uint32_t>(S_TRANS, NTR);
@@ -934,9 +1041,20 @@
     for (int m = 0; m < OTR_MODES; ++m) ta.est_v[m] = est_v[m];
     ta.n_tiers = n_est_tiers;
     for (int t = 0; t < n_est_tiers; ++t) ta.tier_keys[t] = est_tier_keys[t];
-    if (NT > 0) HIPCHK(hipMemsetAsync(task_ovf, 0, 4 * NT, stream));
+    static const bool debug_tasks = getenv("OTR_DEBUG_TASKS") != nullptr;
+    if (debug_tasks && NT > 0) HIPCHK(hipMemsetAsync(task_ovf, 0x7F, 4 * NT, stream));
     if (k32) k_tasks<2><<<(unsigned)grid_per_state_waves(S, 2).blocks, 256, 0, stream>>>(ta);
     else k_tasks<1><<<(unsigned)grid_per_state_waves(S, 1).blocks, 256, 0, stream>>>(ta);
+    if (debug_tasks && NT > 0) {
+      std::vector<int32_t> h((size_t)NT);
+      HIPCHK(hipMemcpyAsync(h.data(), task_ovf, 4 * NT, hipMemcpyDeviceToHost, stream));
+      HIPCHK(hipStreamSynchronize(stream));
+      const int64_t written = NT - std::count(h.begin(), h.end(), 0x7F7F7F7F);
+      if (written != NT) {
+        if (err) *err = "k_tasks wrote " + std::to_string(written) + " of " + std::to_string(NT) + " task flags";
+        return OTR_DEVICE_ERROR;
+      }
+    }
   }
   te(OTR_STAGE_LINK);
   return OTR_OK;
@@ -1039,9 +1157,18 @@
 
 int Batch::route_first() {
   d_turn = need<int32_t>(S_TURN, 181 * OTR_MODES);
-  mat.h_turn.resize(181 * OTR_MODES);
-  for (int m = 0; m < OTR_MODES; ++m) turn_table(mp.m[m].turn_penalty_factor, mat.h_turn.data() + 181 * m);
-  HIPCHK(hipMemcpyAsync(d_turn, mat.h_turn.data(), 4 * 181 * OTR_MODES, hipMemcpyHostToDevice, stream));
+  {
+    int32_t tab[181 * OTR_MODES];
+    for (int m = 0; m < OTR_MODES; ++m) turn_table(mp.m[m].turn_penalty_factor, tab + 181 * m);
+    if (mat.turn_dev != d_turn || mat.h_turn.size() != (size_t)(181 * OTR_MODES) ||
+        memcmp(mat.h_turn.data(), tab, sizeof(tab)) != 0) {
+      mat.turn_dev = nullptr;
+      HIPCHK(hipStreamSynchronize(stream));
+      mat.h_turn.assign(tab, tab + 181 * OTR_MODES);
+      HIPCHK(hipMemcpyAsync(d_turn, mat.h_turn.data(), sizeof(tab), hipMemcpyHostToDevice, stream));
+      mat.turn_dev = d_turn;
+    }
+  }
   ra.task_list = nullptr;
   ra.n_tasks = NT;
   ra.prev = sb.prev;
@@ -1069,8 +1196,6 @@
   for (int m = 0; m < OTR_MODES; ++m) ra.est_v[m] = est_v[m];
   ra.n_tiers = n_est_tiers;
   for (int t = 0; t < n_est_tiers; ++t) ra.tier_keys[t] = est_tier_keys[t];
-  cnt = need<unsigned long long>(S_MISC, C_CURSORS + kShards);
-  HIPCHK(hipMemsetAsync(cnt, 0, 8 * (C_CURSORS + kShards), stream));
   list = need<int64_t>(S_LIST, std::max<int64_t>(NT, S));
   fail_tasks = need<int64_t>(S_GFLAG, std::max<int64_t>(NT, 1));
   flagged = need<int64_t>(S_FLAGGED, std::max<int64_t>(NT, 1));
@@ -1107,8 +1232,6 @@
     ra.force_edge = fe ? atoi(fe) : 0;
   }
 #endif
-  queues = need<unsigned long long>(S_QUEUE, kQueues * kQueueWords);
-  HIPCHK(hipMemsetAsync(queues, 0, 8 * kQueues * kQueueWords, stream));
   static const bool nresume_env = !getenv("OTR_NRESUME") || atoi(getenv("OTR_NRESUME")) != 0;
   static const bool eresume_env = !getenv("OTR_E1RESUME") || atoi(getenv("OTR_E1RESUME")) != 0;
   nresume = nresume_env;
@@ -1136,7 +1259,8 @@
   tb(OTR_STAGE_ROUTE_BIG);
   const std::vector<int>& tiers = route_tiers();
   const int ntier = (int)tiers.size();
-  k_collect_flagged<<<grid_ceil(NT, 1024), 1024, 0, stream>>>(NT, task_ovf, flagged, cnt + C_FLAGGED);
+  k_collect_flagged<<<grid_ceil(NT, kFlaggedBlock * kFlagsPerThread), kFlaggedBlock, 0, stream>>>(
+      NT, task_ovf, flagged, cnt + C_FLAGGED);
   unsigned long long* ndump[2] = {nullptr, nullptr};
   uint32_t nslots[8] = {0u, 0u, 0u, 0u, 0u, 0u, 0u, 0u};
   auto nd_in = [&](int t) { return t > 0 && t < ntier && tiers[t] / 10 >= OTR_ND_IN_MIN; };
@@ -1331,13 +1455,13 @@
   if (S > 0) k_fill_i32<<<grid_ceil(S, 256), 256, 0, stream>>>(path_len, S, 0);
   {
     steps = need<int64_t>(S_LIST2, std::max<int64_t>(S, 1));
+    step_ovf = need<int32_t>(S_STEP_OVF, S + 1);
     nsteps_d = cnt + C_STEPS;
     static const double small_path_keys =
         getenv("OTR_SMALL_PATH_KEYS") ? atof(getenv("OTR_SMALL_PATH_KEYS")) : kSmallPathKeys;
     small_paths = small_path_keys > 0.0 && est_k > 0.f && (small_path_keys >= 1e8 || 2 * (NT4 + NT8) >= NT);
     nsteps4_d = cnt + C_STEPS_FRONT;
     unsigned long long* nall_d = cnt + C_STEPS_ALL;
-    static_assert(C_STEPS_ALL == C_STEPS_FRONT + 1, "cleared together below");
     if (S > 0 && small_paths) {
       PathClass pc{};
       pc.winner = va.winner;
@@ -1349,47 +1473,58 @@
       pc.turn_modes = turn_modes;
       pc.est4 = 8.f * est_k;
       pc.small_keys = (float)small_path_keys;
-      HIPCHK(hipMemsetAsync(nsteps4_d, 0, 16, stream));
       k_step_lists<<<grid_ceil(S, 256), 256, 0, stream>>>(S, sb.prev, va.brk, cb.count, pc, steps, nsteps4_d, nsteps_d,
-                                                          nall_d);
-      if ((rc = read_back(stream, err, fetch(&h_nsteps[0], nsteps4_d), fetch(&h_nsteps[1], nsteps_d)))) return rc;
+                                                          nall_d, step_ovf);
+      if ((rc = post_wait(Matcher::MailRun{nsteps4_d, 1}, Matcher::MailRun{nsteps_d, 1}))) return rc;
+      h_nsteps[0] = mat.mail[0];
+      h_nsteps[1] = mat.mail[1];
     } else if (S > 0) {
-      k_step_list<<<grid_ceil(S, 1024), 1024, 0, stream>>>(S, sb.prev, va.brk, cb.count, steps, nsteps_d);
+      k_step_list<<<grid_ceil(S, 1024), 1024, 0, stream>>>(S, sb.prev, va.brk, cb.count, steps, nsteps_d, step_ovf);
     }
     nscan_d = small_paths ? nall_d : nsteps_d;
-    step_ovf = need<int32_t>(S_STEP_OVF, S + 1);
-    int64_t capacity = kShards * ((int64_t)S * 24 / kShards + 1024);
-    bool paths_fit = S == 0;
-    for (int attempt = 0; attempt < 8 && S > 0; ++attempt) {
-      if ((rc = paths_attempt(capacity))) return rc;
-      unsigned long long capflag = 0;
-      std::vector<unsigned long long> cur(kShards);
-      HIPCHK(hipMemcpyAsync(&capflag, cnt + C_CAP_FLAG, 8, hipMemcpyDeviceToHost, stream));
-      HIPCHK(hipMemcpyAsync(cur.data(), cnt + C_CURSORS, 8 * kShards, hipMemcpyDeviceToHost, stream));
-      HIPCHK(hipStreamSynchronize(stream));
-      if ((capflag & 0xFFFFFFFFu) == 0) {
+    static const int64_t cap0 = getenv("OTR_PATH_CAP0") ? atoll(getenv("OTR_PATH_CAP0")) : 0;
+    int64_t capacity = cap0 > 0 ? kShards * ((cap0 + kShards - 1) / kShards)
+                                : kShards * ((int64_t)S * 24 / kShards + 1024);
+    cap = need<int64_t>(S_CAP, T);
+    cap_off = need<int64_t>(S_CAP_OFF, T + 1);
+    bool paths_fit = false;
+    for (int attempt = 0; attempt < 8; ++attempt) {
+      path_attempts = attempt + 1;
+      if (S > 0 && (rc = paths_attempt(capacity, attempt > 0))) return rc;
+      k_capacity<<<grid_ceil(T, 256), 256, 0, stream>>>(T, trace_state_off, cb.count, path_len, cap);
+      if ((rc = scan(cap, cap_off, T))) return rc;
+      if ((rc = post_wait(Matcher::MailRun{cnt + C_CAP_FLAG, 1}, Matcher::MailRun{cap_off + T, 1},
+                          Matcher::MailRun{cnt + C_CURSORS, kShards})))
+        return rc;
+      if ((mat.mail[0] & 0xFFFFFFFFu) == 0) {
+        C = (int64_t)mat.mail[1];
         paths_fit = true;
         break;
       }
       unsigned long long mx = 0;
-      for (auto c : cur) mx = c > mx ? c : mx;
+      for (int q = 0; q < kShards; ++q) mx = std::max(mx, mat.mail[2 + q]);
       capacity = kShards * ((int64_t)mx + (int64_t)mx / 2 + 1024);
     }
     if (!paths_fit) {
       if (err) *err = "winner paths did not fit the path buffer after 8 attempts";
       return OTR_DEVICE_ERROR;
     }
-  }
-  return OTR_OK;
-}
-
-int Batch::paths_attempt(int64_t capacity) {
+    if (path_attempts > 1 && getenv("OTR_DEBUG_FAIL"))
+      fprintf(stderr, "otr: winner paths regrown: %d attempts, %lld entries\n", path_attempts, (long long)capacity);
+  }
+  return OTR_OK;
+}
+
+int Batch::paths_attempt(int64_t capacity, bool again) {
   int rc;
   uint32_t* path = need<uint32_t>(S_PATH, capacity);
-  HIPCHK(hipMemsetAsync(step_ovf, 0, 4 * (S + 1), stream));
-  HIPCHK(hipMemsetAsync(cnt + C_PATH_TIER, 0, 8 * (C_CAP_FLAG + 1 - C_PATH_TIER), stream));
-  HIPCHK(hipMemsetAsync(cnt + C_EDGE_PATH, 0, 8 * 2, stream));
-  HIPCHK(hipMemsetAsync(cnt + C_CURSORS, 0, 8 * kShards, stream));
+  if (again) {
+    HIPCHK(hipMemsetAsync(step_ovf, 0, 4 * (S + 1), stream));
+    HIPCHK(hipMemsetAsync(cnt + C_PATH_TIER, 0, 8 * (C_CAP_FLAG + 1 - C_PATH_TIER), stream));
+    HIPCHK(hipMemsetAsync(cnt + C_EDGE_PATH, 0, 8 * 2, stream));
+    HIPCHK(hipMemsetAsync(cnt + C_CURSORS, 0, 8 * kShards, stream));
+    HIPCHK(hipMemsetAsync(pq, 0, 8 * 8 * kPQWords, stream));
+  }
   PathArgs pa{};
   pa.steps = steps;
   pa.n_steps = S;
@@ -1417,9 +1552,6 @@
   pa.trans_off = trans_off;
   pa.trans = trans;
   pa.force_edge = ra.force_edge;
-  constexpr int kPQWords = 16 * 8;
-  unsigned long long* pq = need<unsigned long long>(S_PQUEUE, 8 * kPQWords);
-  HIPCHK(hipMemsetAsync(pq, 0, 8 * 8 * kPQWords, stream));
   tb(OTR_STAGE_PATHS);
   if (small_paths) {
     if (h_nsteps[0] > 0) {
@@ -1487,11 +1619,6 @@
 
 int Batch::segments() {
   int rc;
-  int64_t* cap = need<int64_t>(S_CAP, T);
-  cap_off = need<int64_t>(S_CAP_OFF, T + 1);
-  k_capacity<<<grid_ceil(T, 256), 256, 0, stream>>>(T, trace_state_off, cb.count, path_len, cap);
-  if ((rc = scan(cap, cap_off, T))) return rc;
-  if ((rc = read_i64(cap_off + T, &C))) return rc;
   sa.b = b;
   sa.trace_state_off = trace_state_off;
   sa.state_probe = state_probe;
@@ -1516,7 +1643,8 @@
   sa.gstart = need<int32_t>(S_GSTART, C);
   sa.cap_off = cap_off;
   sa.route = need<uint32_t>(S_ROUTE, C);
-  sa.route_n = need<int64_t>(S_ROUTE_N, T);
+  int64_t* counts = need<int64_t>(S_ROUTE_N, 4 * (size_t)T + n_ctr + 2);
+  sa.route_n = counts;
   sa.seg_id = need<unsigned long long>(S_SEG_ID, C);
   sa.seg_start = need<double>(S_SEG_START, C);
   sa.seg_end = need<double>(S_SEG_END, C);
@@ -1526,10 +1654,10 @@
   sa.seg_bshape = need<int32_t>(S_SEG_BSHAPE, C);
   sa.seg_eshape = need<int32_t>(S_SEG_ESHAPE, C);
   sa.seg_index = need<uint32_t>(S_SEG_INDEX, C);
-  sa.seg_n = need<int64_t>(S_SEG_N, T);
+  sa.seg_n = counts + T;
   sa.seg_way_n = need<int64_t>(S_SEG_WAY_N, C);
   sa.seg_way = need<uint32_t>(S_SEG_WAY, C);
-  sa.way_n = need<int64_t>(S_WAY_N, T);
+  sa.way_n = counts + 3 * (size_t)T;
   sa.rep_id = need<unsigned long long>(S_REP_ID, C);
   sa.rep_next = need<unsigned long long>(S_REP_NEXT, C);
   sa.rep_t0 = need<double>(S_REP_T0, C);
@@ -1537,7 +1665,7 @@
   sa.rep_length = need<int32_t>(S_REP_LEN, C);
   sa.rep_queue = need<int32_t>(S_REP_QUEUE, C);
   sa.rep_seg = need<uint32_t>(S_REP_SEG, C);
-  sa.rep_n = need<int64_t>(S_REP_N, T);
+  sa.rep_n = counts + 2 * (size_t)T;
   sa.shape_used = need<int32_t>(S_SHAPE_USED, T);
   sa.stats = need<int32_t>(S_STATS, 7 * (size_t)T);
   sa.stats_len = need<double>(S_STATS_LEN, 2 * (size_t)T);
@@ -1841,17 +1969,26 @@
 }
 
 int Batch::drain() {
-  hc.resize(n_ctr);
-  k_ctr_fold<<<(unsigned)n_ctr, kCShards, 0, stream>>>(d_counters, d_counters + kBanks * bank);
-  HIPCHK(hipMemcpyAsync(hc.data(), d_counters + kBanks * bank, n_ctr * 8, hipMemcpyDeviceToHost, stream));
-  HIPCHK(hipMemcpyAsync(&h_fail[0], cnt + C_TASKS_LEFT, 8, hipMemcpyDeviceToHost, stream));
-  HIPCHK(hipMemcpyAsync(&h_fail[1], cnt + C_PATHS_LEFT, 8, hipMemcpyDeviceToHost, stream));
-  route_n.resize(T), seg_n.resize(T), way_n.resize(T), rep_n.resize(T);
-  HIPCHK(hipMemcpyAsync(route_n.data(), sa.route_n, 8 * T, hipMemcpyDeviceToHost, stream));
-  HIPCHK(hipMemcpyAsync(seg_n.data(), sa.seg_n, 8 * T, hipMemcpyDeviceToHost, stream));
-  HIPCHK(hipMemcpyAsync(rep_n.data(), sa.rep_n, 8 * T, hipMemcpyDeviceToHost, stream));
-  HIPCHK(hipMemcpyAsync(way_n.data(), sa.way_n, 8 * T, hipMemcpyDeviceToHost, stream));
+  const size_t words = 4 * (size_t)T + n_ctr + 2;
+  unsigned long long* slab = (unsigned long long*)sa.route_n;
+  k_ctr_fold<<<(unsigned)n_ctr, kCShards, 0, stream>>>(d_counters, slab + 4 * (size_t)T);
+  if (int rc = mat.post({Matcher::MailRun{cnt + C_TASKS_LEFT, 1}, Matcher::MailRun{cnt + C_PATHS_LEFT, 1}},
+                        slab + 4 * (size_t)T + n_ctr, err))
+    return rc;
+  if (mat.h_drain_words < words) {
+    if (mat.h_drain) (void)hipHostFree(mat.h_drain);
+    mat.h_drain = nullptr;
+    mat.h_drain_words = 0;
+    HIPCHK(hipHostMalloc((void**)&mat.h_drain, 8 * (words + words / 4), hipHostMallocDefault));
+    mat.h_drain_words = words + words / 4;
+  }
+  HIPCHK(hipMemcpyAsync(mat.h_drain, slab, 8 * words, hipMemcpyDeviceToHost, stream));
   HIPCHK(hipStreamSynchronize(stream));
+  const int64_t* h = (const int64_t*)mat.h_drain;
+  route_n = h, seg_n = h + T, rep_n = h + 2 * (size_t)T, way_n = h + 3 * (size_t)T;
+  hc = mat.h_drain + 4 * (size_t)T;
+  h_fail[0] = hc[n_ctr];
+  h_fail[1] = hc[n_ctr + 1];
   return OTR_OK;
 }
 
@@ -2004,7 +2141,15 @@
   ca.way_off = way_off;
   ca.rep_off = rep_off;
   SegArgs* d_sa = need<SegArgs>(S_C_ARGS, 1);
-  HIPCHK(hipMemcpyAsync(d_sa, &sa, sizeof(SegArgs), hipMemcpyHostToDevice, stream));
+  static_assert(sizeof(SegArgs) <= 8 * Matcher::kMailWords, "SegArgs goes through the mailbox");
+  if (mat.seg_args_dev != d_sa || mat.seg_args.size() != sizeof(SegArgs) ||
+      memcmp(mat.seg_args.data(), &sa, sizeof(SegArgs)) != 0) {
+    mat.seg_args_dev = nullptr;
+    mat.seg_args.assign((const char*)&sa, (const char*)&sa + sizeof(SegArgs));
+    memcpy(mat.mail, &sa, sizeof(SegArgs));
+    HIPCHK(hipMemcpyAsync(d_sa, mat.mail, sizeof(SegArgs), hipMemcpyHostToDevice, stream));
+    mat.seg_args_dev = d_sa;
+  }
   ca.s = d_sa;
   auto n1 = [](int64_t n) { return (size_t)(n > 0 ? n : 1); };
   ca.route = need<uint32_t>(S_C_ROUTE, n1(nroute));
diff --git a/reporter_amd/csrc/otr_kernels.h b/reporter_amd/csrc/otr_kernels.h
--- a/reporter_amd/csrc/otr_kernels.h
+++ b/reporter_amd/csrc/otr_kernels.h
@@ -1347,7 +1347,7 @@
   const uint32_t meta = (uint32_t)a.cand_count[s] | ((uint32_t)md << 8) | ((a.forced[s] ? 1u : 0u) << 10) |
                         (sh << 11) | ((general ? 1u : 0u) << 16) | (turn << 17) | (pre << 18);
   const int64_t to = a.trans_off[s];
-  if (turn && a.flag_turn) a.flag_turn[o] = 5;
+  if (a.flag_turn) a.flag_turn[o] = turn ? 5 : 0;
   a.rec[3 * o] = make_uint4((uint32_t)s, (uint32_t)sp, root, bmm);
   a.rec[3 * o + 1] = make_uint4(d0min, meta, (uint32_t)same, (uint32_t)(same >> 32));
   a.rec[3 * o + 2] = make_uint4(0u, (uint32_t)bt, (uint32_t)to, (uint32_t)((uint64_t)to >> 32));
diff --git a/reporter_amd/csrc/otr_tiles.hip b/reporter_amd/csrc/otr_tiles.hip
--- a/reporter_amd/csrc/otr_tiles.hip
+++ b/reporter_amd/csrc/otr_tiles.hip
@@ -97,8 +97,11 @@
   });
 }
 
-__global__ void k_rows_to_entries(const otr_tile_row* r, int64_t n, otr_hist_entry* e) {
+struct EntryRange;
+__device__ inline void entry_range_init(EntryRange* rng);
+__global__ void k_rows_to_entries(const otr_tile_row* r, int64_t n, otr_hist_entry* e, EntryRange* rng) {
   const int64_t i = (int64_t)blockIdx.x * blockDim.x + threadIdx.x;
+  if (i == 0) entry_range_init(rng);
   if (i >= n) return;
   otr_hist_entry x;
   x.file = r[i].file;
@@ -111,6 +114,8 @@
 struct EntryRange {
   unsigned long long id_or, next_or, file_or, bmin, bmax, foreign;
 };
+__device__ inline void entry_range_init(EntryRange* rng) { *rng = EntryRange{0ull, 0ull, 0ull, ~0ull, 0ull, 0ull}; }
+__global__ void k_entry_range_init(EntryRange* rng) { entry_range_init(rng); }
 constexpr int kRangeBlocks = 128;
 __global__ __launch_bounds__(1024) void k_entry_range(const otr_hist_entry* e, int64_t n, EntryRange* r) {
   unsigned long long v[6] = {0ull, 0ull, 0ull, ~0ull, 0ull, 0ull};
@@ -150,10 +155,11 @@
 }
 static int bit_width(unsigned long long v) { return v ? 64 - __builtin_clzll(v) : 0; }
 __global__ void k_entry_key(const otr_hist_entry* e, const int32_t* perm, int64_t n, int field,
-                            unsigned long long bmin, unsigned long long* key) {
+                            unsigned long long bmin, unsigned long long* key, int32_t* iota) {
   const int64_t i = (int64_t)blockIdx.x * blockDim.x + threadIdx.x;
   if (i >= n) return;
-  const otr_hist_entry& x = e[perm[i]];
+  if (iota) iota[i] = (int32_t)i;
+  const otr_hist_entry& x = e[iota ? i : perm[i]];
   unsigned long long k;
   switch (field) {
     case 0: k = x.file; break;
@@ -167,9 +173,18 @@
   }
   key[i] = k;
 }
-__global__ void k_gather_entries(const otr_hist_entry* in, const int32_t* idx, int64_t n, otr_hist_entry* out) {
+__global__ void k_gather_entries(const otr_hist_entry* in, const int32_t* idx, int64_t n, otr_hist_entry* out,
+                                 int64_t* head) {
   const int64_t i = (int64_t)blockIdx.x * blockDim.x + threadIdx.x;
-  if (i < n) out[i] = in[idx[i]];
+  if (i >= n) return;
+  const otr_hist_entry b = in[idx[i]];
+  out[i] = b;
+  bool h = i == 0;
+  if (!h) {
+    const otr_hist_entry& a = in[idx[i - 1]];
+    h = a.file != b.file || a.id != b.id || a.next_id != b.next_id || a.speed_bin != b.speed_bin;
+  }
+  head[i] = h ? 1 : 0;
 }
 __global__ void k_entry_heads(const otr_hist_entry* e, int64_t n, int pair, int64_t* head) {
   const int64_t i = (int64_t)blockIdx.x * blockDim.x + threadIdx.x;
@@ -181,10 +196,11 @@
   }
   head[i] = h ? 1 : 0;
 }
-__global__ void k_entry_counts(const otr_hist_entry* e, int64_t n, int64_t* c) {
-  const int64_t i = (int64_t)blockIdx.x * blockDim.x + threadIdx.x;
-  if (i < n) c[i] = e[i].count;
-}
+struct HeadCountColumns {
+  const int64_t* head;
+  const otr_hist_entry* e;
+  __host__ __device__ int64_t operator()(int q, int64_t i) const { return q == 0 ? head[i] : (int64_t)e[i].count; }
+};
 __global__ void k_entry_reduce(const otr_hist_entry* e, int64_t n, const int64_t* run_start, int64_t n_runs,
                                const int64_t* csum, otr_hist_entry* out) {
   const int64_t r = (int64_t)blockIdx.x * blockDim.x + threadIdx.x;
@@ -217,9 +233,11 @@
     T.t2 = t;
   }
 }
-__global__ void k_pair_file_heads(const otr_hist_entry* e, const int64_t* pair_start, int64_t n_pairs, int64_t* head) {
+__global__ void k_pair_file_heads(const otr_hist_entry* e, const int64_t* pair_start, const int64_t* n_pairs,
+                                  int64_t n_max, int64_t* head) {
   const int64_t p = (int64_t)blockIdx.x * blockDim.x + threadIdx.x;
-  if (p < n_pairs) head[p] = p == 0 || e[pair_start[p]].file != e[pair_start[p - 1]].file ? 1 : 0;
+  if (p >= n_max) return;
+  head[p] = p < *n_pairs && (p == 0 || e[pair_start[p]].file != e[pair_start[p - 1]].file) ? 1 : 0;
 }
 struct PairKey {
   unsigned long long s, n;
@@ -307,39 +325,53 @@
     int rc;
     Workspace tmp;
     if ((rc = scan_sort_bytes(head, pos, key_a, key_b, perm_a, perm_b, ni, &tmp.bytes, stream, err))) return rc;
+    {
+      Workspace q;
+      int64_t* const two[2] = {pos, csum};
+      if ((rc = tuple_sums<2>(&q, HeadCountColumns{head, e_sorted}, two, ni, stream, err))) return rc;
+      tmp.bytes = std::max(tmp.bytes, q.bytes);
+    }
     tmp.p = need<char>(S_SORT_TMP, tmp.bytes);
     const hipMemcpyKind kind = memory == OTR_MEM_DEVICE ? hipMemcpyDeviceToDevice : hipMemcpyHostToDevice;
     if (rows_in) {
-      otr_tile_row* rows = need<otr_tile_row>(S_ROWS_IN, n);
-      HIPCHK(hipMemcpyAsync(rows, in, sizeof(otr_tile_row) * n, kind, stream));
-      k_rows_to_entries<<<grid_ceil(n, 256), 256, 0, stream>>>(rows, n, e_in);
+      const otr_tile_row* rows = (const otr_tile_row*)in;
+      if (memory != OTR_MEM_DEVICE) {
+        otr_tile_row* staged = need<otr_tile_row>(S_ROWS_IN, n);
+        HIPCHK(hipMemcpyAsync(staged, in, sizeof(otr_tile_row) * n, kind, stream));
+        rows = staged;
+      }
+      k_rows_to_entries<<<grid_ceil(n, 256), 256, 0, stream>>>(rows, n, e_in, rng);
     } else {
       HIPCHK(hipMemcpyAsync(e_in, in, sizeof(otr_hist_entry) * n, kind, stream));
-    }
-    EntryRange hr{0ull, 0ull, 0ull, ~0ull, 0ull, 0ull};
-    HIPCHK(hipMemcpyAsync(rng, &hr, sizeof(hr), hipMemcpyHostToDevice, stream));
+      k_entry_range_init<<<1, 1, 0, stream>>>(rng);
+    }
+    static_assert(sizeof(EntryRange) == 6 * 8, "six mailbox words");
     k_entry_range<<<(unsigned)std::min<int64_t>(kRangeBlocks, (n + 1023) / 1024), 1024, 0, stream>>>(e_in, n, rng);
-    if ((rc = read_back(stream, err, fetch(&hr, rng)))) return rc;
+    if ((rc = post_wait({MailRun{rng, 6}}, err))) return rc;
+    EntryRange hr;
+    memcpy(&hr, mail, sizeof(hr));
     std::vector<std::pair<int, int>> passes;
     const int wn = bit_width(hr.next_or), wi = bit_width(hr.id_or), ws = bit_width(hr.bmax - hr.bmin);
     if (wn + 3 <= 64) passes.push_back({4, wn + 3});
     else passes.insert(passes.end(), {{3, 3}, {2, wn}});
     if (!hr.foreign && wi <= 46 && ws + 46 <= 64) passes.push_back({5, std::max(46 + ws, 1)});
     else passes.insert(passes.end(), {{1, std::max(wi, 1)}, {0, std::max(bit_width(hr.file_or), 1)}});
-    k_iota<int32_t><<<grid_ceil(n, 256), 256, 0, stream>>>(perm_a, n);
+    bool first = true;
     for (const auto& ps : passes) {
-      k_entry_key<<<grid_ceil(n, 256), 256, 0, stream>>>(e_in, perm_a, n, ps.first, hr.bmin, key_a);
+      k_entry_key<<<grid_ceil(n, 256), 256, 0, stream>>>(e_in, perm_a, n, ps.first, hr.bmin, key_a,
+                                                         first ? perm_a : nullptr);
+      first = false;
       if ((rc = sort_pairs(tmp, key_a, key_b, perm_a, perm_b, ni, 0, ps.second, stream, err))) return rc;
       std::swap(perm_a, perm_b);
     }
-    k_gather_entries<<<grid_ceil(n, 256), 256, 0, stream>>>(e_in, perm_a, n, e_sorted);
-    k_entry_heads<<<grid_ceil(n, 256), 256, 0, stream>>>(e_sorted, n, 0, head);
-    if ((rc = inclusive_sum(tmp, head, pos, ni, stream, err))) return rc;
+    k_gather_entries<<<grid_ceil(n, 256), 256, 0, stream>>>(e_in, perm_a, n, e_sorted, head);
+    {
+      int64_t* const two[2] = {pos, csum};
+      if ((rc = tuple_sums<2>(&tmp, HeadCountColumns{head, e_sorted}, two, ni, stream, err))) return rc;
+    }
     k_scatter_index<int64_t><<<grid_ceil(n, 256), 256, 0, stream>>>(head, pos, n, rstart);
-    k_entry_counts<<<grid_ceil(n, 256), 256, 0, stream>>>(e_sorted, n, head);
-    if ((rc = inclusive_sum(tmp, head, csum, ni, stream, err))) return rc;
-    int64_t nr = 0;
-    if ((rc = read_back(stream, err, fetch(&nr, pos + (n - 1))))) return rc;
+    if ((rc = post_wait({MailRun{pos + (n - 1), 1}}, err))) return rc;
+    const int64_t nr = (int64_t)mail[0];
     if (nr < 1 || nr > n) {
       if (err) *err = "histogram run split failed";
       return OTR_DEVICE_ERROR;
@@ -350,19 +382,21 @@
     if (privacy > 1) {
       const int nri = (int)nr;
       k_entry_heads<<<grid_ceil(nr, 256), 256, 0, stream>>>(e_red, nr, 1, head);
-      if ((rc = inclusive_sum(tmp, head, pos, nri, stream, err))) return rc;
+      {
+        int64_t* const two[2] = {pos, csum};
+        if ((rc = tuple_sums<2>(&tmp, HeadCountColumns{head, e_red}, two, nri, stream, err))) return rc;
+      }
       k_scatter_index<int64_t><<<grid_ceil(nr, 256), 256, 0, stream>>>(head, pos, nr, rstart);
-      int64_t np = 0;
-      HIPCHK(hipMemcpyAsync(&np, pos + (nr - 1), 8, hipMemcpyDeviceToHost, stream));
-      k_entry_counts<<<grid_ceil(nr, 256), 256, 0, stream>>>(e_red, nr, head);
-      if ((rc = inclusive_sum(tmp, head, csum, nri, stream, err))) return rc;
-      HIPCHK(hipStreamSynchronize(stream));
-      int64_t* fidx = need<int64_t>(S_HE_FIDX, std::max<int64_t>(np, 1));
-      int64_t* fhead = need<int64_t>(S_HE_FHEAD, std::max<int64_t>(np, 1));
-      k_pair_file_heads<<<grid_ceil(np, 256), 256, 0, stream>>>(e_red, rstart, np, fhead);
-      if ((rc = inclusive_sum(tmp, fhead, fidx, (int)np, stream, err))) return rc;
-      int64_t nf = 0;
-      if ((rc = read_back(stream, err, fetch(&nf, fidx + (np - 1))))) return rc;
+      int64_t* fidx = need<int64_t>(S_HE_FIDX, nr);
+      int64_t* fhead = need<int64_t>(S_HE_FHEAD, nr);
+      k_pair_file_heads<<<grid_ceil(nr, 256), 256, 0, stream>>>(e_red, rstart, pos + (nr - 1), nr, fhead);
+      if ((rc = inclusive_sum(tmp, fhead, fidx, nri, stream, err))) return rc;
+      if ((rc = post_wait({MailRun{pos + (nr - 1), 1}, MailRun{fidx + (nr - 1), 1}}, err))) return rc;
+      const int64_t np = (int64_t)mail[0], nf = (int64_t)mail[1];
+      if (np < 1 || np > nr || nf < 1 || nf > np) {
+        if (err) *err = "histogram pair split failed";
+        return OTR_DEVICE_ERROR;
+      }
       PairFile* pf = need<PairFile>(S_HE_PFILE, std::max<int64_t>(nf, 1));
       int64_t* ffirst = need<int64_t>(S_HE_FFIRST, std::max<int64_t>(nf, 1));
       PairKey* pkey = need<PairKey>(S_HE_PKEY, std::max<int64_t>(np, 1));
@@ -374,7 +408,8 @@
       int64_t* kpos = rstart;
       if ((rc = inclusive_sum(tmp, keep, kpos, nri, stream, err))) return rc;
       k_scatter_flagged<otr_hist_entry><<<grid_ceil(nr, 256), 256, 0, stream>>>(e_red, keep, kpos, nr, e_out);
-      if ((rc = read_back(stream, err, fetch(&nres, kpos + (nr - 1))))) return rc;
+      if ((rc = post_wait({MailRun{kpos + (nr - 1), 1}}, err))) return rc;
+      nres = (int64_t)mail[0];
       result = e_out;
     }
     HIPCHK(hipGetLastError());
diff --git a/reporter_amd/csrc/otr_util_kernels.h b/reporter_amd/csrc/otr_util_kernels.h
--- a/reporter_amd/csrc/otr_util_kernels.h
+++ b/reporter_amd/csrc/otr_util_kernels.h
@@ -29,4 +29,19 @@
   if (i < n && flag[i]) out[pos[i] - 1] = (Out)i;
 }
 
+constexpr int kPostRuns = 8;
+struct PostArgs {
+  const unsigned long long* src[kPostRuns];
+  int n[kPostRuns];
+  unsigned long long* dst;
+};
+template <int RUNS = kPostRuns>
+__global__ void k_post(PostArgs a) {
+  int o = 0;
+  for (int q = 0; q < RUNS; ++q) {
+    for (int i = threadIdx.x; i < a.n[q]; i += blockDim.x) a.dst[o + i] = a.src[q][i];
+    o += a.n[q];
+  }
 }
+
+}
```
